# fnzhan/EMLight

Hardware: AMD Instinct MI355X
Metric: training images/sec (regression step: DenseNet-BC fwd + Sinkhorn loss + bwd + Adam) (higher is better)
Workload: dtype f32; 1 GPU; RegressionNetwork train step, BASELINE configs[1]; per_gpu_batch=64, global_batch=64, anchors=128, parallelism=single

## Files before the change

### emlight_amd/RegressionNetwork/dense_engine_bwd.py

```python
import ctypes
import os

import torch

from .. import _lib
from .._knobs import knob_choice, knob_flag


def _r16(v):
    return (v + 15) // 16 * 16


def _side_stream(dev, prio):
    if prio <= 0:
        return torch.cuda.Stream(device=dev, priority=prio)
    hip = ctypes.CDLL("libamdhip64.so")
    h = ctypes.c_void_p()
    with torch.cuda.device(dev):
        rc = hip.hipStreamCreateWithPriority(ctypes.byref(h), ctypes.c_uint(1), ctypes.c_int(prio))
    if rc != 0:
        raise RuntimeError("hipStreamCreateWithPriority failed (%d)" % rc)
    return torch.cuda.ExternalStream(h.value, device=dev)


def _masked_stream(dev, n_cu, keep):
    hip = ctypes.CDLL("libamdhip64.so")
    words = (n_cu + 31) // 32
    mask = (ctypes.c_uint32 * words)()
    for i in range(n_cu):
        if keep(i):
            mask[i // 32] |= 1 << (i % 32)
    h = ctypes.c_void_p()
    with torch.cuda.device(dev):
        rc = hip.hipExtStreamCreateWithCUMask(ctypes.byref(h), ctypes.c_uint32(words), mask)
    if rc != 0:
        raise RuntimeError("hipExtStreamCreateWithCUMask failed (%d)" % rc)
    return torch.cuda.ExternalStream(h.value, device=dev)


class _BwdBuffers:
    def __init__(self, enc, ws, dev):
        f32 = dict(dtype=torch.float32, device=dev)
        self.G = [torch.zeros(blk["P"], blk["ld"], **f32) for blk in ws.blocks]
        self.GF = torch.zeros(ws.F.shape[0], ws.F.shape[1], **f32)
        maxP = ws.blocks[0]["P"]
        self.DZ = torch.empty(2, maxP, 48, **f32)
        self.ring = max(1, int(os.environ.get("EML_WGRAD_RING", 4))) if enc.overlap_wgrad(dev) else 1
        self.GF12 = [torch.empty(maxP, 12, **f32) for _ in range(self.ring)]
        self.N12 = torch.empty(maxP, 12, **f32)
        self.TOP = torch.empty(2 * maxP * 12, **f32) if knob_flag("EML_DGRAD_TOP", True) else None
        kp, ko, g = enc.kp_max, max(enc.ko_max, 48), enc.grid_max
        self.Wd = [[torch.empty(lay["Kp"] * 48, **f32) for lay in blk["layers"]] for blk in ws.blocks]
        self.WdT = [torch.empty(blk["trans"]["Kp"] * blk["trans"]["Ko"], **f32) for blk in ws.blocks]
        self.permutes = None
        self.coef = torch.zeros(8, max(kp, ko), **f32)
        self.part2 = torch.zeros(2, g * kp * 2, dtype=torch.float64, device=dev)
        self.partW = torch.empty(g * max(kp * 48, 2 * 27 * 256, 4 * 1024), **f32)
        i32 = dict(dtype=torch.int32, device=dev)
        self.cond = [[torch.zeros(lay["Kp"], **i32) for lay in blk["layers"]] for blk in ws.blocks]
        self.condT = [torch.zeros(blk["trans"]["Kp"], **i32) for blk in ws.blocks]
        self.any_ill = torch.zeros(1, **i32)
        self.dg_grid = 128
        self.dg_scratch = torch.empty(self.dg_grid * kp, dtype=torch.float64, device=dev)
        self.side = None
        if enc.overlap_wgrad(dev):
            m = int(os.environ.get("EML_CU_SPLIT", 0))
            self.main_masked = None
            if m > 1:
                n_cu = torch.cuda.get_device_properties(dev).multi_processor_count
                self.side = _masked_stream(dev, n_cu, lambda i: i % m == m - 1)
                self.main_masked = _masked_stream(dev, n_cu, lambda i: i % m != m - 1)
            else:
                self.side = _side_stream(dev, int(os.environ.get("EML_SIDE_PRIO", 0)))
            self.partW3 = [torch.empty(g * 2 * 27 * 256, **f32) for _ in range(self.ring)]
            self.ev_ready = [torch.cuda.Event() for _ in range(self.ring)]
            self.ev_done = [None] * self.ring


def run_backward(enc, ws, x, gpooled, need_x=False, need_params=None):
    if getattr(ws, "bwd", None) is None:
        ws.bwd = _BwdBuffers(enc, ws, x.device)
    masked = getattr(ws.bwd, "main_masked", None)
    if masked is None:
        return _run_backward(enc, ws, x, gpooled, need_x, need_params)
    cur = torch.cuda.current_stream(x.device)
    masked.wait_stream(cur)
    with torch.cuda.stream(masked):
        out = _run_backward(enc, ws, x, gpooled, need_x, need_params)
    cur.wait_stream(masked)
    return out


def _run_backward(enc, ws, x, gpooled, need_x, need_params):
    L, p, st = _lib.lib(), _lib.ptr, _lib.current_stream()
    m = enc.model
    f = m.features
    if not m.training:
        raise NotImplementedError("HIP DenseNet backward is implemented for train-mode BatchNorm "
                                  "(EMLight trains and tests in train mode, train.py:42 / test.py:36-37)")
    dev = x.device
    B, _, H, W = x.shape
    G = enc._grid(dev)
    G3 = enc._grid3(dev)
    G3d = enc._tuned("EML_GRID3_DGRAD", 2 * G3 if knob_flag("EML_D3_SHORT", False) else G3)
    Gw = enc._tuned("EML_GRID_WGRAD1", G)
    Gd = enc._tuned("EML_GRID_DGRAD", G)
    Gb = min(enc.grid_max, 4 * enc._cu)
    bw = ws.bwd
    part = ws.partials
    ring = [0]
    if bw.side is not None:
        main = torch.cuda.current_stream(dev)
        st_side = ctypes.c_void_p(bw.side.cuda_stream)
        G3s = enc._tuned("EML_GRID3_SIDE", G3)
        bw.side.wait_stream(main)
    if bw.permutes is None:
        from .dense_engine import _PermuteTable
        bw.permutes = _PermuteTable()
    items = []
    for bi_, blk_ in enumerate(ws.blocks):
        mod_ = getattr(f, "denseblock%d" % (bi_ + 1))
        for l_, lay_ in enumerate(blk_["layers"]):
            items.append((getattr(mod_, "denselayer%d" % (l_ + 1)).conv1.weight, bw.Wd[bi_][l_], 2, 48, lay_["Cin"],
                          lay_["Kp"], 48))
        tr_ = blk_["trans"]
        items.append((getattr(f, "transition%d" % (bi_ + 1)).conv.weight, bw.WdT[bi_], 2, tr_["Cout"], blk_["Ctot"],
                      tr_["Kp"], tr_["Ko"]))
    bw.permutes.launch(L, st, items)
    params = enc.param_list()
    if need_params is None:
        need_params = [True] * len(params)
    from .._dist import grad_slot
    grads = {}
    for q, need in zip(params, need_params):
        slot = grad_slot(q) if need else None
        grads[id(q)] = slot if slot is not None else torch.empty_like(q)
    gr = lambda q: p(grads[id(q)])
    coefs = [tuple(bw.coef[3 * k + i] for i in range(3)) for k in range(2)]
    cA, cB, cC = coefs[0]
    sB, sC = bw.coef[6], bw.coef[7]

    direct = knob_choice("EML_DGAMMA_DIRECT", "always", ("always", "never")) != "never"
    c3_fold = knob_flag("EML_C3_FOLD", True)
    bw.any_ill.zero_()

    def dgamma_direct(blk, X_ld, Pin, Hin, Win, pool, DY, ld_dy, Zr, ld_z, co, Cout, conv, Cin, scale1, shift1, cond, bn):
        if not direct:
            return
        a, b, c = co if co is not None else (None, None, None)
        _lib.check(L.eml_dense_bn_dgamma_direct_f32(
            p(blk["X"]), X_ld, Pin, Hin, Win, pool, p(DY), ld_dy, p(Zr), ld_z, p(a), p(b), p(c), Cout, p(conv.weight), Cin,
            p(scale1), p(shift1), p(blk["mean"]), p(blk["istd"]), p(cond), p(bw.dg_scratch), gr(bn.weight), bw.dg_grid, st),
            "eml_dense_bn_dgamma_direct_f32")

    def finalize(R, pstride, count, bn, mean, istd, C, Cpad, coef=0, s_acc=None, src=None, c_lo=0, c_hi=None, conv=None,
                 cond=None):
        a, b, c = coefs[coef] if coef is not None else (None, None, None)
        wargs = (p(bn.bias), p(conv.weight), gr(conv.weight), conv.weight.shape[0]) if conv is not None else (None, None, None, 0)
        _lib.check(L.eml_dense_bn_bwd_finalize_f32(
            p(part if src is None else src), R, pstride, float(count), p(bn.weight), p(mean), p(istd), C, Cpad, 1,
            gr(bn.weight), gr(bn.bias), p(a), p(b), p(c),
            p(sB) if s_acc is not None else None, p(sC) if s_acc is not None else None, int(bool(s_acc)),
            c_lo, Cpad if c_hi is None else c_hi, *wargs, p(cond), p(bw.any_ill) if cond is not None else None, st),
            "eml_dense_bn_bwd_finalize_f32")

    def parr(tensors):
        return (ctypes.c_void_p * len(tensors))(*[t.data_ptr() for t in tensors])

    def materialize(Gbuf, blk, c0, n):
        _lib.check(L.eml_dense_grad_materialize_f32(p(Gbuf), blk["ld"], p(blk["X"]), blk["ld"], p(sB), p(sC), c0, n,
                                                    blk["P"], st), "eml_dense_grad_materialize_f32")

    cf, k = enc.trans_cout[-1], enc.avgpool
    ldF = ws.F.shape[1]
    _lib.check(L.eml_dense_head_pool_bwd_f32(p(gpooled), p(ws.F), ldF, cf, B, ws.hf, ws.wf, k, p(bw.GF), ldF, st),
               "eml_dense_head_pool_bwd_f32")
    dY, ld_dy = bw.GF, ldF
    nb = len(ws.blocks)
    for bi in reversed(range(nb)):
        blk, tr = ws.blocks[bi], ws.blocks[bi]["trans"]
        mod = getattr(f, "denseblock%d" % (bi + 1))
        T, LN = getattr(f, "transition%d" % (bi + 1)), getattr(f, "last_norm%d" % (bi + 1))
        P, Hb, Wb, ld, ctot = blk["P"], blk["H"], blk["W"], blk["ld"], blk["Ctot"]
        cout, Ko, kpt = tr["Cout"], tr["Ko"], tr["Kp"]
        Pn = B * (Hb // 2) * (Wb // 2)
        Gbuf = bw.G[bi]
        gl0 = sum(enc.block_layers[:bi])
        top2 = bw.TOP[:2 * P * 12].view(2, P, 12) if bw.TOP is not None else None
        _lib.check(L.eml_dense_bn_bwd_stats_f32(p(dY), ld_dy, p(tr["T"]), Ko, None, 0, 0, cout, Pn, p(tr["tmean"]),
                                                p(tr["tistd"]), p(part), Gb, st), "eml_dense_bn_bwd_stats_f32")
        finalize(Gb, 2 * cout, Pn, LN, tr["tmean"], tr["tistd"], cout, Ko, coef=0)
        _lib.check(L.eml_dense_conv1x1_bwd_weight_f32(
            p(tr["A"]), kpt, Pn, Hb // 2, Wb // 2, 0, kpt, ctot, p(tr["one"]), p(tr["zero"]), p(dY), ld_dy, p(tr["T"]),
            Ko, p(cA), p(cB), p(cC), cout, p(bw.partW), gr(T.conv.weight), G, None, None, 0, None, 0, None, None, st),
            "eml_dense_conv1x1_bwd_weight_f32")
        _lib.check(L.eml_dense_conv1x1_bwd_data_f32(
            p(dY), ld_dy, p(tr["T"]), Ko, p(cA), p(cB), p(cC), Ko, p(bw.WdT[bi]), None, ld, p(tr["scale"]),
            p(tr["shift"]), None, None, Pn, Hb, Wb, 1, kpt, p(Gbuf), ld, 0, p(part), G, p(tr["mask16"]), st),
            "eml_dense_conv1x1_bwd_data_f32")
        finalize(G, 2 * kpt, P, T.norm, blk["mean"], blk["istd"], ctot, kpt, coef=None, s_acc=False, conv=T.conv,
                 cond=bw.condT[bi])
        dgamma_direct(blk, ld, P, Hb, Wb, 1, dY, ld_dy, tr["T"], Ko, coefs[0], cout, T.conv, ctot, tr["scale"], tr["shift"],
                      bw.condT[bi], T.norm)
        def conv2_backward(l, slot, n12=False, narrow_lo=None, top=False):
            lay = blk["layers"][l]
            Lm = getattr(mod, "denselayer%d" % (l + 1))
            cin, kp, z, dz = lay["Cin"], lay["Kp"], blk["Z"][l], bw.DZ[slot]
            gsrc = (p(bw.N12), 12, 0) if n12 else (p(top2[1]), 12, 0) if top else (p(Gbuf), ld, cin)
            r = ring[0] = (ring[0] + 1) % bw.ring
            if bw.side is not None and bw.ev_done[r] is not None:
                main.wait_event(bw.ev_done[r])
            fold = (bw.side is None and c3_fold
                    and L.eml_dense_conv3x3_bwd_fused_supported(gsrc[1], gsrc[2], ld, cin) == 1)
            q = ws.drop_plan[bi][l] if ws.drop_plan is not None else 0.0
            drop = (ws.drop_key, gl0 + l, q) if q > 0 else ()
            if fold:
                fn = "eml_dense_conv3x3_bwd_fused_drop_f32" if drop else "eml_dense_conv3x3_bwd_fused_f32"
                _lib.check(getattr(L, fn)(*gsrc, p(Lm.conv2.weight), p(z), p(lay["zmean"]), p(lay["zistd"]), p(dz), B, Hb, Wb,
                                          p(part), G3d, p(blk["X"]), ld, cin, p(sB), p(sC), p(bw.GF12[r]), p(lay["scale2"]),
                                          p(lay["shift2"]), p(bw.partW), gr(Lm.conv2.weight), *drop, st), fn)
            else:
                fn = "eml_dense_conv3x3_bwd_data_drop_f32" if drop else "eml_dense_conv3x3_bwd_data_f32"
                _lib.check(getattr(L, fn)(*gsrc, p(Lm.conv2.weight), p(z), p(lay["zmean"]), p(lay["zistd"]), p(dz), B, Hb, Wb,
                                          p(part), G3d, p(blk["X"]), ld, cin, p(sB), p(sC), p(bw.GF12[r]), *drop, st), fn)
            if fold:
                pass
            elif bw.side is None:
                _lib.check(L.eml_dense_conv3x3_bwd_weight_f32(p(bw.GF12[r]), 12, 0, p(z), p(lay["scale2"]),
                                                              p(lay["shift2"]), B, Hb, Wb, p(bw.partW),
                                                              gr(Lm.conv2.weight), G3, st),
                           "eml_dense_conv3x3_bwd_weight_f32")
            else:
                bw.ev_ready[r].record(main)
                bw.side.wait_event(bw.ev_ready[r])
                _lib.check(L.eml_dense_conv3x3_bwd_weight_f32(p(bw.GF12[r]), 12, 0, p(z), p(lay["scale2"]),
                                                              p(lay["shift2"]), B, Hb, Wb, p(bw.partW3[r]),
                                                              gr(Lm.conv2.weight), G3s, st_side),
                           "eml_dense_conv3x3_bwd_weight_f32")
                if bw.ev_done[r] is None:
                    bw.ev_done[r] = torch.cuda.Event()
                bw.ev_done[r].record(bw.side)
            finalize(G3d, 96, P, Lm.norm2, lay["zmean"], lay["zistd"], 48, 48, coef=slot)
            a, b, c = coefs[slot]
            _lib.check(L.eml_dense_conv1x1_bwd_weight_f32(
                p(blk["X"]), ld, P, Hb, Wb, 0, kp, cin, p(lay["scale1"]), p(lay["shift1"]), p(dz), 48, p(z), 48,
                p(a), p(b), p(c), 48, p(bw.partW), gr(Lm.conv1.weight), Gw, p(dz),
                *((p(Lm.conv1.weight), narrow_lo, *((p(top2[0]), 12) if top else (p(Gbuf), ld)), p(bw.N12),
                   p(bw.part2[slot])) if narrow_lo is not None
                  else (None, 0, None, 0, None, None)), st), "eml_dense_conv1x1_bwd_weight_f32")
            return Lm

        def dgrad(layers, slots, k_lo, k_hi, top=False):
            lays = [blk["layers"][l] for l in layers]
            if top:
                _lib.check(L.eml_dense_conv1x1_bwd_data_multi_top_f32(
                    parr([bw.DZ[s_] for s_ in slots]), parr([bw.Wd[bi][l_] for l_ in layers]),
                    parr([y["scale1"] for y in lays]), parr([y["shift1"] for y in lays]),
                    parr([bw.part2[s_] for s_ in slots]), (ctypes.c_int * len(layers))(*[y["Kp"] for y in lays]),
                    P, k_hi, p(Gbuf), ld, Gd, parr([y["mask"] for y in lays]), p(top2), st),
                    "eml_dense_conv1x1_bwd_data_multi_top_f32")
                return
            _lib.check(L.eml_dense_conv1x1_bwd_data_multi_f32(
                len(layers), parr([bw.DZ[s_] for s_ in slots]), None, None, None, None,
                parr([bw.Wd[bi][l_] for l_ in layers]),
                parr([y["scale1"] for y in lays]), parr([y["shift1"] for y in lays]),
                parr([bw.part2[s_] for s_ in slots]), (ctypes.c_int * len(layers))(*[y["Kp"] for y in lays]),
                None, ld, None, None, P, k_lo, k_hi, p(Gbuf), ld, Gd,
                parr([y["mask"] for y in lays]), st),
                "eml_dense_conv1x1_bwd_data_multi_f32")

        def bn1_finalize(l, Lm, slot, c_lo, c_hi, rows=None):
            lay = blk["layers"][l]
            finalize(Gd if rows is None else rows, 2 * lay["Kp"], P, Lm.norm1, blk["mean"], blk["istd"], lay["Cin"], lay["Kp"], coef=None,
                     s_acc=True, src=bw.part2[slot], c_lo=c_lo, c_hi=c_hi, conv=Lm.conv1, cond=bw.cond[bi][l])

        def bn1_direct(l, Lm, slot):
            lay = blk["layers"][l]
            dgamma_direct(blk, ld, P, Hb, Wb, 0, bw.DZ[slot], 48, None, 0, None, 48, Lm.conv1, lay["Cin"], lay["scale1"],
                          lay["shift1"], bw.cond[bi][l], Lm.norm1)

        l = len(blk["layers"]) - 1
        have_top = False
        while l >= 0:
            if l >= 1:
                la, lb = l, l - 1
                cin_a, cin_b = blk["layers"][la]["Cin"], blk["layers"][lb]["Cin"]
                Lma = conv2_backward(la, 0, narrow_lo=cin_b, top=have_top)
                bn1_finalize(la, Lma, 0, cin_b, cin_a, rows=Gw)
                Lmb = conv2_backward(lb, 1, n12=True)
                to_top = (top2 is not None and lb >= 2 and blk["layers"][la]["mask"] is not None and bw.side is None
                          and cin_b >= 24 and cin_b % 4 == 0)
                dgrad([la, lb], [0, 1], 0, cin_b, top=to_top)
                have_top = to_top
                bn1_finalize(la, Lma, 0, 0, cin_b)
                bn1_finalize(lb, Lmb, 1, 0, blk["layers"][lb]["Kp"])
                bn1_direct(la, Lma, 0)
                bn1_direct(lb, Lmb, 1)
                l -= 2
            else:
                Lm0 = conv2_backward(l, 0)
                dgrad([l], [0], 0, blk["layers"][l]["Cin"])
                bn1_finalize(l, Lm0, 0, 0, blk["layers"][l]["Kp"])
                bn1_direct(l, Lm0, 0)
                l -= 1
        c0b = blk["C0"]
        norm0_fused = bi == 0 and knob_flag("EML_NORM0_FUSED", True) and c0b % 4 == 0 and c0b <= 32
        if not norm0_fused:
            materialize(Gbuf, blk, 0, c0b)
        dY, ld_dy = Gbuf, ld
    b0 = ws.blocks[0]
    c0 = enc.c_init
    if norm0_fused:
        _lib.check(L.eml_dense_norm0_bwd_stats_f32(p(dY), ld_dy, p(ws.Y0), c0, p(ws.scale0), p(ws.shift0), p(sB), p(sC), c0,
                                                   b0["P"], p(ws.mean0), p(ws.istd0), p(part), Gb, st),
                   "eml_dense_norm0_bwd_stats_f32")
    else:
        _lib.check(L.eml_dense_bn_bwd_stats_f32(p(dY), ld_dy, p(ws.Y0), c0, p(b0["X"]), b0["ld"], 1, c0, b0["P"],
                                                p(ws.mean0), p(ws.istd0), p(part), Gb, st), "eml_dense_bn_bwd_stats_f32")
    finalize(Gb, 2 * c0, b0["P"], f.norm0, ws.mean0, ws.istd0, c0, _r16(c0), coef=0)
    if norm0_fused:
        _lib.check(L.eml_dense_conv0_bwd_weight_fused_f32(p(x), p(dY), ld_dy, p(ws.Y0), c0, p(ws.scale0), p(ws.shift0), p(sB),
                                                          p(sC), p(cA), p(cB), p(cC), B, H, W, p(bw.partW),
                                                          gr(f.conv0.weight), G, st), "eml_dense_conv0_bwd_weight_fused_f32")
    else:
        _lib.check(L.eml_dense_conv0_bwd_weight_f32(p(x), p(dY), ld_dy, p(b0["X"]), b0["ld"], p(ws.Y0), c0, p(cA), p(cB),
                                                    p(cC), B, H, W, p(bw.partW), gr(f.conv0.weight), G, st),
                   "eml_dense_conv0_bwd_weight_f32")
    dx = None
    if need_x:
        dx = torch.empty(B, 3, H, W, dtype=torch.float32, device=dev)
        X1 = (None, 0) if norm0_fused else (p(b0["X"]), b0["ld"])
        _lib.check(L.eml_dense_conv0_bwd_data_f32(p(dY), ld_dy, *X1, p(ws.Y0), c0, p(ws.scale0), p(ws.shift0), p(sB), p(sC),
                                                  p(cA), p(cB), p(cC), p(f.conv0.weight), B, H, W, p(dx), st),
                   "eml_dense_conv0_bwd_data_f32")
    if bw.side is not None:
        main.wait_stream(bw.side)
    return dx, [grads[id(q)] for q in params]
```

### emlight_amd/_lib.py

```python
import ctypes
import os
import threading

_HERE = os.path.dirname(os.path.abspath(__file__))
LIB_PATH = os.environ.get("EML_LIB_PATH") or os.path.join(_HERE, "libemlight_hip.so")

_f32p = ctypes.c_void_p
_i32p = ctypes.c_void_p
_f64p = ctypes.c_void_p
_stream = ctypes.c_void_p
_int = ctypes.c_int
_u64 = ctypes.c_ulonglong

ABI_VERSION = 31

SIGNATURES = {
    "eml_abi_version": (_int, []),
    "eml_last_error": (ctypes.c_char_p, []),
    "eml_sg_rasterise_f32": (_int, [_f32p, _f32p, _f32p, _f32p, _int, _int, _int, _int, _stream]),
    "eml_sg_rasterise_ex_f32": (_int, [_f32p, _f32p, _f32p, _f32p, _int, _int, _int, _int, _int, ctypes.c_void_p, _stream]),
    "eml_sg_rasterise_bwd_colors_f32": (_int, [_f32p, _f32p, _f32p, _f32p, _int, _int, _int, _int, _stream]),
    "eml_emd_anchor_cost_f32": (_int, [_f32p, _f32p, _int, _stream]),
    "eml_sinkhorn_schedule_f32": (_int, [_f32p, _f32p, ctypes.c_long, ctypes.c_double, ctypes.c_double, _int,
                                         ctypes.c_double, _f32p, _f32p, _i32p, _f32p, _stream]),
    "eml_sinkhorn_work_floats": (ctypes.c_size_t, [_int, _int]),
    "eml_sinkhorn_fwd_f32": (_int, [_f32p, _f32p, _f32p, _f32p, _f32p, _f32p, ctypes.c_double, ctypes.c_double, _int,
                                    ctypes.c_double, _f32p, _f32p, _i32p, _f32p, _f32p, _f32p, _f32p, _f32p, _int, _int,
                                    _stream]),
    "eml_sinkhorn_fwd_ex_f32": (_int, [_f32p, _f32p, _f32p, _f32p, _f32p, _f32p, ctypes.c_double, ctypes.c_double, _int,
                                       ctypes.c_double, _f32p, _f32p, _i32p, _f32p, _f32p, _f32p, _f32p, _f32p, _int, _int,
                                       _int, _stream]),
    "eml_sinkhorn_fwd_rho_f32": (_int, [_f32p, _f32p, _f32p, _f32p, _f32p, _f32p, ctypes.c_double, ctypes.c_double, _int,
                                        ctypes.c_double, _f32p, _f32p, _i32p, _f32p, _f32p, _f32p, _f32p, _f32p, _int, _int,
                                        _int, ctypes.c_double, _f32p, _stream]),
    "eml_sinkhorn_bwd_f32": (_int, [_f32p, _f32p, _f32p, _int, _int, _stream]),
    "eml_l1_pairs_partial_doubles": (ctypes.c_size_t, [_int]),
    "eml_l1_pairs_fwd_f32": (_int, [_int, ctypes.c_void_p, ctypes.c_void_p, ctypes.c_void_p, ctypes.c_void_p, ctypes.c_void_p,
                                    ctypes.c_void_p, _f64p, _f32p, _stream]),
    "eml_l1_pairs_bwd_f32": (_int, [_int, ctypes.c_void_p, ctypes.c_void_p, ctypes.c_void_p, ctypes.c_void_p, ctypes.c_void_p,
                                    ctypes.c_void_p, _f32p, ctypes.c_void_p, ctypes.c_void_p, ctypes.c_void_p, _stream]),
    "eml_colsum_partial_doubles": (ctypes.c_size_t, [_int]),
    "eml_colsum_f32": (_int, [_f32p, ctypes.c_long, _int, _f64p, _f32p, _stream]),
    "eml_gt_anchor_index_i32": (_int, [_f32p, _int, _int, _int, _i32p, _stream]),
    "eml_gt_parametrise_f64": (_int, [_f32p, _i32p, _i32p, _int, _int, _int, _int, _f32p, _f32p, _f32p, _stream]),
    "eml_sphere_tap_table_f32": (_int, [_f32p, _int, _int, _int, _int, _i32p, _f32p, _stream]),
    "eml_sphere_im2col_f32": (_int, [_f32p, _i32p, _f32p, _f32p, _int, _int, _int, _int, _stream]),
    "eml_sphere_col2im_f32": (_int, [_f32p, _i32p, _i32p, _f32p, _f32p, _int, _int, _int, _int, _stream]),
    "eml_sphere_conv_fwd_fused_f32": (_int, [_f32p, _i32p, _f32p, _f32p, _f32p, _f32p, _int, _int, _int, _int, _int, _int,
                                             _stream]),
    "eml_sphere_conv_fwd_fused_ex_f32": (_int, [_f32p, _i32p, _f32p, _f32p, _f32p, _f32p, _int, _int, _int, _int, _int, _int,
                                                _f32p, ctypes.c_float, _int, _stream]),
    "eml_sphere_conv_small_supported": (_int, [_int, _int]),
    "eml_sphere_conv_small_fwd_f32": (_int, [_f32p, _i32p, _f32p, _f32p, _f32p, _f32p, _int, _int, _int, _int, _int,
                                             ctypes.c_float, _stream]),
    "eml_sphere_conv_small_wgrad_partial_floats": (ctypes.c_size_t, [_int, _int, _int, _int]),
    "eml_sphere_conv_small_wgrad_f32": (_int, [_f32p, _i32p, _f32p, _f32p, _f32p, ctypes.c_float, _f32p, _f32p, _f32p, _int,
                                               _int, _int, _int, _int, _stream]),
    "eml_sphere_conv_small_da9_f32": (_int, [_f32p, _f32p, ctypes.c_float, _f32p, _f32p, ctypes.c_long, _int, _int, _stream]),
    "eml_spade_norm_modulate_up2_fwd_f32": (_int, [_f32p, _f32p, _f32p, _int, _int, _int, _int, ctypes.c_float, _f32p, _f32p,
                                                   _stream]),
    "eml_spade_norm_modulate_bwd_cols_f32": (_int, [_f32p, _f32p, _f32p, _f32p, _f32p, _int, _int, _int, _int, _int,
                                                    ctypes.c_float, _f32p, _f32p, _f32p, _int, _stream]),
    "eml_sg_rasterise_bwd_work_floats": (ctypes.c_size_t, [_int, _int, _int, _int]),
    "eml_sg_rasterise_bwd_colors_ex_f32": (_int, [_f32p, _f32p, _f32p, _f32p, _f32p, _int, _int, _int, _int, _int, _stream]),
    "eml_sg_rasterise_bwd_full_work_floats": (ctypes.c_size_t, [_int, _int, _int, _int]),
    "eml_sg_rasterise_bwd_f32": (_int, [_f32p, _f32p, _f32p, _f32p, _f32p, _f32p, _f32p, _f32p, _int, _int, _int, _int, _int,
                                        _stream]),
    "eml_sphere_conv_narrow_supported": (_int, [_int, _int]),
    "eml_sphere_conv_narrow_fwd_f32": (_int, [_f32p, _i32p, _f32p, _f32p, _f32p, _f32p, _int, _int, _int, _int, _int, _stream]),
    "eml_sphere_conv_narrow_dgrad_f32": (_int, [_f32p, _i32p, _f32p, _int, _f32p, _f32p, _int, _int, _int, _int, _int, _stream]),
    "eml_sphere_conv_narrow_wgrad_partial_floats": (ctypes.c_size_t, [_int, _int, _int, _int]),
    "eml_sphere_conv_narrow_wgrad_f32": (_int, [_f32p, _i32p, _f32p, _f32p, _f32p, _f32p, _int, _int, _int, _int, _int, _stream]),
    "eml_sphere_conv_narrow_scratch_floats": (ctypes.c_size_t, [_int, _int]),
    "eml_sphere_conv_narrow_fwd2_f32": (_int, [_f32p, _i32p, _f32p, _f32p, _f32p, _f32p, _f32p, _int, _int, _int, _int, _int, _stream]),
    "eml_sphere_conv_narrow_wgrad2_partial_floats": (ctypes.c_size_t, [_int, _int, _int]),
    "eml_sphere_conv_narrow_dgrad2_f32": (_int, [_f32p, _i32p, _f32p, _int, ctypes.c_void_p, _f32p, _f32p, _f32p, _int, _int, _int,
                                                 _int, _int, _int, _stream]),
    "eml_sphere_conv_narrow_wgrad2_f32": (_int, [_f32p, _i32p, _f32p, _int, ctypes.c_void_p, _f32p, _f32p, _f32p, _f32p, _int, _int,
                                                 _int, _int, _int, _stream]),
    "eml_sphere_conv_spade_supported": (_int, [_int, _int, ctypes.c_long]),
    "eml_sphere_conv_spade_fwd_f32": (_int, [_f32p, _i32p, _f32p, _f32p, _f32p, _f32p, _f32p, _f32p, _f32p, _f32p, _int, _int,
                                             _int, _int, _int, _int, ctypes.c_float, _int, _stream]),
    "eml_spade_norm_modulate_bwd_y_f32": (_int, [_f32p, _f32p, _f32p, _f32p, _f32p, _f32p, _int, _int, _int, _int, _int,
                                                 ctypes.c_float, _f32p, _f32p, _f32p, _int, _stream]),
    "eml_bn_bwd_apply_up2_f32": (_int, [_f32p, _f32p, _int, _int, _int, _int, _f32p, _f32p, _f32p, _f32p, _stream]),
    "eml_spectral_norm_scratch_floats": (ctypes.c_size_t, [_int, _int]),
    "eml_spectral_norm_w2_f32": (_int, [_f32p, _f32p, _f32p, _int, ctypes.c_float, _f32p, _f32p, _f32p, _f32p, _int, _int,
                                        _stream]),
    "eml_spectral_norm_w2_bwd_f32": (_int, [_f32p, _f32p, _f32p, _f32p, _f32p, _f32p, _f32p, _int, _int, _stream]),
    "eml_spectral_norm_w2_batch_f32": (_int, [_int, ctypes.c_void_p, ctypes.c_void_p, ctypes.c_void_p, _int, ctypes.c_float,
                                              ctypes.c_void_p, ctypes.c_void_p, ctypes.c_void_p, ctypes.c_void_p, ctypes.c_void_p,
                                              ctypes.c_void_p, _stream]),
    "eml_spade_heads_w2_f32": (_int, [_f32p, _f32p, _f32p, _f32p, _f32p, _f32p, _int, _int, _int, _stream]),
    "eml_instance_norm_act_fwd_f32": (_int, [_f32p, _f32p, _f32p, _int, _int, _int, _int, ctypes.c_float, ctypes.c_float,
                                             _stream]),
    "eml_instance_norm_act_bwd_f32": (_int, [_f32p, _f32p, _f32p, _f32p, _int, _int, _int, _int, ctypes.c_float, _stream]),
    "eml_sphere_conv_dgrad_fused_f32": (_int, [_f32p, _i32p, _f32p, _i32p, _int, _f32p, _f32p, _int, _int, _int, _int, _int,
                                               _int, _stream]),
    "eml_sphere_conv_lowres_variant": (_int, [_int, _int, _int, _int]),
    "eml_sphere_conv_lowres_table_i32": (_int, [_i32p, _i32p, _i32p, _int, _int, _stream]),
    "eml_sphere_conv_lowres_partial_floats": (ctypes.c_size_t, [ctypes.c_long, _int, _int]),
    "eml_sphere_conv_lowres_f32": (_int, [_f32p, _i32p, _f32p, _i32p, _int, _i32p, _int, _f32p, _f32p, _f32p, _f32p, _int, _int,
                                          _int, _int, _int, _int, _f32p, ctypes.c_float, _stream]),
    "eml_sphere_conv_wgrad_partial_floats": (ctypes.c_size_t, [_int, _int, _int]),
    "eml_sphere_conv_wgrad_fused_f32": (_int, [_f32p, _i32p, _f32p, _f32p, _f32p, _f32p, _int, _int, _int, _int, _int, _int,
                                               _stream]),
    "eml_spade_modulate_fwd_f32": (_int, [_f32p, _int, _f32p, _int, _f32p, _int, ctypes.c_long, _int, ctypes.c_float,
                                          _stream]),
    "eml_spade_modulate_bwd_f32": (_int, [_f32p, _int, _f32p, _int, _f32p, _int, _f32p, _int, _f32p, _int, ctypes.c_long,
                                          _int, ctypes.c_float, _stream]),
    "eml_bn_stats_f32": (_int, [_f32p, _int, ctypes.c_long, _int, _f32p, _int, _stream]),
    "eml_bn_fold_f64": (_int, [_f32p, _int, _int, _f32p, _stream]),
    "eml_bn_finalize_f32": (_int, [_f32p, _int, ctypes.c_float, ctypes.c_float, _f32p, _f32p, _f32p, _f32p, _stream]),
    "eml_spade_norm_modulate_fwd_f32": (_int, [_f32p, _int, _f32p, _int, _f32p, _int, ctypes.c_long, _int, ctypes.c_float,
                                               _f32p, _f32p, _stream]),
    "eml_bn_bwd_apply_f32": (_int, [_f32p, _int, _f32p, _int, ctypes.c_long, _int, _f32p, _f32p, _f32p, _f32p, _int,
                                    _stream]),
    "eml_dense_conv0_fwd_f32": (_int, [_f32p, _f32p, _f32p, _int, _int, _int, _int, _int, _f32p, _int, _stream]),
    "eml_dense_conv0_fwd_mfma_f32": (_int, [_f32p, _f32p, _f32p, _int, _int, _int, _int, _int, _f32p, _int, _stream]),
    "eml_dense_bn_apply_f32": (_int, [_f32p, _int, _f32p, _int, _int, ctypes.c_long, _f32p, _f32p, _int, _f32p,
                                      _int, _stream]),
    "eml_dense_bn_prepare_f32": (_int, [_f32p, _int, _int, _int, _int, ctypes.c_double, _f32p, _f32p, _f32p, _f32p,
                                        _f32p, _f32p, _f32p, _int, _int, ctypes.c_float, ctypes.c_float, _int,
                                        _f32p, _f32p, _stream]),
    "eml_dense_permute_w1_f32": (_int, [_f32p, _int, _int, _int, _f32p, _stream]),
    "eml_dense_permute_w2_f32": (_int, [_f32p, _int, _f32p, _stream]),
    "eml_dense_permute_batch_f32": (_int, [ctypes.c_void_p, _int, _stream]),
    "eml_dense_conv1x1_fwd_f32": (_int, [_f32p, _int, ctypes.c_long, _int, _int, _int, _int, _f32p, _f32p, _f32p,
                                         _int, _f32p, _int, _f32p, _int, ctypes.c_void_p, _stream]),
    "eml_dense_conv3x3_fwd_f32": (_int, [_f32p, _f32p, _f32p, _f32p, _f32p, _int, _int, _int, _int, _int, _f32p,
                                         _int, _stream]),
    "eml_dense_permute_w2_tp_f32": (_int, [_f32p, _f32p, _stream]),
    "eml_dense_conv3x3_fwd_tp_supported": (_int, [_int, _int, _int]),
    "eml_dense_conv3x3_fwd_tp_f32": (_int, [_f32p, _f32p, _f32p, _f32p, _f32p, _int, _int, _int, _int, _int, _int, _f32p,
                                            _int, _stream]),
    "eml_dense_conv3x3_fwd_drop_f32": (_int, [_f32p, _f32p, _f32p, _f32p, _f32p, _int, _int, _int, _int, _int, _f32p,
                                              _int, _u64, _int, ctypes.c_double, _stream]),
    "eml_dense_conv3x3_fwd_tp_drop_f32": (_int, [_f32p, _f32p, _f32p, _f32p, _f32p, _int, _int, _int, _int, _int, _int, _f32p,
                                                 _int, _u64, _int, ctypes.c_double, _stream]),
    "eml_dense_dropout_mask_u16": (_int, [_u64, _int, ctypes.c_double, ctypes.c_long, ctypes.c_void_p, _stream]),
    "eml_dense_pool_act_f32": (_int, [_f32p, _int, _int, _int, _int, _int, _f32p, _f32p, _f32p, _int, ctypes.c_void_p,
                                      _stream]),
    "eml_dense_head_pool_fwd_f32": (_int, [_f32p, _int, _int, _int, _int, _int, _int, _f32p, _stream]),
    "eml_dense_conv3x3_bwd_data_f32": (_int, [_f32p, _int, _int, _f32p, _f32p, _f32p, _f32p, _f32p, _int, _int, _int,
                                              _f32p, _int, _f32p, _int, _int, _f32p, _f32p, _f32p, _stream]),
    "eml_dense_conv3x3_bwd_fused_supported": (_int, [_int, _int, _int, _int]),
    "eml_dense_conv3x3_bwd_fused_f32": (_int, [_f32p, _int, _int, _f32p, _f32p, _f32p, _f32p, _f32p, _int, _int, _int, _f64p, _int,
                                               _f32p, _int, _int, _f32p, _f32p, _f32p, _f32p, _f32p, _f32p, _f32p, _stream]),
    "eml_dense_conv3x3_bwd_data_drop_f32": (_int, [_f32p, _int, _int, _f32p, _f32p, _f32p, _f32p, _f32p, _int, _int, _int,
                                                   _f32p, _int, _f32p, _int, _int, _f32p, _f32p, _f32p, _u64, _int,
                                                   ctypes.c_double, _stream]),
    "eml_dense_conv3x3_bwd_fused_drop_f32": (_int, [_f32p, _int, _int, _f32p, _f32p, _f32p, _f32p, _f32p, _int, _int, _int,
                                                    _f64p, _int, _f32p, _int, _int, _f32p, _f32p, _f32p, _f32p, _f32p, _f32p,
                                                    _f32p, _u64, _int, ctypes.c_double, _stream]),
    "eml_dense_conv3x3_bwd_weight_f32": (_int, [_f32p, _int, _int, _f32p, _f32p, _f32p, _int, _int, _int, _f32p,
                                                _f32p, _int, _stream]),
    "eml_dense_bn_bwd_finalize_f32": (_int, [_f32p, _int, _int, ctypes.c_double, _f32p, _f32p, _f32p, _int, _int,
                                             _int, _f32p, _f32p, _f32p, _f32p, _f32p, _f32p, _f32p, _int, _int, _int,
                                             _f32p, _f32p, _f32p, _int, _i32p, _i32p, _stream]),
    "eml_dense_bn_dgamma_direct_f32": (_int, [_f32p, _int, ctypes.c_long, _int, _int, _int, _f32p, _int, _f32p, _int,
                                              _f32p, _f32p, _f32p, _int, _f32p, _int, _f32p, _f32p, _f32p, _f32p, _i32p,
                                              _f32p, _f32p, _int, _stream]),
    "eml_dense_conv1x1_bwd_weight_f32": (_int, [_f32p, _int, ctypes.c_long, _int, _int, _int, _int, _int, _f32p,
                                                _f32p, _f32p, _int, _f32p, _int, _f32p, _f32p, _f32p, _int, _f32p,
                                                _f32p, _int, _f32p, _f32p, _int, _f32p, _int, _f32p, _f32p, _stream]),
    "eml_dense_conv1x1_bwd_narrow_f32": (_int, [_f32p, _f32p, _int, _int, _f32p, _int, _f32p, _f32p, _f32p, _f32p,
                                                ctypes.c_long, _f32p, _int, _f32p, _f32p, _int, _int, _stream]),
    "eml_dense_permute_w1_bwd_f32": (_int, [_f32p, _int, _int, _int, _int, _f32p, _stream]),
    "eml_dense_conv1x1_bwd_data_f32": (_int, [_f32p, _int, _f32p, _int, _f32p, _f32p, _f32p, _int, _f32p, _f32p,
                                              _int, _f32p, _f32p, _f32p, _f32p, ctypes.c_long, _int, _int, _int,
                                              _int, _f32p, _int, _int, _f32p, _int, ctypes.c_void_p, _stream]),
    "eml_dense_conv1x1_bwd_data_multi_f32": (_int, [_int] + [ctypes.c_void_p] * 10 + [_f32p, _int, _f32p, _f32p,
                                                    ctypes.c_long, _int, _int, _f32p, _int, _int, ctypes.c_void_p,
                                                    _stream]),
    "eml_dense_conv1x1_bwd_data_multi_top_f32": (_int, [ctypes.c_void_p] * 6 + [ctypes.c_long, _int, _f32p, _int, _int,
                                                        ctypes.c_void_p, _f32p, _stream]),
    "eml_dense_grad_materialize_f32": (_int, [_f32p, _int, _f32p, _int, _f32p, _f32p, _int, _int, ctypes.c_long,
                                              _stream]),
    "eml_dense_bn_bwd_stats_f32": (_int, [_f32p, _int, _f32p, _int, _f32p, _int, _int, _int, ctypes.c_long, _f32p,
                                          _f32p, _f32p, _int, _stream]),
    "eml_dense_norm0_bwd_stats_f32": (_int, [_f32p, _int, _f32p, _int, _f32p, _f32p, _f32p, _f32p, _int, ctypes.c_long, _f32p, _f32p,
                                             ctypes.c_void_p, _int, _stream]),
    "eml_dense_conv0_bwd_weight_fused_f32": (_int, [_f32p, _f32p, _int, _f32p, _int, _f32p, _f32p, _f32p, _f32p, _f32p, _f32p, _f32p,
                                                    _int, _int, _int, _f32p, _f32p, _int, _stream]),
    "eml_dense_conv0_bwd_weight_f32": (_int, [_f32p, _f32p, _int, _f32p, _int, _f32p, _int, _f32p, _f32p, _f32p,
                                              _int, _int, _int, _f32p, _f32p, _int, _stream]),
    "eml_dense_conv0_bwd_data_f32": (_int, [_f32p, _int, _f32p, _int, _f32p, _int, _f32p, _f32p, _f32p, _f32p, _f32p, _f32p,
                                            _f32p, _f32p, _int, _int, _int, _f32p, _stream]),
    "eml_dense_head_pool_bwd_f32": (_int, [_f32p, _f32p, _int, _int, _int, _int, _int, _int, _f32p, _int, _stream]),
}

_lock = threading.Lock()
_lib = None


class EmlightHipError(RuntimeError):
    pass


def lib():
    global _lib
    if _lib is not None:
        return _lib
    with _lock:
        if _lib is not None:
            return _lib
        if not os.path.exists(LIB_PATH):
            raise EmlightHipError(
                "libemlight_hip.so not found at %s -- build it with "
                "`python -c 'import __graft_entry__ as g; g.build()'` or `make -C emlight_amd/csrc`. "
                "There is no CPU fallback." % LIB_PATH)
        handle = ctypes.CDLL(LIB_PATH)
        for name, (res, args) in SIGNATURES.items():
            try:
                fn = getattr(handle, name)
            except AttributeError as e:
                raise EmlightHipError("libemlight_hip.so lacks symbol %s" % name) from e
            fn.restype, fn.argtypes = res, args
        got = handle.eml_abi_version()
        if got != ABI_VERSION:
            raise EmlightHipError("libemlight_hip.so has ABI version %d, this binding expects %d -- rebuild it "
                                  "(make -C emlight_amd/csrc)" % (got, ABI_VERSION))
        _lib = handle
    from . import _gemm_selection
    _gemm_selection.ensure_if_requested()
    return _lib


_DEBUG_SYNC = bool(os.environ.get("EML_DEBUG_SYNC"))


def check(rc, what):
    if rc != 0:
        msg = lib().eml_last_error()
        raise EmlightHipError("%s failed (rc=%d): %s" % (what, rc, msg.decode() if msg else "?"))
    if _DEBUG_SYNC:
        import sys
        import torch
        sys.stderr.write("[eml] %s ... " % what)
        sys.stderr.flush()
        torch.cuda.synchronize()
        sys.stderr.write("ok\n")


def ptr(t):
    if t is None:
        return None
    return ctypes.c_void_p(t.data_ptr())


def current_stream():
    import torch
    return ctypes.c_void_p(torch.cuda.current_stream().cuda_stream)


def require_gpu_tensor(t, name, dtype=None):
    import torch
    if not isinstance(t, torch.Tensor) or not t.is_cuda:
        raise EmlightHipError("%s must be a tensor on the MI355X (got %s); there is no CPU path"
                              % (name, getattr(t, "device", type(t))))
    if t.dtype != (dtype or torch.float32):
        raise EmlightHipError("%s must be %s (got %s)" % (name, dtype or torch.float32, t.dtype))
    return t.contiguous()
```

### emlight_amd/csrc/dense_bwd.hip

```cpp
#include "eml_common.h"
#include "eml_dropout.h"

#include <cstdint>
#include <cstdlib>
#include <type_traits>

namespace {

using f32x4 = __attribute__((ext_vector_type(4))) float;

__device__ __forceinline__ f32x4 mfma16(float a, float b, f32x4 c) {
  return __builtin_amdgcn_mfma_f32_16x16x4f32(a, b, c, 0, 0, 0);
}
__device__ __forceinline__ float f4c(const float4& v, int t) { return t == 0 ? v.x : t == 1 ? v.y : t == 2 ? v.z : v.w; }
__device__ __forceinline__ double shfl_xor_d(double v, int m) { return __shfl_xor(v, m, 64); }

constexpr int kTH = 8, kTW = 32, kHH = kTH + 2, kHW = kTW + 2;

constexpr int kPSG = 14;
constexpr int kBD = 512;
constexpr int kGRows = 2;
constexpr int kGPass = kHH / kGRows;

template <bool FUSE, bool WIDE, int TH, bool DROP = false>
// ... 991 lines not shown
        }
        __builtin_amdgcn_sched_barrier(0);
      }
    };
    if (role == 0) phase_b(std::integral_constant<int, 3>{});
    else phase_b(std::integral_constant<int, 4>{});
    EML_C3_STAMP(2);
    eml::lds_barrier();
    EML_C3_STAMP(3);
#ifdef EML_STAMPS
    st_acc[4] += 1;
#endif
    cur ^= 1;
  }
#ifdef EML_STAMPS
  if (tid == 0)
    for (int i = 0; i < 5; ++i) atomicAdd(&eml_c3_stamps[i], st_acc[i]);
#endif
  asm volatile("s_waitcnt vmcnt(0)" ::: "memory");
  __syncthreads();
  float* wsum = smem;
  for (int w8 = 0; w8 < 8; ++w8) {
    if (wave == w8) {
#pragma unroll
      for (int i = 0; i < 4; ++i)
        if (i < 3 + role) {
#pragma unroll
          for (int n = 0; n < 3; ++n)
#pragma unroll
            for (int g = 0; g < 4; ++g) {
              float* q = wsum + ((((3 * role + i) * 3 + n) * 16 + 4 * kk + g) * 16 + r);
              *q = ((w8 & 3) == 0 ? 0.f : *q) + accw[i][n][g];
            }
        }
    }
    __syncthreads();
  }
  for (int e = tid; e < 21 * 256; e += 512) partialW[(size_t)blockIdx.x * (21 * 256) + e] = wsum[e];
  if (tid < 48) {
    double t1 = 0.0, t2 = 0.0;
#pragma unroll
    for (int w8 = 0; w8 < 8; ++w8) {
      t1 += red[(w8 * 48 + tid) * 2 + 0];
      t2 += red[(w8 * 48 + tid) * 2 + 1];
    }
    partials[(size_t)blockIdx.x * 96 + 2 * tid + 0] = t1;
    partials[(size_t)blockIdx.x * 96 + 2 * tid + 1] = (double)zistd[tid] * (t2 - (double)zmean[tid] * t1);
  }
}


__global__ __launch_bounds__(256) void bn_bwd_finalize_kernel(
    const double* __restrict__ partials, int R, int pstride, double count, const float* __restrict__ gamma,
    const float* __restrict__ mean, const float* __restrict__ istd, int C, int Cpad, int training,
    float* __restrict__ dgamma, float* __restrict__ dbeta, float* __restrict__ cA, float* __restrict__ cB,
    float* __restrict__ cC, float* __restrict__ sB, float* __restrict__ sC, int s_accumulate, int c_lo, int c_hi,
    const float* __restrict__ beta, const float* __restrict__ Wc, const float* __restrict__ dWc, int w_rows,
    int* __restrict__ cond , int* __restrict__ any_cond ) {
  const int lane = threadIdx.x & 63, wave = threadIdx.x >> 6;
  const int c = c_lo + blockIdx.x * 4 + wave;
  if (c >= Cpad || c >= c_hi) return;
  float a = 0.f, b = 0.f, d = 0.f;
  if (c < C) {
    double S1 = 0.0, S2 = 0.0;
    for (int g = lane; g < R; g += 64) {
      S1 += partials[(size_t)g * pstride + 2 * c];
      S2 += partials[(size_t)g * pstride + 2 * c + 1];
    }
    double Q = 0.0;
    if (Wc)
      for (int o = lane; o < w_rows; o += 64) Q += (double)Wc[(size_t)o * C + c] * (double)dWc[(size_t)o * C + c];
#pragma unroll
    for (int o = 32; o > 0; o >>= 1) {
      S1 += __shfl_xor(S1, o, 64);
      S2 += __shfl_xor(S2, o, 64);
      Q += __shfl_xor(Q, o, 64);
    }
    if (Wc) {
      const double ga0 = gamma[c], bs = (double)beta[c] * S1, num = Q - bs;
      S2 = fabs(ga0) >= 1e-12 ? num / ga0 : 0.0;
      if (cond && lane == 0) {
        const int ill = fabs(ga0) < 1e-3 * fabs((double)beta[c]) || ga0 == 0.0;
        cond[c] = ill;
        if (ill && any_cond) *any_cond = 1;
      }
    }
    if (lane == 0) {
      dgamma[c] = (float)S2;
      dbeta[c] = (float)S1;
    }
    const double ga = gamma[c], is = istd[c], mu = mean[c];
    a = (float)(ga * is);
    if (training) {
      b = (float)(-ga * is * is * S2 / count);
      d = (float)(-ga * is * S1 / count + ga * is * is * S2 / count * mu);
    }
  }
  if (lane != 0) return;
  if (cA) {
    cA[c] = a;
    cB[c] = b;
    cC[c] = d;
  }
  if (sB) {
    sB[c] = (s_accumulate ? sB[c] : 0.f) + b;
    sC[c] = (s_accumulate ? sC[c] : 0.f) + d;
  }
}

__global__ __launch_bounds__(256) void reduce_rows_kernel(const float* __restrict__ partial, int R, size_t row_stride,
                                                          int mode, int dim0, int dim1, int n0,
                                                          float* __restrict__ out) {
  __shared__ double red[4][64];
  const int tid = threadIdx.x, e = blockIdx.x * 64 + (tid & 63), slice = tid >> 6;
  size_t src = 0, dst = 0;
  bool valid = false;
  if (mode == 0) {
    const int k = e / 48, o = e - 48 * k;
    valid = k < dim0 && o < dim1;
    src = (size_t)e;
    dst = (size_t)(n0 + o) * dim0 + k;
  } else if (mode == 1) {
    const int o = e & 15, ci = (e >> 4) & 15, pair = e >> 8, tap = pair / 3, mc = pair - 3 * tap;
    valid = pair < 27 && o < 12;
    src = (size_t)e;
    dst = (size_t)(o * 48 + 16 * mc + ci) * 9 + tap;
  } else if (mode == 3) {
    const int j = e & 15, i = (e >> 4) & 15, tn = e >> 8, t = tn / 3, n = tn - 3 * t, row = 16 * t + i;
    valid = tn < 21 && row < 108;
    src = (size_t)e;
    dst = (size_t)((row % 12) * 48 + 16 * n + j) * 9 + row / 12;
  } else {
    const int t = e >> 5, o = e & 31;
    valid = t < 27 && o < dim1;
    src = (size_t)e;
    dst = (size_t)o * 27 + t;
  }
  double s = 0.0;
  if (valid) {
#pragma unroll 8
    for (int r = slice; r < R; r += 4) s += (double)partial[(size_t)r * row_stride + src];
  }
  red[slice][tid & 63] = s;
  __syncthreads();
  if (slice == 0 && valid) out[dst] = (float)((red[0][tid] + red[1][tid]) + (red[2][tid] + red[3][tid]));
}

struct NarrowArgs {
  const float* W1;
  const float* G;
  float* N12;
  double* partials;
  int Cin, k_lo, ldg;
};
template <bool POOL, bool NARROW = false, int VEC = 2>
__global__ __launch_bounds__(256, (NARROW || VEC == 4) ? 2 : 1) void conv1x1_bwd_weight_kernel(
    const float* __restrict__ X, int ldx, int P, int Hin, int Win, int Kp, const float* __restrict__ scale1,
    const float* __restrict__ shift1, const float* __restrict__ DY, int ld_dy, const float* __restrict__ Zr,
    int ld_z, const float* __restrict__ cA, const float* __restrict__ cB, const float* __restrict__ cC, int n_valid,
    int n_load ,
    float* __restrict__ partial ,
    float* __restrict__ dz_out ,
    NarrowArgs na) {
  __shared__ __attribute__((aligned(16))) float dz_l[2][64 * 48];
  const int tid = threadIdx.x, lane = tid & 63, wave = tid >> 6;
  const int r = lane & 15, kk = lane >> 4;
  static_assert(VEC == 2 || (VEC == 4 && !POOL), "float4 operand: dense layers only");
  constexpr int GW = 16 * VEC;
  constexpr int MAXG = VEC == 2 ? 3 : 2;
  const int ngroups = (Kp + GW - 1) / GW;
  float nsk[4] = {0.f, 0.f, 0.f, 0.f}, ntk[4] = {0.f, 0.f, 0.f, 0.f};
  double ns1[4] = {0.0, 0.0, 0.0, 0.0};
  const int kq = min(kk, 2);
  if constexpr (NARROW) {
#pragma unroll
    for (int g = 0; g < 4; ++g) {
      nsk[g] = kk < 3 ? scale1[na.k_lo + 4 * kq + g] : 0.f;
      ntk[g] = kk < 3 ? shift1[na.k_lo + 4 * kq + g] : 0.f;
    }
  }

  float sv[MAXG][VEC], tv[MAXG][VEC];
  int coff[MAXG];
  bool gv[MAXG];
#pragma unroll
  for (int i = 0; i < MAXG; ++i) {
    const int cg = wave + 4 * i;
    const int ch = GW * cg + VEC * r;
    gv[i] = cg < ngroups && ch < Kp;
    coff[i] = gv[i] ? ch : 0;
#pragma unroll
    for (int t = 0; t < VEC; ++t) {
      sv[i][t] = gv[i] ? scale1[ch + t] : 0.f;
      tv[i][t] = gv[i] ? shift1[ch + t] : 0.f;
    }
  }
  const int spix = tid >> 2, sq = tid & 3;
  __shared__ __attribute__((aligned(16))) float co_l[3 * 48];
  __shared__ float wn_l[NARROW ? 12 * 64 : 1];
  constexpr bool CO_LDS = NARROW || VEC == 4;
  float4 sa_r[CO_LDS ? 1 : 3], sb_r[CO_LDS ? 1 : 3], sc_r[CO_LDS ? 1 : 3];
  if constexpr (CO_LDS) {
    if (tid < 48) {
      const bool v = tid < n_valid;
      co_l[tid] = v ? cA[tid] : 0.f;
      co_l[48 + tid] = v ? cB[tid] : 0.f;
      co_l[96 + tid] = v ? cC[tid] : 0.f;
    }
  } else {
#pragma unroll
    for (int j = 0; j < 3; ++j) {
      const int col = 4 * (sq + 4 * j);
      float a[4], b[4], c[4];
#pragma unroll
      for (int e = 0; e < 4; ++e) {
        const bool v = col + e < n_valid;
        a[e] = v ? cA[col + e] : 0.f;
        b[e] = v ? cB[col + e] : 0.f;
        c[e] = v ? cC[col + e] : 0.f;
      }
      sa_r[j] = make_float4(a[0], a[1], a[2], a[3]);
      sb_r[j] = make_float4(b[0], b[1], b[2], b[3]);
      sc_r[j] = make_float4(c[0], c[1], c[2], c[3]);
    }
  }
  if constexpr (NARROW) {
    for (int e = tid; e < 12 * 64; e += 256) {
      const int st = e >> 6, l = e & 63, rr = l & 15, k4 = l >> 4;
      wn_l[e] = rr < 12 ? na.W1[(size_t)(4 * st + k4) * na.Cin + na.k_lo + rr] : 0.f;
    }
  }
  __syncthreads();
  f32x4 acc[MAXG][VEC][3];
#pragma unroll
  for (int i = 0; i < MAXG; ++i)
#pragma unroll
    for (int t = 0; t < VEC; ++t)
#pragma unroll
      for (int n = 0; n < 3; ++n) acc[i][t][n] = f32x4{0.f, 0.f, 0.f, 0.f};

  const int Wo = Win >> 1, Ho = Hin >> 1;
  const int nchunks = (P + 63) >> 6;
  const int ngw = (ngroups > wave) ? (ngroups - wave + 3) >> 2 : 0;

  float4 rdy[3], rzr[3];
  bool rpv = false;
  int rp = 0;
  auto stage_load = [&](int chunk) {
    const int p = chunk * 64 + spix;
    rpv = chunk < nchunks && p < P;
    const size_t pc = rpv ? p : 0;
    rp = (int)pc;
#pragma unroll
    for (int j = 0; j < 3; ++j) {
      const int col = 4 * (sq + 4 * j);
      const bool cv = col < n_load;
      rdy[j] = cv ? *reinterpret_cast<const float4*>(DY + pc * ld_dy + col) : make_float4(0.f, 0.f, 0.f, 0.f);
      rzr[j] = cv ? *reinterpret_cast<const float4*>(Zr + pc * ld_z + col) : make_float4(0.f, 0.f, 0.f, 0.f);
    }
  };
  auto stage_write = [&](float* dzb) {
#pragma unroll
    for (int j = 0; j < 3; ++j) {
      const int col = 4 * (sq + 4 * j);
      float4 sa, sb, sc;
      if constexpr (CO_LDS) {
        sa = *reinterpret_cast<const float4*>(co_l + col);
        sb = *reinterpret_cast<const float4*>(co_l + 48 + col);
        sc = *reinterpret_cast<const float4*>(co_l + 96 + col);
      } else {
        sa = sa_r[j];
        sb = sb_r[j];
        sc = sc_r[j];
      }
      float4 v;
      v.x = rpv ? fmaf(sa.x, rdy[j].x, fmaf(sb.x, rzr[j].x, sc.x)) : 0.f;
      v.y = rpv ? fmaf(sa.y, rdy[j].y, fmaf(sb.y, rzr[j].y, sc.y)) : 0.f;
      v.z = rpv ? fmaf(sa.z, rdy[j].z, fmaf(sb.z, rzr[j].z, sc.z)) : 0.f;
      v.w = rpv ? fmaf(sa.w, rdy[j].w, fmaf(sb.w, rzr[j].w, sc.w)) : 0.f;
      *reinterpret_cast<float4*>(dzb + spix * 48 + col) = v;
      if (dz_out && rpv) *reinterpret_cast<float4*>(dz_out + (size_t)rp * 48 + col) = v;
    }
  };
  auto chunk_loop = [&](auto ngw_c) {
    constexpr int NGW = decltype(ngw_c)::value;
#ifdef EML_WGRAD_DEEP
    constexpr int UQ = POOL ? 1 : 2;
    constexpr int NBUF = POOL ? 2 : 4;
#else
    constexpr int UQ = POOL ? 1 : (VEC == 4 ? 2 : 4);
    constexpr int NBUF = 2;
#endif
    constexpr int NS = POOL ? 4 : 1;
    constexpr int NB = 16 / UQ;
    constexpr int AHEAD = NBUF - 1;
    using xv_t = std::conditional_t<VEC == 2, float2, float4>;
    xv_t xr[NBUF][UQ][NGW > 0 ? NGW : 1][NS];
    auto load_batch = [&](int chunk, int q0, xv_t (&dst)[UQ][NGW > 0 ? NGW : 1][NS]) {
#pragma unroll
      for (int u = 0; u < UQ; ++u) {
        const int pc = min(chunk * 64 + 4 * (q0 + u) + kk, P - 1);
        const float* xp;
        if constexpr (POOL) {
          const int b = pc / (Ho * Wo), rem = pc - b * (Ho * Wo);
          const int oy = rem / Wo, ox = rem - oy * Wo;
          xp = X + ((size_t)(b * Hin + 2 * oy) * Win + 2 * ox) * ldx;
        } else {
          xp = X + (size_t)pc * ldx;
        }
#pragma unroll
        for (int i = 0; i < NGW; ++i)
#pragma unroll
          for (int sub = 0; sub < NS; ++sub)
            dst[u][i][sub] = *reinterpret_cast<const xv_t*>(xp + ((sub >> 1) * (size_t)Win + (sub & 1)) * ldx + coff[i]);
      }
    };
    stage_load(blockIdx.x);
    stage_write(dz_l[0]);
    if constexpr (NGW > 0) {
#pragma unroll
      for (int a = 0; a < AHEAD; ++a) load_batch(min((int)blockIdx.x, nchunks - 1), a * UQ, xr[a]);
    }
    __syncthreads();
    int it = 0;
    for (int chunk = blockIdx.x; chunk < nchunks; chunk += gridDim.x, ++it) {
      const float* dzb = dz_l[it & 1];
      stage_load(chunk + gridDim.x);
      float2 nx[2], ng[2];
      const int pn = chunk * 64 + 16 * wave + r;
      if constexpr (NARROW) {
        const size_t pc = (size_t)min(pn, P - 1);
        const float* xs = X + pc * ldx + na.k_lo + 4 * kq;
        const float* gs = na.G + pc * na.ldg + (na.ldg == 12 ? 0 : na.k_lo) + 4 * kq;
        nx[0] = *reinterpret_cast<const float2*>(xs);
        nx[1] = *reinterpret_cast<const float2*>(xs + 2);
        ng[0] = *reinterpret_cast<const float2*>(gs);
        ng[1] = *reinterpret_cast<const float2*>(gs + 2);
      }
      if constexpr (NGW > 0) {
        float bzq[2][3];
#pragma unroll
        for (int n = 0; n < 3; ++n) bzq[0][n] = dzb[kk * 48 + 16 * n + r];
#pragma unroll
        for (int bi = 0; bi < NB; ++bi) {
          const int q0 = bi * UQ;
          if (bi + AHEAD < NB)
            load_batch(chunk, q0 + AHEAD * UQ, xr[(bi + AHEAD) % NBUF]);
          else
            load_batch(min(chunk + (int)gridDim.x, nchunks - 1), (bi + AHEAD - NB) * UQ, xr[(bi + AHEAD) % NBUF]);
          __builtin_amdgcn_sched_barrier(0);
#pragma unroll
          for (int u = 0; u < UQ; ++u) {
            const int pl = 4 * (q0 + u) + kk;
            const bool pvu = chunk * 64 + pl < P;
            float bz[3];
#pragma unroll
            for (int n = 0; n < 3; ++n) bz[n] = bzq[(q0 + u) & 1][n];
            if (q0 + u + 1 < 16) {
#pragma unroll
              for (int n = 0; n < 3; ++n) bzq[(q0 + u + 1) & 1][n] = dzb[(pl + 4) * 48 + 16 * n + r];
            }
#pragma unroll
            for (int i = 0; i < NGW; ++i) {
              float av[VEC];
#pragma unroll
              for (int t = 0; t < VEC; ++t) av[t] = 0.f;
#pragma unroll
              for (int sub = 0; sub < NS; ++sub) {
                const xv_t xv = xr[bi % NBUF][u][i][sub];
                av[0] += fmaxf(fmaf(xv.x, sv[i][0], tv[i][0]), 0.f);
                av[1] += fmaxf(fmaf(xv.y, sv[i][1], tv[i][1]), 0.f);
                if constexpr (VEC == 4) {
                  av[2] += fmaxf(fmaf(xv.z, sv[i][2], tv[i][2]), 0.f);
                  av[3] += fmaxf(fmaf(xv.w, sv[i][3], tv[i][3]), 0.f);
                }
              }
#pragma unroll
              for (int t = 0; t < VEC; ++t) {
                if constexpr (POOL) av[t] *= 0.25f;
                if (!pvu) av[t] = 0.f;
              }
#pragma unroll
              for (int n = 0; n < 3; ++n)
#pragma unroll
                for (int t = 0; t < VEC; ++t) acc[i][t][n] = mfma16(av[t], bz[n], acc[i][t][n]);
            }
          }
          __builtin_amdgcn_sched_barrier(0);
        }
      }
      if constexpr (NARROW) {
        asm volatile("" ::"v"(ng[0].x), "v"(ng[0].y), "v"(ng[1].x), "v"(ng[1].y), "v"(nx[0].x), "v"(nx[0].y), "v"(nx[1].x), "v"(nx[1].y));
        f32x4 an = f32x4{0.f, 0.f, 0.f, 0.f};
#pragma unroll
        for (int st = 0; st < 12; ++st) an = mfma16(wn_l[st * 64 + lane], dzb[(16 * wave + r) * 48 + 4 * st + kk], an);
        const bool nv = pn < P && kk < 3;
        const float xg[4] = {nx[0].x, nx[0].y, nx[1].x, nx[1].y}, gg[4] = {ng[0].x, ng[0].y, ng[1].x, ng[1].y};
        float o4[4];
#pragma unroll
        for (int g = 0; g < 4; ++g) {
          const float dam = (nv && fmaf(xg[g], nsk[g], ntk[g]) > 0.f) ? an[g] : 0.f;
          o4[g] = fmaf(nsk[g], dam, gg[g]);
          ns1[g] += (double)dam;
        }
        if (nv) *reinterpret_cast<float4*>(na.N12 + ((unsigned)pn * 12u + 4u * (unsigned)kk)) = make_float4(o4[0], o4[1], o4[2], o4[3]);
      }
      stage_write(dz_l[(it + 1) & 1]);
      eml::lds_barrier();
    }
  };
  switch (ngw) {
    case 0: chunk_loop(std::integral_constant<int, 0>{}); break;
    case 1: chunk_loop(std::integral_constant<int, 1>{}); break;
    case 2: chunk_loop(std::integral_constant<int, 2>{}); break;
    default: chunk_loop(std::integral_constant<int, MAXG>{}); break;
  }
  float* out = partial + (size_t)blockIdx.x * Kp * 48;
#pragma unroll
  for (int i = 0; i < MAXG; ++i) {
    const int cg = wave + 4 * i;
#pragma unroll
    for (int t = 0; t < VEC; ++t)
#pragma unroll
      for (int g = 0; g < 4; ++g) {
        const int ch = GW * cg + VEC * (4 * kk + g) + t;
        if (cg < ngroups && ch < Kp) {
#pragma unroll
          for (int n = 0; n < 3; ++n) out[(size_t)ch * 48 + 16 * n + r] = acc[i][t][n][g];
        }
      }
  }
  if constexpr (NARROW) {
    __syncthreads();
    double* red = reinterpret_cast<double*>(&dz_l[0][0]);
#pragma unroll
    for (int g = 0; g < 4; ++g) {
#pragma unroll
      for (int o = 1; o < 16; o <<= 1) ns1[g] += shfl_xor_d(ns1[g], o);
      if (r == 0 && kk < 3) red[wave * 12 + 4 * kk + g] = ns1[g];
    }
    __syncthreads();
    if (tid < 12) {
      double* dst = na.partials + ((size_t)blockIdx.x * Kp + na.k_lo + tid) * 2;
      dst[0] = (red[tid] + red[12 + tid]) + (red[24 + tid] + red[36 + tid]);
      dst[1] = 0.0;
    }
  }
}

template <bool POOL, bool RES , int NCH = 4>
__global__ __launch_bounds__(256) void conv1x1_bwd_data_kernel(
    const float* __restrict__ DY, int ld_dy, const float* __restrict__ Zr, int ld_z, const float* __restrict__ cA,
    const float* __restrict__ cB, const float* __restrict__ cC, int Ko, const float* __restrict__ Wd,
    const float* __restrict__ X, int ldx, const float* __restrict__ scale1, const float* __restrict__ shift1,
    const float* __restrict__ mean, const float* __restrict__ istd, int P, int Hin, int Win, int Kp,
    float* __restrict__ Gd, int ldg, int accumulate, double* __restrict__ partials ) {
  extern __shared__ __attribute__((aligned(16))) float smem[];
  double* sacc = reinterpret_cast<double*>(smem);
  const int tid = threadIdx.x, lane = tid & 63, wave = tid >> 6;
  const int r = lane & 15, kk = lane >> 4;
  for (int e = tid; e < 4 * Kp * 2; e += 256) sacc[e] = 0.0;
  __syncthreads();
  double* my = sacc + (size_t)wave * Kp * 2;
  const int nnt = Kp >> 4, njo = Ko >> 4;
  const int ntiles = (P + 255) >> 8;
  const int Wo = Win >> 1, Ho = Hin >> 1;

  for (int tile = blockIdx.x; tile < ntiles; tile += gridDim.x) {
    const int p0 = tile * 256 + wave * 64;
    long prow[4];
    size_t pin[4];
#pragma unroll
    for (int m = 0; m < 4; ++m) {
      prow[m] = min(p0 + 16 * m + r, P - 1);
      if constexpr (POOL) {
        const int b = (int)(prow[m] / (Ho * Wo)), rem = (int)(prow[m] - (long)b * (Ho * Wo));
        const int oy = rem / Wo, ox = rem - oy * Wo;
        pin[m] = (size_t)(b * Hin + 2 * oy) * Win + 2 * ox;
      } else {
        pin[m] = (size_t)prow[m];
      }
    }
    auto load_dz = [&](int jo, float4 (&dz)[4]) {
      const int ch = 16 * jo + 4 * kk;
      const float4 a4 = *reinterpret_cast<const float4*>(cA + ch);
      const float4 b4 = *reinterpret_cast<const float4*>(cB + ch);
      const float4 c4 = *reinterpret_cast<const float4*>(cC + ch);
#pragma unroll
      for (int m = 0; m < 4; ++m) {
        const float4 dy = *reinterpret_cast<const float4*>(DY + prow[m] * ld_dy + ch);
        const float4 zr = *reinterpret_cast<const float4*>(Zr + prow[m] * ld_z + ch);
        dz[m].x = fmaf(a4.x, dy.x, fmaf(b4.x, zr.x, c4.x));
        dz[m].y = fmaf(a4.y, dy.y, fmaf(b4.y, zr.y, c4.y));
        dz[m].z = fmaf(a4.z, dy.z, fmaf(b4.z, zr.z, c4.z));
        dz[m].w = fmaf(a4.w, dy.w, fmaf(b4.w, zr.w, c4.w));
      }
    };
    float4 dzr[3][4];
    if constexpr (RES) {
#pragma unroll
      for (int jo = 0; jo < 3; ++jo) load_dz(jo, dzr[jo]);
    }
    for (int nt0 = 0; nt0 < nnt; nt0 += NCH) {
      f32x4 acc[4][NCH];
#pragma unroll
      for (int m = 0; m < 4; ++m)
#pragma unroll
        for (int n = 0; n < NCH; ++n) acc[m][n] = f32x4{0.f, 0.f, 0.f, 0.f};
      auto mma = [&](int jo, const float4 (&dz)[4]) {
#pragma unroll
        for (int n = 0; n < NCH; ++n) {
          const int nt = min(nt0 + n, nnt - 1);
          const float4 w = *reinterpret_cast<const float4*>(Wd + ((((size_t)nt * njo + jo) * 4 + kk) * 16 + r) * 4);
#pragma unroll
          for (int t = 0; t < 4; ++t)
#pragma unroll
            for (int m = 0; m < 4; ++m) acc[m][n] = mfma16(f4c(w, t), f4c(dz[m], t), acc[m][n]);
        }
      };
      if constexpr (RES) {
#pragma unroll
        for (int jo = 0; jo < 3; ++jo) mma(jo, dzr[jo]);
      } else {
        for (int jo = 0; jo < njo; ++jo) {
          float4 dz[4];
          load_dz(jo, dz);
          mma(jo, dz);
        }
      }
#pragma unroll
      for (int n = 0; n < NCH; ++n) {
        const int nt = nt0 + n;
        if (nt < nnt) {
          const int k4 = 16 * nt + 4 * kk;
          const float4 sk = *reinterpret_cast<const float4*>(scale1 + k4);
          const float4 tk = *reinterpret_cast<const float4*>(shift1 + k4);
          const float4 mu = *reinterpret_cast<const float4*>(mean + k4);
          const float4 is = *reinterpret_cast<const float4*>(istd + k4);
          float l1[4] = {0.f, 0.f, 0.f, 0.f}, l2[4] = {0.f, 0.f, 0.f, 0.f};
#pragma unroll
          for (int m = 0; m < 4; ++m) {
            if (p0 + 16 * m + r < P) {
              const float da[4] = {acc[m][n][0], acc[m][n][1], acc[m][n][2], acc[m][n][3]};
              constexpr int NSUB = POOL ? 4 : 1;
#pragma unroll
              for (int sub = 0; sub < NSUB; ++sub) {
                const size_t pi = pin[m] + (sub >> 1) * (size_t)Win + (sub & 1);
                const float4 xv = *reinterpret_cast<const float4*>(X + pi * ldx + k4);
                float4* gp = reinterpret_cast<float4*>(Gd + pi * ldg + k4);
                float4 g = accumulate ? *gp : make_float4(0.f, 0.f, 0.f, 0.f);
                const float f = POOL ? 0.25f : 1.0f;
                const float d0 = (fmaf(xv.x, sk.x, tk.x) > 0.f) ? f * da[0] : 0.f;
                const float d1 = (fmaf(xv.y, sk.y, tk.y) > 0.f) ? f * da[1] : 0.f;
                const float d2 = (fmaf(xv.z, sk.z, tk.z) > 0.f) ? f * da[2] : 0.f;
                const float d3 = (fmaf(xv.w, sk.w, tk.w) > 0.f) ? f * da[3] : 0.f;
                g.x = fmaf(sk.x, d0, g.x);
                g.y = fmaf(sk.y, d1, g.y);
                g.z = fmaf(sk.z, d2, g.z);
                g.w = fmaf(sk.w, d3, g.w);
                *gp = g;
                l1[0] += d0;
                l1[1] += d1;
                l1[2] += d2;
                l1[3] += d3;
                l2[0] = fmaf(d0, (xv.x - mu.x) * is.x, l2[0]);
                l2[1] = fmaf(d1, (xv.y - mu.y) * is.y, l2[1]);
                l2[2] = fmaf(d2, (xv.z - mu.z) * is.z, l2[2]);
                l2[3] = fmaf(d3, (xv.w - mu.w) * is.w, l2[3]);
              }
            }
          }
#pragma unroll
          for (int g = 0; g < 4; ++g) {
            l1[g] = eml::row16_sum(l1[g]);
            l2[g] = eml::row16_sum(l2[g]);
            if (r == 0) {
              my[2 * (k4 + g)] += (double)l1[g];
              my[2 * (k4 + g) + 1] += (double)l2[g];
            }
          }
        }
      }
    }
  }
  __syncthreads();
  for (int e = tid; e < Kp * 2; e += 256)
    partials[(size_t)blockIdx.x * Kp * 2 + e] =
        (sacc[e] + sacc[(size_t)Kp * 2 + e]) + (sacc[(size_t)2 * Kp * 2 + e] + sacc[(size_t)3 * Kp * 2 + e]);
}

template <int MT, int NCH, bool ACC , bool MASKED = false, int NJO = 0>
__global__ __launch_bounds__(256, 2) void transition_bwd_data_kernel(
    const float* __restrict__ DY, int ld_dy, const float* __restrict__ Zr, int ld_z, const float* __restrict__ cA,
    const float* __restrict__ cB, const float* __restrict__ cC, int Ko, const float* __restrict__ Wd,
    const float* __restrict__ X, int ldx, const float* __restrict__ scale1, const float* __restrict__ shift1,
    const float* __restrict__ mean, const float* __restrict__ istd, int P, int Hin, int Win, int Kp,
    float* __restrict__ Gd, int ldg, double* __restrict__ partials ,
// ... 132 lines not shown
          float4 dz[MT];
#pragma unroll
          for (int m = 0; m < MT; ++m) {
            dz[m].x = fmaf(a4.x, ry[m].x, fmaf(b4.x, rz[m].x, c4.x));
            dz[m].y = fmaf(a4.y, ry[m].y, fmaf(b4.y, rz[m].y, c4.y));
            dz[m].z = fmaf(a4.z, ry[m].z, fmaf(b4.z, rz[m].z, c4.z));
            dz[m].w = fmaf(a4.w, ry[m].w, fmaf(b4.w, rz[m].w, c4.w));
          }
          group_step(jo, dz);
        }
      }
      if constexpr (MASKED && !ACC) {
        float l1n[NCH][4];
        float4 skn[NCH];
#pragma unroll
        for (int n = 0; n < NCH; ++n) {
          skn[n] = *reinterpret_cast<const float4*>(vec_l + 16 * min(nt0 + n, nnt - 1) + 4 * kk);
#pragma unroll
          for (int g = 0; g < 4; ++g) l1n[n][g] = 0.f;
        }
        const int piece = lane & 7;
        const bool col_ok = nt0 + (piece >> 2) < nnt;
#pragma unroll
        for (int m = 0; m < MT; ++m) {
#pragma unroll
          for (int sub = 0; sub < 4; ++sub) {
#pragma unroll
            for (int n = 0; n < NCH; ++n) {
              const unsigned b = pv[m] ? mk[m][n] >> (4 * sub) : 0u;
              const float d0 = (b & 1u) ? 0.25f * acc[m][n][0] : 0.f, d1 = (b & 2u) ? 0.25f * acc[m][n][1] : 0.f;
              const float d2 = (b & 4u) ? 0.25f * acc[m][n][2] : 0.f, d3 = (b & 8u) ? 0.25f * acc[m][n][3] : 0.f;
              *reinterpret_cast<f32x4*>(stg + r * 36 + 16 * n + 4 * kk) = f32x4{skn[n].x * d0, skn[n].y * d1, skn[n].z * d2, skn[n].w * d3};
              if (nt0 + n < nnt) {
                l1n[n][0] += d0;
                l1n[n][1] += d1;
                l1n[n][2] += d2;
                l1n[n][3] += d3;
              }
            }
            __builtin_amdgcn_fence(__ATOMIC_RELEASE, "wavefront");
            __builtin_amdgcn_wave_barrier();
            __builtin_amdgcn_fence(__ATOMIC_ACQUIRE, "wavefront");
            const size_t suboff = ((size_t)(sub >> 1) * Win + (sub & 1)) * (size_t)ldg + 16 * nt0 + 4 * piece;
#pragma unroll
            for (int h = 0; h < 2; ++h) {
              const f32x4 v = *reinterpret_cast<const f32x4*>(stg + ((lane >> 3) + 8 * h) * 36 + 4 * piece);
              if (pvx[m][h] && col_ok) *reinterpret_cast<f32x4*>(Gd + pinx[m][h] * ldg + suboff) = v;
            }
            __builtin_amdgcn_fence(__ATOMIC_RELEASE, "wavefront");
            __builtin_amdgcn_wave_barrier();
            __builtin_amdgcn_fence(__ATOMIC_ACQUIRE, "wavefront");
          }
        }
#pragma unroll
        for (int n = 0; n < NCH; ++n) {
          if (nt0 + n < nnt) {
            const int k4 = 16 * (nt0 + n) + 4 * kk;
#pragma unroll
            for (int g = 0; g < 4; ++g) {
              const float t1 = eml::row16_sum(l1n[n][g]);
              if (r == 0) my[2 * (k4 + g)] += (double)t1;
            }
          }
        }
      } else {
#pragma unroll
      for (int n = 0; n < NCH; ++n) {
        const int nt = nt0 + n;
        if (nt < nnt) {
          const int k4 = 16 * nt + 4 * kk;
          const float4 sk = *reinterpret_cast<const float4*>(vec_l + k4);
          const float4 tk = *reinterpret_cast<const float4*>(vec_l + Kp + k4);
          const float4 mu = *reinterpret_cast<const float4*>(vec_l + 2 * Kp + k4);
          const float4 is = *reinterpret_cast<const float4*>(vec_l + 3 * Kp + k4);
          float l1[4] = {0.f, 0.f, 0.f, 0.f}, l2[4] = {0.f, 0.f, 0.f, 0.f};
#pragma unroll
          for (int m = 0; m < MT; ++m) {
            const float da0 = 0.25f * acc[m][n][0], da1 = 0.25f * acc[m][n][1];
            const float da2 = 0.25f * acc[m][n][2], da3 = 0.25f * acc[m][n][3];
#pragma unroll
            for (int sub = 0; sub < 4; ++sub) {
              float4 g = make_float4(0.f, 0.f, 0.f, 0.f);
              if constexpr (ACC) g = gs[m][n][sub];
              float d0, d1, d2, d3;
              float4 x = make_float4(0.f, 0.f, 0.f, 0.f);
              if constexpr (MASKED) {
                const unsigned b = pv[m] ? mk[m][n] >> (4 * sub) : 0u;
                d0 = (b & 1u) ? da0 : 0.f;
                d1 = (b & 2u) ? da1 : 0.f;
                d2 = (b & 4u) ? da2 : 0.f;
                d3 = (b & 8u) ? da3 : 0.f;
              } else {
                x = xv[m][n][sub];
                d0 = (pv[m] && fmaf(x.x, sk.x, tk.x) > 0.f) ? da0 : 0.f;
                d1 = (pv[m] && fmaf(x.y, sk.y, tk.y) > 0.f) ? da1 : 0.f;
                d2 = (pv[m] && fmaf(x.z, sk.z, tk.z) > 0.f) ? da2 : 0.f;
                d3 = (pv[m] && fmaf(x.w, sk.w, tk.w) > 0.f) ? da3 : 0.f;
              }
              g.x = fmaf(sk.x, d0, g.x);
              g.y = fmaf(sk.y, d1, g.y);
              g.z = fmaf(sk.z, d2, g.z);
              g.w = fmaf(sk.w, d3, g.w);
              if (pv[m]) {
                const size_t pi = pin[m] + (sub >> 1) * (size_t)Win + (sub & 1);
                *reinterpret_cast<float4*>(Gd + pi * ldg + k4) = g;
              }
              l1[0] += d0;
              l1[1] += d1;
              l1[2] += d2;
              l1[3] += d3;
              if constexpr (!MASKED) {
                l2[0] = fmaf(d0, (x.x - mu.x) * is.x, l2[0]);
                l2[1] = fmaf(d1, (x.y - mu.y) * is.y, l2[1]);
                l2[2] = fmaf(d2, (x.z - mu.z) * is.z, l2[2]);
                l2[3] = fmaf(d3, (x.w - mu.w) * is.w, l2[3]);
              }
            }
          }
#pragma unroll
          for (int g = 0; g < 4; ++g) {
            l1[g] = eml::row16_sum(l1[g]);
            if constexpr (!MASKED) l2[g] = eml::row16_sum(l2[g]);
            if (r == 0) {
              my[2 * (k4 + g)] += (double)l1[g];
              if constexpr (!MASKED) my[2 * (k4 + g) + 1] += (double)l2[g];
            }
          }
        }
      }
      }
    }
  }
  __syncthreads();
  for (int e = tid; e < Kp * 2; e += 256)
    partials[(size_t)blockIdx.x * Kp * 2 + e] =
        (sacc[e] + sacc[(size_t)Kp * 2 + e]) + (sacc[(size_t)2 * Kp * 2 + e] + sacc[(size_t)3 * Kp * 2 + e]);
}

struct BwdLayer {
  const float* DZ;
  const float* Zr;
  const float* cA;
  const float* cB;
  const float* cC;
  const float* Wd;
  const float* scale1;
  const float* shift1;
  double* partials;
  int Kp;
};

template <int NL, int MT , bool RAW = false ,
          bool MASKED = false, bool TOP = false>
__global__ __launch_bounds__(256, 2) void conv1x1_bwd_data_multi_kernel(BwdLayer L0, BwdLayer L1,
                                                                        const float* __restrict__ X, int ldx,
                                                                        const float* __restrict__ mean,
                                                                        const float* __restrict__ istd, int P,
                                                                        int k_lo, int k_hi, float* __restrict__ Gd,
                                                                        int ldg, int KpMax,
                                                                        const unsigned long long* __restrict__ M0,
                                                                        const unsigned long long* __restrict__ M1,
                                                                        float* __restrict__ Top) {
  extern __shared__ __attribute__((aligned(16))) float smem[];
  double* sacc = reinterpret_cast<double*>(smem);
  float* vec_l = reinterpret_cast<float*>(sacc + (size_t)NL * 4 * KpMax * 2);
  const int tid = threadIdx.x, lane = tid & 63, wave = tid >> 6;
  const int r = lane & 15, kk = lane >> 4;
  const BwdLayer Ls[2] = {L0, L1};
  for (int e = tid; e < NL * 4 * KpMax * 2; e += 256) sacc[e] = 0.0;
  for (int e = tid; e < KpMax; e += 256) {
    vec_l[e] = MASKED ? 0.f : mean[e];
    vec_l[KpMax + e] = MASKED ? 0.f : istd[e];
#pragma unroll
    for (int j = 0; j < NL; ++j) {
      vec_l[(2 + 2 * j) * KpMax + e] = e < Ls[j].Kp ? Ls[j].scale1[e] : 0.f;
      vec_l[(3 + 2 * j) * KpMax + e] = e < Ls[j].Kp ? Ls[j].shift1[e] : 0.f;
    }
  }
  __syncthreads();
  constexpr int TP = 64 * MT;
  const int ntiles = (P + TP - 1) / TP;
  const int nt_lo = k_lo >> 4, nt_hi = (k_hi + 15) >> 4;
  constexpr int NCH = 2;

  float4 wq[2][3][NCH];
  auto load_w = [&](int j, int nt0, float4 (&dst)[3][NCH]) {
    const int nnt = Ls[j].Kp >> 4;
#pragma unroll
    for (int jo = 0; jo < 3; ++jo)
#pragma unroll
      for (int n = 0; n < NCH; ++n) {
        const int nt = min(nt0 + n, nnt - 1);
        dst[jo][n] = *reinterpret_cast<const float4*>(Ls[j].Wd + ((((size_t)nt * 3 + jo) * 4 + kk) * 16 + r) * 4);
      }
  };
  load_w(0, nt_lo, wq[0]);
  int wsel = 0;

  for (int tile = blockIdx.x; tile < ntiles; tile += gridDim.x) {
    const int p0 = tile * TP + wave * 16 * MT;
    long prow[MT];
    bool pv[MT];
#pragma unroll
    for (int m = 0; m < MT; ++m) {
      pv[m] = p0 + 16 * m + r < P;
      prow[m] = min(p0 + 16 * m + r, P - 1);
    }
    unsigned long long pvb[MT];
#pragma unroll
    for (int m = 0; m < MT; ++m) pvb[m] = MASKED ? __ballot(pv[m]) : 0ull;
    float4 dz[NL][3][MT];
#pragma unroll
    for (int j = 0; j < NL; ++j)
#pragma unroll
      for (int jo = 0; jo < 3; ++jo) {
        const int ch = 16 * jo + 4 * kk;
        if constexpr (RAW) {
#pragma unroll
          for (int m = 0; m < MT; ++m) dz[j][jo][m] = *reinterpret_cast<const float4*>(Ls[j].DZ + prow[m] * 48 + ch);
        } else {
          const float4 a4 = *reinterpret_cast<const float4*>(Ls[j].cA + ch);
          const float4 b4 = *reinterpret_cast<const float4*>(Ls[j].cB + ch);
          const float4 c4 = *reinterpret_cast<const float4*>(Ls[j].cC + ch);
#pragma unroll
          for (int m = 0; m < MT; ++m) {
            const float4 dy = *reinterpret_cast<const float4*>(Ls[j].DZ + prow[m] * 48 + ch);
            const float4 zr = *reinterpret_cast<const float4*>(Ls[j].Zr + prow[m] * 48 + ch);
            dz[j][jo][m].x = fmaf(a4.x, dy.x, fmaf(b4.x, zr.x, c4.x));
            dz[j][jo][m].y = fmaf(a4.y, dy.y, fmaf(b4.y, zr.y, c4.y));
            dz[j][jo][m].z = fmaf(a4.z, dy.z, fmaf(b4.z, zr.z, c4.z));
            dz[j][jo][m].w = fmaf(a4.w, dy.w, fmaf(b4.w, zr.w, c4.w));
          }
        }
      }
    for (int nt0 = nt_lo; nt0 < nt_hi; nt0 += NCH) {
      float4 gs[MT][NCH], xv[MT][NCH];
#pragma unroll
      for (int n = 0; n < NCH; ++n) {
        const int k4 = 16 * min(nt0 + n, nt_hi - 1) + 4 * kk;
        const int k4l = (k4 + 3 >= k_lo && k4 < k_hi) ? k4 : (k_lo & ~3);
#pragma unroll
        for (int m = 0; m < MT; ++m) {
          gs[m][n] = *reinterpret_cast<const float4*>(Gd + prow[m] * ldg + k4l);
          if constexpr (!MASKED) xv[m][n] = *reinterpret_cast<const float4*>(X + prow[m] * ldx + k4l);
        }
      }
      const int nt_next = nt0 + NCH < nt_hi ? nt0 + NCH : nt_lo;
#pragma unroll
      for (int j = 0; j < NL; ++j) {
        const int nnt = Ls[j].Kp >> 4;
        unsigned long long mk[MT][NCH][4];
        if constexpr (MASKED) {
          const unsigned long long* __restrict__ Mj = j == 0 ? M0 : M1;
#pragma unroll
          for (int m = 0; m < MT; ++m)
#pragma unroll
            for (int n = 0; n < NCH; ++n) {
              const size_t wi =
                  ((size_t)__builtin_amdgcn_readfirstlane((p0 >> 4) + m) * nnt + min(nt0 + n, nnt - 1)) * 4;
#pragma unroll
              for (int g = 0; g < 4; ++g) mk[m][n][g] = Mj[wi + g];
            }
        }
        const int cur = NL == 2 ? j : wsel;
        if (j + 1 < NL)
          load_w(j + 1, nt0, wq[cur ^ 1]);
        else
          load_w(0, nt_next, wq[cur ^ 1]);
        __builtin_amdgcn_sched_barrier(0);
        f32x4 acc[MT][NCH];
#pragma unroll
        for (int m = 0; m < MT; ++m)
#pragma unroll
          for (int n = 0; n < NCH; ++n) acc[m][n] = f32x4{0.f, 0.f, 0.f, 0.f};
#pragma unroll
        for (int jo = 0; jo < 3; ++jo)
#pragma unroll
          for (int t = 0; t < 4; ++t)
#pragma unroll
            for (int n = 0; n < NCH; ++n)
#pragma unroll
              for (int m = 0; m < MT; ++m) acc[m][n] = mfma16(f4c(wq[cur][jo][n], t), f4c(dz[j][jo][m], t), acc[m][n]);
        if (NL == 1) wsel ^= 1;
        double* my = sacc + ((size_t)(j * 4 + wave) * KpMax) * 2;
#pragma unroll
        for (int n = 0; n < NCH; ++n) {
          const int nt = nt0 + n;
          if (nt < nnt && nt < nt_hi) {
            const int k4 = 16 * nt + 4 * kk;
            const float4 mu = *reinterpret_cast<const float4*>(vec_l + k4);
            const float4 is = *reinterpret_cast<const float4*>(vec_l + KpMax + k4);
            const float4 sk = *reinterpret_cast<const float4*>(vec_l + (2 + 2 * j) * KpMax + k4);
            const float4 tk = *reinterpret_cast<const float4*>(vec_l + (3 + 2 * j) * KpMax + k4);
            const bool in0 = k4 + 0 >= k_lo && k4 + 0 < k_hi, in1 = k4 + 1 >= k_lo && k4 + 1 < k_hi;
            const bool in2 = k4 + 2 >= k_lo && k4 + 2 < k_hi, in3 = k4 + 3 >= k_lo && k4 + 3 < k_hi;
            unsigned long long inb[4] = {0ull, 0ull, 0ull, 0ull};
            if constexpr (MASKED) {
              inb[0] = __ballot(in0);
              inb[1] = __ballot(in1);
              inb[2] = __ballot(in2);
              inb[3] = __ballot(in3);
            }
            float l1[4] = {0.f, 0.f, 0.f, 0.f}, l2[4] = {0.f, 0.f, 0.f, 0.f};
#pragma unroll
            for (int m = 0; m < MT; ++m) {
              float d0, d1, d2, d3;
              if constexpr (MASKED) {
                d0 = __builtin_amdgcn_inverse_ballot_w64(mk[m][n][0] & pvb[m] & inb[0]) ? acc[m][n][0] : 0.f;
                d1 = __builtin_amdgcn_inverse_ballot_w64(mk[m][n][1] & pvb[m] & inb[1]) ? acc[m][n][1] : 0.f;
                d2 = __builtin_amdgcn_inverse_ballot_w64(mk[m][n][2] & pvb[m] & inb[2]) ? acc[m][n][2] : 0.f;
                d3 = __builtin_amdgcn_inverse_ballot_w64(mk[m][n][3] & pvb[m] & inb[3]) ? acc[m][n][3] : 0.f;
              } else {
                const float4 x = xv[m][n];
                d0 = (pv[m] && in0 && fmaf(x.x, sk.x, tk.x) > 0.f) ? acc[m][n][0] : 0.f;
                d1 = (pv[m] && in1 && fmaf(x.y, sk.y, tk.y) > 0.f) ? acc[m][n][1] : 0.f;
                d2 = (pv[m] && in2 && fmaf(x.z, sk.z, tk.z) > 0.f) ? acc[m][n][2] : 0.f;
                d3 = (pv[m] && in3 && fmaf(x.w, sk.w, tk.w) > 0.f) ? acc[m][n][3] : 0.f;
                l2[0] = fmaf(d0, (x.x - mu.x) * is.x, l2[0]);
                l2[1] = fmaf(d1, (x.y - mu.y) * is.y, l2[1]);
                l2[2] = fmaf(d2, (x.z - mu.z) * is.z, l2[2]);
                l2[3] = fmaf(d3, (x.w - mu.w) * is.w, l2[3]);
              }
              gs[m][n].x = fmaf(sk.x, d0, gs[m][n].x);
              gs[m][n].y = fmaf(sk.y, d1, gs[m][n].y);
              gs[m][n].z = fmaf(sk.z, d2, gs[m][n].z);
              gs[m][n].w = fmaf(sk.w, d3, gs[m][n].w);
              l1[0] += d0;
              l1[1] += d1;
              l1[2] += d2;
              l1[3] += d3;
            }
#pragma unroll
            for (int g = 0; g < 4; ++g) {
              l1[g] = eml::row16_sum(l1[g]);
              if constexpr (!MASKED) l2[g] = eml::row16_sum(l2[g]);
              if (r == 0) {
                my[2 * (k4 + g)] += (double)l1[g];
                if constexpr (!MASKED) my[2 * (k4 + g) + 1] += (double)l2[g];
              }
            }
          }
        }
      }
#pragma unroll
      for (int n = 0; n < NCH; ++n) {
        const int nt = nt0 + n;
        if (nt < nt_hi) {
          const int k4 = 16 * nt + 4 * kk;
          const bool act = k4 + 3 >= k_lo && k4 < k_hi;
          if constexpr (TOP) {
            const int t = k4 - (k_hi - 24);
            float* cdst = Top + (t >= 12 ? (size_t)P * 12 + (t - 12) : (size_t)max(t, 0));
#pragma unroll
            for (int m = 0; m < MT; ++m) {
              float* dst = t >= 0 ? cdst + prow[m] * 12 : Gd + prow[m] * ldg + k4;
              if (pv[m] && act) *reinterpret_cast<float4*>(dst) = gs[m][n];
            }
          } else {
#pragma unroll
            for (int m = 0; m < MT; ++m) {
              if (pv[m] && act) *reinterpret_cast<float4*>(Gd + prow[m] * ldg + k4) = gs[m][n];
            }
          }
        }
      }
    }
  }
  __syncthreads();
#pragma unroll
  for (int j = 0; j < NL; ++j) {
    const int Kp = Ls[j].Kp;
    const double* base = sacc + (size_t)j * 4 * KpMax * 2;
    for (int e = tid; e < Kp * 2; e += 256)
      Ls[j].partials[(size_t)blockIdx.x * Kp * 2 + e] = (base[e] + base[(size_t)KpMax * 2 + e]) +
                                                        (base[(size_t)2 * KpMax * 2 + e] + base[(size_t)3 * KpMax * 2 + e]);
  }
}

template <int MT>
__global__ __launch_bounds__(256, 2) void conv1x1_bwd_narrow_kernel(
    const float* __restrict__ DZ, const float* __restrict__ W1 , int Cin, int k_lo,
    const float* __restrict__ X, int ldx, const float* __restrict__ scale1, const float* __restrict__ shift1,
    const float* __restrict__ mean, const float* __restrict__ istd, int P, const float* __restrict__ Gd, int ldg,
    float* __restrict__ N12, double* __restrict__ partials , int Kp) {
  __shared__ double red[4][12][2];
  const int tid = threadIdx.x, lane = tid & 63, wave = tid >> 6;
  const int r = lane & 15, kk = lane >> 4;
  float aw[3][4];
#pragma unroll
  for (int jo = 0; jo < 3; ++jo)
#pragma unroll
    for (int t = 0; t < 4; ++t) aw[jo][t] = r < 12 ? W1[(size_t)(16 * jo + 4 * kk + t) * Cin + k_lo + r] : 0.f;
  const bool cv = kk < 3;
  const int cq = k_lo + 4 * (cv ? kk : 2);
  float sk[4], tk[4], mu[4], is[4];
#pragma unroll
  for (int g = 0; g < 4; ++g) {
    sk[g] = scale1[cq + g];
    tk[g] = shift1[cq + g];
    mu[g] = mean[cq + g];
    is[g] = istd[cq + g];
  }
  double s1[4] = {0.0, 0.0, 0.0, 0.0}, s2[4] = {0.0, 0.0, 0.0, 0.0};
  constexpr int TP = 64 * MT;
  const int ntiles = (P + TP - 1) / TP;
  for (int tile = blockIdx.x; tile < ntiles; tile += gridDim.x) {
    const int p0 = tile * TP + wave * 16 * MT;
    size_t prow[MT];
    bool pv[MT];
    float4 dz[MT][3];
    float2 xa[MT], xb[MT], ga[MT], gb[MT];
#pragma unroll
    for (int m = 0; m < MT; ++m) {
      pv[m] = p0 + 16 * m + r < P;
      prow[m] = (size_t)min(p0 + 16 * m + r, P - 1);
#pragma unroll
      for (int jo = 0; jo < 3; ++jo) dz[m][jo] = *reinterpret_cast<const float4*>(DZ + prow[m] * 48 + 16 * jo + 4 * kk);
      xa[m] = *reinterpret_cast<const float2*>(X + prow[m] * ldx + cq);
      xb[m] = *reinterpret_cast<const float2*>(X + prow[m] * ldx + cq + 2);
      ga[m] = *reinterpret_cast<const float2*>(Gd + prow[m] * ldg + cq);
      gb[m] = *reinterpret_cast<const float2*>(Gd + prow[m] * ldg + cq + 2);
    }
    f32x4 acc[MT];
#pragma unroll
    for (int m = 0; m < MT; ++m) acc[m] = f32x4{0.f, 0.f, 0.f, 0.f};
#pragma unroll
    for (int jo = 0; jo < 3; ++jo)
#pragma unroll
      for (int t = 0; t < 4; ++t)
#pragma unroll
        for (int m = 0; m < MT; ++m) acc[m] = mfma16(aw[jo][t], f4c(dz[m][jo], t), acc[m]);
#pragma unroll
    for (int m = 0; m < MT; ++m) {
      const float x[4] = {xa[m].x, xa[m].y, xb[m].x, xb[m].y};
      const float gold[4] = {ga[m].x, ga[m].y, gb[m].x, gb[m].y};
      float o[4];
#pragma unroll
      for (int g = 0; g < 4; ++g) {
        const float d = (pv[m] && cv && fmaf(x[g], sk[g], tk[g]) > 0.f) ? acc[m][g] : 0.f;
        o[g] = fmaf(sk[g], d, gold[g]);
        s1[g] += (double)d;
        s2[g] += (double)(d * ((x[g] - mu[g]) * is[g]));
      }
      if (pv[m] && cv) *reinterpret_cast<float4*>(N12 + prow[m] * 12 + 4 * kk) = make_float4(o[0], o[1], o[2], o[3]);
    }
  }
#pragma unroll
  for (int g = 0; g < 4; ++g) {
#pragma unroll
    for (int o = 1; o < 16; o <<= 1) {
      s1[g] += shfl_xor_d(s1[g], o);
      s2[g] += shfl_xor_d(s2[g], o);
    }
    if (r == 0 && cv) {
      red[wave][4 * kk + g][0] = s1[g];
      red[wave][4 * kk + g][1] = s2[g];
    }
  }
  __syncthreads();
  if (tid < 24) {
    const int c = tid >> 1, e = tid & 1;
    partials[((size_t)blockIdx.x * Kp + k_lo + c) * 2 + e] = (red[0][c][e] + red[1][c][e]) + (red[2][c][e] + red[3][c][e]);
  }
}

__global__ void permute_w1_bwd_kernel(const float* __restrict__ W, int Cout, int Cin, int Kp, int Ko,
                                      float* __restrict__ Wd) {
  const size_t total = (size_t)Kp * Ko;
  for (size_t e = (size_t)blockIdx.x * blockDim.x + threadIdx.x; e < total; e += (size_t)gridDim.x * blockDim.x) {
    const int t = (int)(e & 3), col = (int)((e >> 2) & 15), kk = (int)((e >> 6) & 3);
    const size_t rest = e >> 8;
    const int jo = (int)(rest % (Ko >> 4)), nt = (int)(rest / (Ko >> 4));
    const int o = 16 * jo + 4 * kk + t, k = 16 * nt + col;
    Wd[e] = (o < Cout && k < Cin) ? W[(size_t)o * Cin + k] : 0.f;
  }
}

__global__ __launch_bounds__(256) void grad_materialize_kernel(float* __restrict__ Gd, int ldg,
                                                               const float* __restrict__ X, int ldx,
                                                               const float* __restrict__ sB,
                                                               const float* __restrict__ sC, int c0, int n, size_t P) {
  const int nh = n >> 1;
  const size_t total = P * nh;
  for (size_t e = (size_t)blockIdx.x * 256 + threadIdx.x; e < total; e += (size_t)gridDim.x * 256) {
    const size_t p = e / nh;
    const int c = c0 + 2 * (int)(e - p * nh);
    const float2 x = *reinterpret_cast<const float2*>(X + p * ldx + c);
    float2* gp = reinterpret_cast<float2*>(Gd + p * ldg + c);
    float2 g = *gp;
    g.x += fmaf(sB[c], x.x, sC[c]);
    g.y += fmaf(sB[c + 1], x.y, sC[c + 1]);
    *gp = g;
  }
}

__global__ __launch_bounds__(256) void bn_bwd_stats_kernel(const float* __restrict__ DY, int ld_dy,
                                                           const float* __restrict__ raw, int ld_raw,
                                                           const float* __restrict__ out, int ld_out, int relu, int C,
                                                           size_t P, const float* __restrict__ mean,
                                                           const float* __restrict__ istd,
                                                           double* __restrict__ partials ) {
  extern __shared__ __attribute__((aligned(16))) float smem[];
  double* red = reinterpret_cast<double*>(smem);
  const int tid = threadIdx.x, lane = tid & 63, wave = tid >> 6;
  const int nk = (C + 63) >> 6;
// ... 529 lines not shown
#ifdef EML_STAMPS
extern "C" int eml_c3_read_stamps(unsigned long long* out, int reset) {
  if (hipMemcpyFromSymbol(out, HIP_SYMBOL(eml_c3_stamps), 8 * sizeof(unsigned long long)) != hipSuccess) return -1;
  if (reset) {
    const unsigned long long z[8] = {0};
    if (hipMemcpyToSymbol(HIP_SYMBOL(eml_c3_stamps), z, sizeof(z)) != hipSuccess) return -1;
  }
  return 0;
}
#endif
extern "C" int eml_dense_conv3x3_bwd_fused_supported(int ldg, int c0, int ldx, int cx) {
  return ((ldg & 1) == 0 && (c0 & 1) == 0 && (ldx & 1) == 0 && (cx & 1) == 0) ? 1 : 0;
}
template <bool DROP>
static int conv3x3_bwd_fused_launch(const char* name, const float* G, int ldg, int c0, const float* W2, const float* Z,
                                    const float* zmean, const float* zistd, float* DZ, int B, int H, int W, double* partials,
                                    int grid, const float* X, int ldx, int cx, const float* sB, const float* sC, float* GF,
                                    const float* scale2, const float* shift2, float* partialW, float* dW2, eml::DropKey dk,
                                    eml_stream_t stream) {
  if (!G || !W2 || !Z || !zmean || !zistd || !DZ || !partials || !X || !sB || !sC || !GF || !scale2 || !shift2 || !partialW ||
      !dW2 || B < 1 || H < 1 || W < 1 || grid < 1 || cx < 0)
    return eml::fail(EML_EINVAL, "%s: bad arguments", name);
  const auto al16 = [](const void* q) { return (reinterpret_cast<uintptr_t>(q) & 15) == 0; };
  if (!eml_dense_conv3x3_bwd_fused_supported(ldg, c0, ldx, cx) || !al16(G) || !al16(X) || !al16(GF) || !al16(Z) || !al16(scale2) ||
      !al16(shift2))
    return eml::fail(EML_EINVAL, "%s: needs even ldg, c0, ldx, cx and 16-byte aligned buffers", name);
  const bool a16 = (ldg & 3) == 0 && (c0 & 3) == 0 && (ldx & 3) == 0 && (cx & 3) == 0;
#ifndef EML_C3_WTP
#define EML_C3_WTP 1
#endif
#if EML_C3_WTP
  const size_t lds = (size_t)(2 * kHH * kHW * kPSG + 2 * kTH * kTW * 48 + 27 * 3 * 64 + 32) * sizeof(float) + 8 * 48 * 2 * sizeof(double);
  if (a16) {
    EML_ENSURE_LDS((&conv3x3_bwd_fused_tp_kernel<true, DROP>), lds);
    hipLaunchKernelGGL((conv3x3_bwd_fused_tp_kernel<true, DROP>), dim3(grid), dim3(512), lds, (hipStream_t)stream, G, ldg, c0, W2, Z,
                       zmean, zistd, DZ, B, H, W, partials, X, ldx, cx, sB, sC, GF, scale2, shift2, partialW, dk);
  } else {
    EML_ENSURE_LDS((&conv3x3_bwd_fused_tp_kernel<false, DROP>), lds);
    hipLaunchKernelGGL((conv3x3_bwd_fused_tp_kernel<false, DROP>), dim3(grid), dim3(512), lds, (hipStream_t)stream, G, ldg, c0, W2, Z,
                       zmean, zistd, DZ, B, H, W, partials, X, ldx, cx, sB, sC, GF, scale2, shift2, partialW, dk);
  }
  int rc = eml::check_launch(name);
  if (rc) return rc;
  hipLaunchKernelGGL(reduce_rows_kernel, dim3(21 * 256 / 64), dim3(256), 0, (hipStream_t)stream, partialW, grid,
                     (size_t)21 * 256, 3, 0, 0, 0, dW2);
  return eml::check_launch(DROP ? "eml_dense_conv3x3_bwd_fused_drop_f32(reduce)" : "eml_dense_conv3x3_bwd_fused_f32(reduce)");
#else
  const size_t lds = (size_t)(2 * kHH * kHW * kPSG + kHH * kHW * kPSW + 27 * 3 * 64 + 32) * sizeof(float) + 8 * 48 * 2 * sizeof(double);
  if (a16) {
    EML_ENSURE_LDS((&conv3x3_bwd_fused_kernel<true, DROP>), lds);
    hipLaunchKernelGGL((conv3x3_bwd_fused_kernel<true, DROP>), dim3(grid), dim3(512), lds, (hipStream_t)stream, G, ldg, c0, W2, Z, zmean,
                       zistd, DZ, B, H, W, partials, X, ldx, cx, sB, sC, GF, scale2, shift2, partialW, dk);
  } else {
    EML_ENSURE_LDS((&conv3x3_bwd_fused_kernel<false, DROP>), lds);
    hipLaunchKernelGGL((conv3x3_bwd_fused_kernel<false, DROP>), dim3(grid), dim3(512), lds, (hipStream_t)stream, G, ldg, c0, W2, Z, zmean,
                       zistd, DZ, B, H, W, partials, X, ldx, cx, sB, sC, GF, scale2, shift2, partialW, dk);
  }
  int rc = eml::check_launch(name);
  if (rc) return rc;
  hipLaunchKernelGGL(reduce_rows_kernel, dim3(27 * 256 / 64), dim3(256), 0, (hipStream_t)stream, partialW, 2 * grid,
                     (size_t)27 * 256, 1, 0, 0, 0, dW2);
  return eml::check_launch(DROP ? "eml_dense_conv3x3_bwd_fused_drop_f32(reduce)" : "eml_dense_conv3x3_bwd_fused_f32(reduce)");
#endif
}

extern "C" int eml_dense_conv3x3_bwd_fused_f32(const float* G, int ldg, int c0, const float* W2, const float* Z,
                                               const float* zmean, const float* zistd, float* DZ, int B, int H, int W,
                                               double* partials, int grid, const float* X, int ldx, int cx,
                                               const float* sB, const float* sC, float* GF, const float* scale2,
                                               const float* shift2, float* partialW, float* dW2, eml_stream_t stream) {
  return conv3x3_bwd_fused_launch<false>("eml_dense_conv3x3_bwd_fused_f32", G, ldg, c0, W2, Z, zmean, zistd, DZ, B, H, W, partials,
                                         grid, X, ldx, cx, sB, sC, GF, scale2, shift2, partialW, dW2, eml::DropKey{}, stream);
}

extern "C" int eml_dense_conv3x3_bwd_fused_drop_f32(const float* G, int ldg, int c0, const float* W2, const float* Z,
                                                    const float* zmean, const float* zistd, float* DZ, int B, int H, int W,
                                                    double* partials, int grid, const float* X, int ldx, int cx,
                                                    const float* sB, const float* sC, float* GF, const float* scale2,
                                                    const float* shift2, float* partialW, float* dW2, unsigned long long seed,
                                                    int layer, double p, eml_stream_t stream) {
  if (!(p >= 0.0 && p <= 1.0) || layer < 0)
    return eml::fail(EML_EINVAL, "eml_dense_conv3x3_bwd_fused_drop_f32: p must be in [0, 1] and layer >= 0 (p = %g, layer = %d)", p,
                     layer);
  if ((long long)B * H * W > 0x7FFFFFFFll)
    return eml::fail(EML_EINVAL, "eml_dense_conv3x3_bwd_fused_drop_f32: B*H*W must fit the 32-bit pixel counter");
  return conv3x3_bwd_fused_launch<true>("eml_dense_conv3x3_bwd_fused_drop_f32", G, ldg, c0, W2, Z, zmean, zistd, DZ, B, H, W,
                                        partials, grid, X, ldx, cx, sB, sC, GF, scale2, shift2, partialW, dW2,
                                        eml_drop_key(seed, layer, p), stream);
}

namespace {
__global__ __launch_bounds__(256) void dropout_mask_kernel(eml::DropKey dk, unsigned P, unsigned short* __restrict__ out) {
  for (unsigned q = blockIdx.x * 256u + threadIdx.x; q < P; q += gridDim.x * 256u) {
    unsigned m = 0;
#pragma unroll
    for (unsigned grp = 0; grp < 3; ++grp) {
      const uint4 d = eml::drop_draws(dk, q, grp);
#pragma unroll
      for (int w = 0; w < 4; ++w)
        if ((unsigned long long)eml::draw_word(d, w) >= dk.thr) m |= 1u << (4 * grp + w);
    }
    out[q] = (unsigned short)m;
  }
}
}

extern "C" int eml_dense_dropout_mask_u16(unsigned long long seed, int layer, double p, long P, unsigned short* mask,
                                          eml_stream_t stream) {
  if (!mask || P < 1 || P > 0x7FFFFFFFl || layer < 0 || !(p >= 0.0 && p <= 1.0))
    return eml::fail(EML_EINVAL, "eml_dense_dropout_mask_u16: bad arguments (mask null, P outside [1, 2^31), layer < 0 or p "
                                 "outside [0, 1])");
  const unsigned grid = (unsigned)std::min<long>((P + 255) / 256, 4096);
  hipLaunchKernelGGL(dropout_mask_kernel, dim3(grid), dim3(256), 0, (hipStream_t)stream, eml_drop_key(seed, layer, p), (unsigned)P,
                     mask);
  return eml::check_launch("eml_dense_dropout_mask_u16");
}

extern "C" int eml_dense_bn_bwd_finalize_f32(const double* partials, int R, int pstride, double count,
                                             const float* gamma, const float* mean, const float* istd, int C, int Cpad,
                                             int training, float* dgamma, float* dbeta, float* cA, float* cB,
                                             float* cC, float* sB, float* sC, int s_accumulate, int c_lo,
                                             int c_hi, const float* beta, const float* W, const float* dW, int w_rows,
                                             int* cond, int* any_cond, eml_stream_t stream) {
  if (!partials || !gamma || !mean || !istd || !dgamma || !dbeta || C < 1 || Cpad < C || R < 1 ||
      (cA && (!cB || !cC)) || (sB && !sC) || c_lo < 0 || c_hi <= c_lo)
    return eml::fail(EML_EINVAL, "eml_dense_bn_bwd_finalize_f32: bad arguments");
  if (W && (!dW || !beta || w_rows < 1))
    return eml::fail(EML_EINVAL, "eml_dense_bn_bwd_finalize_f32: W given without dW / beta / w_rows");
  if (c_hi > Cpad) c_hi = Cpad;
  hipLaunchKernelGGL(bn_bwd_finalize_kernel, dim3((c_hi - c_lo + 3) / 4), dim3(256), 0, (hipStream_t)stream, partials,
                     R, pstride, count, gamma, mean, istd, C, Cpad, training, dgamma, dbeta, cA, cB, cC, sB, sC,
                     s_accumulate, c_lo, c_hi, beta, W, dW, w_rows, W ? cond : nullptr, W ? any_cond : nullptr);
  return eml::check_launch("eml_dense_bn_bwd_finalize_f32");
}

extern "C" int eml_dense_bn_dgamma_direct_f32(const float* X, int ldx, long P, int Hin, int Win, int pool, const float* DY,
                                              int ld_dy, const float* Zr, int ld_z, const float* cA, const float* cB,
                                              const float* cC, int Cout, const float* W, int Cin, const float* scale1,
                                              const float* shift1, const float* mean, const float* istd, const int* cond,
                                              double* scratch, float* dgamma, int grid, eml_stream_t stream) {
  if (!X || !DY || !W || !scale1 || !shift1 || !mean || !istd || !cond || !scratch || !dgamma || P < 1 || grid < 1 ||
      Cin < 1 || Cin > 384 || Cout < 1 || Cout > 192 || Cin > ldx || Cout > ld_dy || (Zr && (!cA || !cB || !cC || Cout > ld_z)) ||
      (pool && ((Hin | Win) & 1)))
    return eml::fail(EML_EINVAL, "eml_dense_bn_dgamma_direct_f32: bad arguments (Cin <= 384, Cout <= 192, even maps when pooled)");
  hipLaunchKernelGGL(bn_dgamma_direct_partial_kernel, dim3(grid), dim3(256), 0, (hipStream_t)stream, X, ldx, P, Hin, Win,
                     pool, DY, ld_dy, Zr, ld_z, cA, cB, cC, Cout, W, Cin, scale1, shift1, mean, istd, cond, scratch);
  int rc = eml::check_launch("eml_dense_bn_dgamma_direct_f32(partial)");
  if (rc) return rc;
  hipLaunchKernelGGL(bn_dgamma_direct_reduce_kernel, dim3((Cin + 255) / 256), dim3(256), 0, (hipStream_t)stream, scratch,
                     grid, Cin, cond, dgamma);
  return eml::check_launch("eml_dense_bn_dgamma_direct_f32(reduce)");
}

extern "C" int eml_dense_conv1x1_bwd_weight_f32(const float* X, int ldx, long P, int Hin, int Win, int pool, int Kp,
                                                int Cin, const float* scale1, const float* shift1, const float* DY,
                                                int ld_dy, const float* Zr, int ld_z, const float* cA, const float* cB,
                                                const float* cC, int Cout, float* partial, float* dW, int grid,
                                                float* dz_out, const float* W1, int k_lo, const float* G, int ldg,
                                                float* N12, double* partials_n, eml_stream_t stream) {
  if (dz_out && (Cout != 48 || pool))
    return eml::fail(EML_EINVAL, "eml_dense_conv1x1_bwd_weight_f32: dz_out is for dense layers (Cout == 48, no pool)");
  if (N12 && (Cout != 48 || pool || !W1 || !G || !partials_n || k_lo < 0 || (k_lo & 1) || k_lo + 12 > Cin || (ldg & 1) ||
              (ldg != 12 && k_lo + 12 > ldg)))
    return eml::fail(EML_EINVAL, "eml_dense_conv1x1_bwd_weight_f32: fused narrow pass needs a dense layer, W1, G, partials_n "
                                 "and an even k_lo with k_lo + 12 <= Cin (k_lo=%d, Cin=%d)", k_lo, Cin);
  if (!X || !scale1 || !shift1 || !DY || !Zr || !cA || !cB || !cC || !partial || !dW || P < 1 || grid < 1 || Kp < 32 ||
      (Kp & 15) || Cin > Kp || Cout < 1)
    return eml::fail(EML_EINVAL, "eml_dense_conv1x1_bwd_weight_f32: bad arguments");
  const int nchunks = (Cout + 47) / 48;
  for (int ch = 0; ch < nchunks; ++ch) {
    const int n0 = ch * 48, nv = (Cout - n0 < 48) ? Cout - n0 : 48;
    int n_load = ((ld_dy < ld_z ? ld_dy : ld_z) - n0) & ~3;
    if (n_load > 48) n_load = 48;
    if (n_load < nv) return eml::fail(EML_EINVAL, "eml_dense_conv1x1_bwd_weight_f32: DY/Zr rows narrower than Cout");
    const NarrowArgs na{W1, G, N12, partials_n, Cin, k_lo, ldg};
    static const int vec_env = [] { const char* v = getenv("EML_W1_VEC"); return v ? atoi(v) : 0; }();
    const bool vec4 = !pool && (ldx & 3) == 0 && (reinterpret_cast<uintptr_t>(X) & 15) == 0 &&
                      vec_env == 4;
    if (vec4 && N12 && vec_env == 4)
      hipLaunchKernelGGL((conv1x1_bwd_weight_kernel<false, true, 4>), dim3(grid), dim3(256), 0, (hipStream_t)stream, X, ldx,
                         (int)P, Hin, Win, Kp, scale1, shift1, DY + n0, ld_dy, Zr + n0, ld_z, cA + n0, cB + n0, cC + n0,
                         nv, n_load, partial, dz_out, na);
    else if (vec4 && !N12)
      hipLaunchKernelGGL((conv1x1_bwd_weight_kernel<false, false, 4>), dim3(grid), dim3(256), 0, (hipStream_t)stream, X, ldx,
                         (int)P, Hin, Win, Kp, scale1, shift1, DY + n0, ld_dy, Zr + n0, ld_z, cA + n0, cB + n0, cC + n0,
                         nv, n_load, partial, dz_out, na);
    else if (pool)
      hipLaunchKernelGGL((conv1x1_bwd_weight_kernel<true, false>), dim3(grid), dim3(256), 0, (hipStream_t)stream, X, ldx,
                         (int)P, Hin, Win, Kp, scale1, shift1, DY + n0, ld_dy, Zr + n0, ld_z, cA + n0, cB + n0, cC + n0,
                         nv, n_load, partial, nullptr, na);
    else if (N12)
      hipLaunchKernelGGL((conv1x1_bwd_weight_kernel<false, true>), dim3(grid), dim3(256), 0, (hipStream_t)stream, X, ldx,
                         (int)P, Hin, Win, Kp, scale1, shift1, DY + n0, ld_dy, Zr + n0, ld_z, cA + n0, cB + n0, cC + n0,
                         nv, n_load, partial, dz_out, na);
    else
      hipLaunchKernelGGL((conv1x1_bwd_weight_kernel<false, false>), dim3(grid), dim3(256), 0, (hipStream_t)stream, X, ldx,
                         (int)P, Hin, Win, Kp, scale1, shift1, DY + n0, ld_dy, Zr + n0, ld_z, cA + n0, cB + n0, cC + n0,
                         nv, n_load, partial, dz_out, na);
    int rc = eml::check_launch("eml_dense_conv1x1_bwd_weight_f32");
    if (rc) return rc;
    hipLaunchKernelGGL(reduce_rows_kernel, dim3((Cin * 48 + 63) / 64), dim3(256), 0, (hipStream_t)stream, partial,
                       grid, (size_t)Kp * 48, 0, Cin, nv, n0, dW);
    rc = eml::check_launch("eml_dense_conv1x1_bwd_weight_f32(reduce)");
    if (rc) return rc;
  }
  return EML_OK;
}

extern "C" int eml_dense_permute_w1_bwd_f32(const float* W, int Cout, int Cin, int Kp, int Ko, float* Wd,
                                            eml_stream_t stream) {
  if (!W || !Wd || Cout < 1 || Cin < 1 || Kp < Cin || (Kp & 15) || Ko < Cout || (Ko & 15))
    return eml::fail(EML_EINVAL, "eml_dense_permute_w1_bwd_f32: bad arguments");
  hipLaunchKernelGGL(permute_w1_bwd_kernel, dim3(64), dim3(256), 0, (hipStream_t)stream, W, Cout, Cin, Kp, Ko, Wd);
  return eml::check_launch("eml_dense_permute_w1_bwd_f32");
}

extern "C" int eml_dense_conv1x1_bwd_data_f32(const float* DY, int ld_dy, const float* Zr, int ld_z, const float* cA,
                                              const float* cB, const float* cC, int Ko, const float* Wd,
                                              const float* X, int ldx, const float* scale1, const float* shift1,
                                              const float* mean, const float* istd, long P, int Hin, int Win, int pool,
                                              int Kp, float* G, int ldg, int accumulate, double* partials, int grid,
                                              const unsigned short* relu_mask16, eml_stream_t stream) {
  if (!DY || !Zr || !cA || !cB || !cC || !Wd || (!relu_mask16 && (!X || !mean || !istd)) || !scale1 || !shift1 || !G ||
      !partials || P < 1 || grid < 1 || (Kp & 15) || (Ko & 15) || Ko > ld_dy || Ko > ld_z || (ld_dy & 3) || (ld_z & 3) ||
      (ldx & 3) || (ldg & 3) || (!relu_mask16 && Kp > ldx) || Kp > ldg)
    return eml::fail(EML_EINVAL, "eml_dense_conv1x1_bwd_data_f32: bad arguments");
  if (relu_mask16 && !(pool && Ko != 48))
    return eml::fail(EML_EINVAL, "eml_dense_conv1x1_bwd_data_f32: relu_mask16 is for the transition form (pool, Ko != 48)");
  const size_t lds = (size_t)4 * Kp * 2 * sizeof(double);
#define EML_LAUNCH_BWD_DATA(POOLV, RESV, NCHV)                                                                        \
  hipLaunchKernelGGL((conv1x1_bwd_data_kernel<POOLV, RESV, NCHV>), dim3(grid), dim3(256), lds, (hipStream_t)stream, DY, \
                     ld_dy, Zr, ld_z, cA, cB, cC, Ko, Wd, X, ldx, scale1, shift1, mean, istd, (int)P, Hin, Win, Kp, G, \
                     ldg, accumulate, partials)
  if (pool) {
    if (Ko == 48) {
      EML_LAUNCH_BWD_DATA(true, true, 4);
    } else {
      const size_t lds_t = lds + (size_t)(4 * Kp + 3 * Ko + 4 * 16 * 36) * sizeof(float);
#define EML_LAUNCH_TRANSITION(ACCV, MSKV)                                                                              \
  do {                                                                                                                \
    EML_ENSURE_LDS((&transition_bwd_data_kernel<2, 2, ACCV, MSKV>), lds_t);                                 \
    hipLaunchKernelGGL((transition_bwd_data_kernel<2, 2, ACCV, MSKV>), dim3(grid), dim3(256), lds_t,                   \
                       (hipStream_t)stream, DY, ld_dy, Zr, ld_z, cA, cB, cC, Ko, Wd, X, ldx, scale1, shift1, mean, istd, \
                       (int)P, Hin, Win, Kp, G, ldg, partials, relu_mask16);                                           \
  } while (0)
#define EML_LAUNCH_TRANSITION_RES(NJOV)                                                                                \
  do {                                                                                                                \
    EML_ENSURE_LDS((&transition_bwd_data_kernel<2, 2, false, true, NJOV>), lds_t);                                     \
    hipLaunchKernelGGL((transition_bwd_data_kernel<2, 2, false, true, NJOV>), dim3(grid), dim3(256), lds_t,            \
                       (hipStream_t)stream, DY, ld_dy, Zr, ld_z, cA, cB, cC, Ko, Wd, X, ldx, scale1, shift1, mean, istd, \
                       (int)P, Hin, Win, Kp, G, ldg, partials, relu_mask16);                                           \
  } while (0)
      if (relu_mask16 && !accumulate && Ko == 112) EML_LAUNCH_TRANSITION_RES(7);
      else if (relu_mask16 && !accumulate && Ko == 160) EML_LAUNCH_TRANSITION_RES(10);
      else if (relu_mask16 && !accumulate && Ko == 176) EML_LAUNCH_TRANSITION_RES(11);
      else if (relu_mask16) {
        if (accumulate) EML_LAUNCH_TRANSITION(true, true); else EML_LAUNCH_TRANSITION(false, true);
      } else {
        if (accumulate) EML_LAUNCH_TRANSITION(true, false); else EML_LAUNCH_TRANSITION(false, false);
      }
#undef EML_LAUNCH_TRANSITION
#undef EML_LAUNCH_TRANSITION_RES
    }
  } else {
    if (Ko == 48) EML_LAUNCH_BWD_DATA(false, true, 2); else EML_LAUNCH_BWD_DATA(false, false, 4);
  }
#undef EML_LAUNCH_BWD_DATA
  return eml::check_launch("eml_dense_conv1x1_bwd_data_f32");
}

namespace {
int launch_bwd_data_multi(int n_layers, const float* const* DZ, const float* const* Zr, const float* const* cA,
                          const float* const* cB, const float* const* cC, const float* const* Wd,
                          const float* const* scale1, const float* const* shift1, double* const* partials, const int* Kp,
                          const float* X, int ldx, const float* mean, const float* istd, long P, int k_lo, int k_hi,
                          float* G, int ldg, int grid, const unsigned long long* const* relu_masks, float* top,
                          eml_stream_t stream) {
  if (top && (n_layers != 2 || !relu_masks || Zr || k_lo != 0 || k_hi < 24 || (k_hi & 3) || P * 12 > 2147483647L))
    return eml::fail(EML_EINVAL, "eml_dense_conv1x1_bwd_data_multi_top_f32: the compact top-24 output needs two layers, "
                                 "relu_masks, materialised dz, k_lo == 0 and k_hi >= 24, a multiple of 4 (k_hi=%d)", k_hi);
  if (n_layers < 1 || n_layers > 2 || !DZ || !Wd || !scale1 || !shift1 || !partials ||
      !Kp || (!relu_masks && (!X || !mean || !istd)) || !G || P < 1 || grid < 1 || k_lo < 0 || k_hi <= k_lo ||
      (ldx & 3) || (ldg & 3))
    return eml::fail(EML_EINVAL, "eml_dense_conv1x1_bwd_data_multi_f32: bad arguments");
  const bool raw = Zr == nullptr;
  if (!raw && (!cA || !cB || !cC))
    return eml::fail(EML_EINVAL, "eml_dense_conv1x1_bwd_data_multi_f32: Zr given without cA/cB/cC");
  if (relu_masks && !raw)
    return eml::fail(EML_EINVAL, "eml_dense_conv1x1_bwd_data_multi_f32: relu_masks needs the materialised dz (Zr == NULL)");
  BwdLayer L[2];
  const unsigned long long* Mk[2] = {nullptr, nullptr};
  int kmax = 0;
  for (int j = 0; j < 2; ++j) {
    const int s = j < n_layers ? j : 0;
    const unsigned long long* mk = relu_masks ? relu_masks[s] : nullptr;
    Mk[j] = mk;
    L[j] = raw ? BwdLayer{DZ[s], nullptr, nullptr, nullptr, nullptr, Wd[s], scale1[s], shift1[s], partials[s], Kp[s]}
               : BwdLayer{DZ[s], Zr[s], cA[s], cB[s], cC[s], Wd[s], scale1[s], shift1[s], partials[s], Kp[s]};
    if (!DZ[s] || (!raw && !Zr[s]) || !Wd[s] || !partials[s] || (relu_masks && !mk) || (Kp[s] & 15) ||
        (!relu_masks && Kp[s] > ldx) || Kp[s] > ldg)
      return eml::fail(EML_EINVAL, "eml_dense_conv1x1_bwd_data_multi_f32: bad layer %d", s);
    if (Kp[s] > kmax) kmax = Kp[s];
  }
  if (((k_hi + 15) & ~15) > kmax) return eml::fail(EML_EINVAL, "eml_dense_conv1x1_bwd_data_multi_f32: range beyond Kp");
  const size_t lds = (size_t)n_layers * 4 * kmax * 2 * sizeof(double) + (size_t)(2 + 2 * n_layers) * kmax * sizeof(float);
  if (lds > 80 * 1024) return eml::fail(EML_EINVAL, "eml_dense_conv1x1_bwd_data_multi_f32: Kp=%d does not fit LDS", kmax);
#define EML_LAUNCH_MULTI(NLV, MTV, RAWV, MSKV)                                                                       \
  do {                                                                                                              \
    EML_ENSURE_LDS((&conv1x1_bwd_data_multi_kernel<NLV, MTV, RAWV, MSKV>), lds);                                 \
    hipLaunchKernelGGL((conv1x1_bwd_data_multi_kernel<NLV, MTV, RAWV, MSKV>), dim3(grid), dim3(256), lds,            \
                       (hipStream_t)stream, L[0], L[1], X, ldx, mean, istd, (int)P, k_lo, k_hi, G, ldg, kmax,        \
                       Mk[0], Mk[1], (float*)nullptr);                                                              \
  } while (0)
  if (n_layers == 1) {
    if (relu_masks) EML_LAUNCH_MULTI(1, 4, true, true);
    else if (raw) EML_LAUNCH_MULTI(1, 4, true, false);
    else EML_LAUNCH_MULTI(1, 4, false, false);
  } else if (top) {
    EML_ENSURE_LDS((&conv1x1_bwd_data_multi_kernel<2, 2, true, true, true>), lds);
    hipLaunchKernelGGL((conv1x1_bwd_data_multi_kernel<2, 2, true, true, true>), dim3(grid), dim3(256), lds,
                       (hipStream_t)stream, L[0], L[1], X, ldx, mean, istd, (int)P, k_lo, k_hi, G, ldg, kmax, Mk[0], Mk[1],
                       top);
  } else {
    if (relu_masks) EML_LAUNCH_MULTI(2, 2, true, true);
    else if (raw) EML_LAUNCH_MULTI(2, 2, true, false);
    else EML_LAUNCH_MULTI(2, 2, false, false);
  }
#undef EML_LAUNCH_MULTI
  return eml::check_launch("eml_dense_conv1x1_bwd_data_multi_f32");
}
}

extern "C" int eml_dense_conv1x1_bwd_data_multi_f32(int n_layers, const float* const* DZ, const float* const* Zr,
                                                    const float* const* cA, const float* const* cB,
                                                    const float* const* cC, const float* const* Wd,
                                                    const float* const* scale1, const float* const* shift1,
                                                    double* const* partials, const int* Kp, const float* X, int ldx,
                                                    const float* mean, const float* istd, long P, int k_lo, int k_hi,
                                                    float* G, int ldg, int grid,
                                                    const unsigned long long* const* relu_masks, eml_stream_t stream) {
  return launch_bwd_data_multi(n_layers, DZ, Zr, cA, cB, cC, Wd, scale1, shift1, partials, Kp, X, ldx, mean, istd, P, k_lo,
                               k_hi, G, ldg, grid, relu_masks, nullptr, stream);
}

extern "C" int eml_dense_conv1x1_bwd_data_multi_top_f32(const float* const* DZ, const float* const* Wd,
                                                        const float* const* scale1, const float* const* shift1,
                                                        double* const* partials, const int* Kp, long P, int k_hi,
                                                        float* G, int ldg, int grid,
                                                        const unsigned long long* const* relu_masks, float* top,
                                                        eml_stream_t stream) {
  if (!top) return eml::fail(EML_EINVAL, "eml_dense_conv1x1_bwd_data_multi_top_f32: top is NULL");
  return launch_bwd_data_multi(2, DZ, nullptr, nullptr, nullptr, nullptr, Wd, scale1, shift1, partials, Kp, nullptr, 0,
                               nullptr, nullptr, P, 0, k_hi, G, ldg, grid, relu_masks, top, stream);
}

extern "C" int eml_dense_conv1x1_bwd_narrow_f32(const float* DZ, const float* W1, int Cin, int k_lo, const float* X,
                                                int ldx, const float* scale1, const float* shift1, const float* mean,
                                                const float* istd, long P, const float* G, int ldg, float* N12,
                                                double* partials, int Kp, int grid, eml_stream_t stream) {
  if (!DZ || !W1 || !X || !scale1 || !shift1 || !mean || !istd || !G || !N12 || !partials || P < 1 || grid < 1 ||
      k_lo < 0 || (k_lo & 1) || k_lo + 12 > Cin || Cin > Kp || (ldx & 1) || (ldg & 1) || Kp > ldx || Kp > ldg)
    return eml::fail(EML_EINVAL, "eml_dense_conv1x1_bwd_narrow_f32: bad arguments");
  hipLaunchKernelGGL((conv1x1_bwd_narrow_kernel<4>), dim3(grid), dim3(256), 0, (hipStream_t)stream, DZ, W1, Cin, k_lo, X,
                     ldx, scale1, shift1, mean, istd, (int)P, G, ldg, N12, partials, Kp);
  return eml::check_launch("eml_dense_conv1x1_bwd_narrow_f32");
}

extern "C" int eml_dense_grad_materialize_f32(float* G, int ldg, const float* X, int ldx, const float* sB,
                                              const float* sC, int c0, int n, long P, eml_stream_t stream) {
  if (!G || !X || !sB || !sC || P < 1 || n < 2 || (n & 1) || (c0 & 1) || (ldg & 1) || (ldx & 1))
    return eml::fail(EML_EINVAL, "eml_dense_grad_materialize_f32: bad arguments");
  const size_t total = (size_t)P * (n >> 1);
  const int grid = (int)((total + 255) / 256 < 8192 ? (total + 255) / 256 : 8192);
  hipLaunchKernelGGL(grad_materialize_kernel, dim3(grid), dim3(256), 0, (hipStream_t)stream, G, ldg, X, ldx, sB, sC, c0,
                     n, (size_t)P);
  return eml::check_launch("eml_dense_grad_materialize_f32");
}

extern "C" int eml_dense_bn_bwd_stats_f32(const float* DY, int ld_dy, const float* raw, int ld_raw, const float* out,
                                          int ld_out, int relu, int C, long P, const float* mean, const float* istd,
                                          double* partials, int grid, eml_stream_t stream) {
  if (!DY || !raw || !mean || !istd || !partials || (relu && !out) || C < 1 || C > 384 || P < 1 || grid < 1)
    return eml::fail(EML_EINVAL, "eml_dense_bn_bwd_stats_f32: bad arguments");
  auto a16 = [](const void* q) { return (reinterpret_cast<size_t>(q) & 15) == 0; };
  if (C <= 32 && (C & 3) == 0 && ((ld_dy | ld_raw | (relu ? ld_out : 0)) & 3) == 0 && a16(DY) && a16(raw) && (!relu || a16(out)) &&
      a16(mean) && a16(istd)) {
    hipLaunchKernelGGL(bn_bwd_stats_small_kernel, dim3(grid), dim3(256), 0, (hipStream_t)stream, DY, ld_dy, raw, ld_raw, out, ld_out,
                       relu, C, (size_t)P, mean, istd, partials);
    return eml::check_launch("eml_dense_bn_bwd_stats_f32");
  }
  const size_t lds = (size_t)4 * ((C + 63) / 64) * 64 * 2 * sizeof(double);
  hipLaunchKernelGGL(bn_bwd_stats_kernel, dim3(grid), dim3(256), lds, (hipStream_t)stream, DY, ld_dy, raw, ld_raw, out,
                     ld_out, relu, C, (size_t)P, mean, istd, partials);
  return eml::check_launch("eml_dense_bn_bwd_stats_f32");
}

extern "C" int eml_dense_conv0_bwd_weight_f32(const float* x, const float* G, int ldg, const float* X1, int ldx,
                                              const float* Y0, int C0, const float* cA, const float* cB,
                                              const float* cC, int B, int H, int W, float* partial, float* dW0,
                                              int grid, eml_stream_t stream) {
  if (!x || !G || !X1 || !Y0 || !cA || !cB || !cC || !partial || !dW0 || C0 < 1 || C0 > 32 || B < 1 || grid < 1)
    return eml::fail(EML_EINVAL, "eml_dense_conv0_bwd_weight_f32: bad arguments");
  hipLaunchKernelGGL(conv0_bwd_weight_kernel<false>, dim3(grid), dim3(256), 0, (hipStream_t)stream, x, G, ldg, X1, ldx, Y0, C0,
                     cA, cB, cC, B, H, W, partial, nullptr, nullptr, nullptr, nullptr);
  int rc = eml::check_launch("eml_dense_conv0_bwd_weight_f32");
  if (rc) return rc;
  hipLaunchKernelGGL(reduce_rows_kernel, dim3(27 * 32 / 64 + 1), dim3(256), 0, (hipStream_t)stream, partial, grid * 4,
                     (size_t)1024, 2, 0, C0, 0, dW0);
  return eml::check_launch("eml_dense_conv0_bwd_weight_f32(reduce)");
}

extern "C" int eml_dense_head_pool_bwd_f32(const float* gpooled, const float* F, int ldf, int C, int B, int H, int W,
                                           int k, float* dF, int ldd, eml_stream_t stream) {
  if (!gpooled || !F || !dF || C < 1 || B < 1 || k < 1) return eml::fail(EML_EINVAL, "eml_dense_head_pool_bwd_f32: bad arguments");
  const size_t total = (size_t)B * H * W * C;
  const int grid = (int)((total + 255) / 256 < 4096 ? (total + 255) / 256 : 4096);
  hipLaunchKernelGGL(head_pool_bwd_kernel, dim3(grid), dim3(256), 0, (hipStream_t)stream, gpooled, F, ldf, C, B, H, W, k,
                     dF, ldd);
  return eml::check_launch("eml_dense_head_pool_bwd_f32");
}

extern "C" int eml_dense_norm0_bwd_stats_f32(const float* G, int ldg, const float* Y0, int ld_y0, const float* scale0,
                                             const float* shift0, const float* sB, const float* sC, int C, long P,
                                             const float* mean, const float* istd, double* partials, int grid,
                                             eml_stream_t stream) {
  auto a16 = [](const void* q) { return (reinterpret_cast<size_t>(q) & 15) == 0; };
  if (!G || !Y0 || !scale0 || !shift0 || !sB || !sC || !mean || !istd || !partials || C < 4 || C > 32 || (C & 3) || P < 1 ||
      grid < 1 || ((ldg | ld_y0) & 3) || !a16(G) || !a16(Y0) || !a16(scale0) || !a16(shift0) || !a16(sB) || !a16(sC) || !a16(mean) ||
      !a16(istd))
    return eml::fail(EML_EINVAL, "eml_dense_norm0_bwd_stats_f32: bad arguments (C a multiple of 4 <= 32, 16-byte aligned operands)");
  hipLaunchKernelGGL(norm0_bwd_stats_kernel, dim3(grid), dim3(256), 0, (hipStream_t)stream, G, ldg, Y0, ld_y0, scale0, shift0, sB,
                     sC, C, (size_t)P, mean, istd, partials);
  return eml::check_launch("eml_dense_norm0_bwd_stats_f32");
}

extern "C" int eml_dense_conv0_bwd_weight_fused_f32(const float* x, const float* G, int ldg, const float* Y0, int C0,
                                                    const float* scale0, const float* shift0, const float* sB, const float* sC,
                                                    const float* cA, const float* cB, const float* cC, int B, int H, int W,
                                                    float* partial, float* dW0, int grid, eml_stream_t stream) {
  if (!x || !G || !Y0 || !scale0 || !shift0 || !sB || !sC || !cA || !cB || !cC || !partial || !dW0 || C0 < 1 || C0 > 32 || B < 1 ||
      grid < 1)
    return eml::fail(EML_EINVAL, "eml_dense_conv0_bwd_weight_fused_f32: bad arguments");
  hipLaunchKernelGGL(conv0_bwd_weight_kernel<true>, dim3(grid), dim3(256), 0, (hipStream_t)stream, x, G, ldg, nullptr, 0, Y0, C0, cA,
                     cB, cC, B, H, W, partial, scale0, shift0, sB, sC);
  int rc = eml::check_launch("eml_dense_conv0_bwd_weight_fused_f32");
  if (rc) return rc;
  hipLaunchKernelGGL(reduce_rows_kernel, dim3(27 * 32 / 64 + 1), dim3(256), 0, (hipStream_t)stream, partial, grid * 4,
                     (size_t)1024, 2, 0, C0, 0, dW0);
  return eml::check_launch("eml_dense_conv0_bwd_weight_fused_f32(reduce)");
}

extern "C" int eml_dense_conv0_bwd_data_f32(const float* G, int ldg, const float* X1, int ldx, const float* Y0, int C0,
                                            const float* scale0, const float* shift0, const float* sB, const float* sC,
                                            const float* cA, const float* cB, const float* cC, const float* W0, int B, int H,
                                            int W, float* dX, eml_stream_t stream) {
  auto a16 = [](const void* q) { return (reinterpret_cast<size_t>(q) & 15) == 0; };
  const bool fused = X1 == nullptr;
  if (!G || !Y0 || !cA || !cB || !cC || !W0 || !dX || (fused && (!scale0 || !shift0 || !sB || !sC)))
    return eml::fail(EML_EINVAL, "eml_dense_conv0_bwd_data_f32: null pointer");
  if (C0 != kC0dC || B < 1 || H < 1 || W < 1 || ldg < C0 || (ldg & 3) || (!fused && (ldx < C0 || (ldx & 3))))
    return eml::fail(EML_EINVAL, "eml_dense_conv0_bwd_data_f32: bad shape (C0 == 24, B, H, W >= 1, ldg / ldx >= 24 and multiples of 4)");
  if (!a16(G) || !a16(Y0) || (!fused && !a16(X1)) || !a16(cA) || !a16(cB) || !a16(cC) ||
      (fused && (!a16(scale0) || !a16(shift0) || !a16(sB) || !a16(sC))))
    return eml::fail(EML_EINVAL, "eml_dense_conv0_bwd_data_f32: G, X1, Y0 and the coefficient vectors must be 16-byte aligned");
  const size_t tiles = (size_t)B * ((H + kC0dTH - 1) / kC0dTH) * ((W + kC0dTW - 1) / kC0dTW);
  if (tiles > 0x7fffffff) return eml::fail(EML_EINVAL, "eml_dense_conv0_bwd_data_f32: more than 2^31 - 1 tiles of 8 x 32 pixels");
  const int grid = (int)tiles;
  if (fused)
    hipLaunchKernelGGL(conv0_bwd_data_kernel<true>, dim3(grid), dim3(256), 0, (hipStream_t)stream, G, ldg, nullptr, 0, Y0,
                       scale0, shift0, sB, sC, cA, cB, cC, W0, B, H, W, dX);
  else
    hipLaunchKernelGGL(conv0_bwd_data_kernel<false>, dim3(grid), dim3(256), 0, (hipStream_t)stream, G, ldg, X1, ldx, Y0,
                       nullptr, nullptr, nullptr, nullptr, cA, cB, cC, W0, B, H, W, dX);
  return eml::check_launch("eml_dense_conv0_bwd_data_f32");
}
```

### include/emlight_hip.h

```cpp
#ifndef EMLIGHT_HIP_H
#define EMLIGHT_HIP_H

#include <stddef.h>
#include <stdint.h>

#ifdef __cplusplus
extern "C" {
#endif

typedef void* eml_stream_t;

#define EML_OK 0
#define EML_EINVAL (-1)
#define EML_ELAUNCH (-2)

#define EML_MAX_EPS 64

#define EML_ABI_VERSION 31
int eml_abi_version(void);
const char* eml_last_error(void);

int eml_sg_rasterise_f32(const float* dirs, const float* sizes, const float* colors,
                         float* out, int B, int N, int H, int W, eml_stream_t stream);

// ... 5 lines not shown
int eml_sg_rasterise_bwd_colors_f32(const float* dirs, const float* sizes, const float* gout,
                                    float* gcolors, int B, int N, int H, int W,
                                    eml_stream_t stream);
size_t eml_sg_rasterise_bwd_work_floats(int B, int N, int H, int W);
int eml_sg_rasterise_bwd_colors_ex_f32(const float* dirs, const float* sizes, const float* gout, float* gcolors, float* work,
                                       int B, int N, int H, int W, int flags, eml_stream_t stream);
size_t eml_sg_rasterise_bwd_full_work_floats(int B, int N, int H, int W);
int eml_sg_rasterise_bwd_f32(const float* dirs, const float* sizes, const float* colors, const float* gout, float* gdirs,
                             float* gsizes, float* gcolors, float* work, int B, int N, int H, int W, int flags,
                             eml_stream_t stream);

int eml_emd_anchor_cost_f32(const float* anchors, float* M, int N, eml_stream_t stream);

int eml_sinkhorn_schedule_f32(const float* x, const float* y, long n, double blur,
                              double scaling, int p, double diameter, const float* range_lo_hi,
                              float* eps_out, int* n_eps_out, float* diameter_out, eml_stream_t stream);

size_t eml_sinkhorn_work_floats(int B, int N);
int eml_sinkhorn_fwd_f32(const float* x, const float* y, const float* M, const float* Mt,
                         const float* alpha, const float* beta, double blur, double scaling, int p,
                         double diameter, const float* range_lo_hi, float* eps_out, int* n_eps_out,
                         float* diameter_out, float* loss, float* gx, float* gy, float* work, int B, int N,
                         eml_stream_t stream);

#define EML_SINKHORN_NO_SPLIT 1
#define EML_SINKHORN_FORCE_SPLIT 2
#define EML_SINKHORN_TEST_STALL 4
int eml_sinkhorn_fwd_ex_f32(const float* x, const float* y, const float* M, const float* Mt,
                            const float* alpha, const float* beta, double blur, double scaling, int p,
                            double diameter, const float* range_lo_hi, float* eps_out, int* n_eps_out,
                            float* diameter_out, float* loss, float* gx, float* gy, float* work, int B, int N,
                            int flags, eml_stream_t stream);

int eml_sinkhorn_fwd_rho_f32(const float* x, const float* y, const float* M, const float* Mt,
                             const float* alpha, const float* beta, double blur, double scaling, int p,
                             double diameter, const float* range_lo_hi, float* eps_out, int* n_eps_out,
                             float* diameter_out, float* loss, float* gx, float* gy, float* work, int B, int N,
                             int flags, double rho, float* lam_out, eml_stream_t stream);

int eml_sinkhorn_bwd_f32(const float* gloss, const float* gunit, float* gout, int B, int N,
                         eml_stream_t stream);



int eml_dense_conv0_fwd_f32(const float* x, const float* w0, float* X, int ldx, int B, int H, int W,
                            int C0, double* partials, int grid, eml_stream_t stream);
int eml_dense_conv0_fwd_mfma_f32(const float* x, const float* w0, float* X, int ldx, int B, int H, int W,
                                 int C0, double* partials, int grid, eml_stream_t stream);

int eml_dense_bn_apply_f32(const float* src, int ld_src, float* dst, int ld_dst, int C, long P,
                           const float* scale, const float* shift, int relu, double* partials,
                           int grid, eml_stream_t stream);

int eml_dense_bn_prepare_f32(const double* partials, int G, int pstride, int n_new, int c_new0,
                             double count, float* mean, float* var, float* istd, const float* gamma,
                             const float* beta, float* rmean, float* rvar, int C, int Cpad, float eps,
                             float momentum, int training, float* scale, float* shift,
                             eml_stream_t stream);

int eml_dense_permute_w1_f32(const float* W, int Cout, int Cin, int Kp, float* Wp, eml_stream_t stream);
int eml_dense_permute_w2_f32(const float* W2, int Cout, float* W2p, eml_stream_t stream);

typedef struct eml_permute_desc {
  const float* src;
  float* dst;
  int kind, Cout, Cin, Kp, Ko, reserved;
} eml_permute_desc;
int eml_dense_permute_batch_f32(const eml_permute_desc* descs, int n, eml_stream_t stream);

int eml_dense_conv1x1_fwd_f32(const float* X, int ldx, long P, int Hin, int Win, int pool, int Kp,
                              const float* scale, const float* shift, const float* Wp, int Cout,
                              float* out, int ldo, double* partials, int grid,
                              unsigned long long* relu_mask, eml_stream_t stream);

int eml_dense_conv3x3_fwd_f32(const float* Z, const float* scale2, const float* shift2,
                              const float* W2p, float* X, int ldx, int c_out0, int B, int H, int W,
                              double* partials, int grid, eml_stream_t stream);

int eml_dense_permute_w2_tp_f32(const float* W2, float* W2t, eml_stream_t stream);
int eml_dense_conv3x3_fwd_tp_supported(int B, int H, int W);
int eml_dense_conv3x3_fwd_tp_f32(const float* Z, const float* scale2, const float* shift2,
                                 const float* W2t, float* X, int ldx, int c_out0, int B, int H, int W,
                                 int band_rows, double* partials, int grid, eml_stream_t stream);

int eml_dense_conv3x3_fwd_drop_f32(const float* Z, const float* scale2, const float* shift2,
                                   const float* W2p, float* X, int ldx, int c_out0, int B, int H, int W,
                                   double* partials, int grid, unsigned long long seed, int layer, double p,
                                   eml_stream_t stream);
int eml_dense_conv3x3_fwd_tp_drop_f32(const float* Z, const float* scale2, const float* shift2,
                                      const float* W2t, float* X, int ldx, int c_out0, int B, int H, int W,
                                      int band_rows, double* partials, int grid, unsigned long long seed, int layer,
                                      double p, eml_stream_t stream);
int eml_dense_dropout_mask_u16(unsigned long long seed, int layer, double p, long P, unsigned short* mask,
                               eml_stream_t stream);

int eml_dense_pool_act_f32(const float* X, int ldx, int B, int Hin, int Win, int Kp, const float* scale,
                           const float* shift, float* A, int lda, unsigned short* relu_mask16,
                           eml_stream_t stream);

int eml_dense_head_pool_fwd_f32(const float* F, int ldf, int C, int B, int H, int W, int k,
                                float* out, eml_stream_t stream);


int eml_dense_conv3x3_bwd_data_f32(const float* G, int ldg, int c0, const float* W2, const float* Z,
                                   const float* zmean, const float* zistd, float* DZ, int B, int H,
                                   int W, double* partials, int grid, const float* X, int ldx, int cx,
                                   const float* sB, const float* sC, float* GF, eml_stream_t stream);

int eml_dense_conv3x3_bwd_fused_supported(int ldg, int c0, int ldx, int cx);
int eml_dense_conv3x3_bwd_fused_f32(const float* G, int ldg, int c0, const float* W2, const float* Z,
                                    const float* zmean, const float* zistd, float* DZ, int B, int H, int W,
                                    double* partials, int grid, const float* X, int ldx, int cx,
                                    const float* sB, const float* sC, float* GF, const float* scale2,
                                    const float* shift2, float* partialW, float* dW2, eml_stream_t stream);

int eml_dense_conv3x3_bwd_data_drop_f32(const float* G, int ldg, int c0, const float* W2, const float* Z,
                                        const float* zmean, const float* zistd, float* DZ, int B, int H,
                                        int W, double* partials, int grid, const float* X, int ldx, int cx,
                                        const float* sB, const float* sC, float* GF, unsigned long long seed,
                                        int layer, double p, eml_stream_t stream);
int eml_dense_conv3x3_bwd_fused_drop_f32(const float* G, int ldg, int c0, const float* W2, const float* Z,
                                         const float* zmean, const float* zistd, float* DZ, int B, int H, int W,
                                         double* partials, int grid, const float* X, int ldx, int cx,
                                         const float* sB, const float* sC, float* GF, const float* scale2,
                                         const float* shift2, float* partialW, float* dW2, unsigned long long seed,
                                         int layer, double p, eml_stream_t stream);

int eml_dense_conv3x3_bwd_weight_f32(const float* G, int ldg, int c0, const float* Z,
                                     const float* scale2, const float* shift2, int B, int H, int W,
                                     float* partial, float* dW2, int grid, eml_stream_t stream);

int eml_dense_bn_bwd_finalize_f32(const double* partials, int R, int pstride, double count,
                                  const float* gamma, const float* mean, const float* istd, int C,
                                  int Cpad, int training, float* dgamma, float* dbeta, float* cA,
                                  float* cB, float* cC, float* sB, float* sC, int s_accumulate,
                                  int c_lo, int c_hi, const float* beta, const float* W, const float* dW,
                                  int w_rows, int* cond, int* any_cond, eml_stream_t stream);

int eml_dense_bn_dgamma_direct_f32(const float* X, int ldx, long P, int Hin, int Win, int pool,
                                   const float* DY, int ld_dy, const float* Zr, int ld_z, const float* cA,
                                   const float* cB, const float* cC, int Cout, const float* W, int Cin,
                                   const float* scale1, const float* shift1, const float* mean,
                                   const float* istd, const int* cond, double* scratch, float* dgamma,
                                   int grid, eml_stream_t stream);

int eml_dense_conv1x1_bwd_weight_f32(const float* X, int ldx, long P, int Hin, int Win, int pool,
                                     int Kp, int Cin, const float* scale1, const float* shift1,
                                     const float* DY, int ld_dy, const float* Zr, int ld_z,
                                     const float* cA, const float* cB, const float* cC, int Cout,
                                     float* partial, float* dW, int grid, float* dz_out,
                                     const float* W1, int k_lo, const float* G, int ldg, float* N12,
                                     double* partials_n, eml_stream_t stream);

int eml_dense_permute_w1_bwd_f32(const float* W, int Cout, int Cin, int Kp, int Ko, float* Wd,
                                 eml_stream_t stream);

int eml_dense_conv1x1_bwd_data_f32(const float* DY, int ld_dy, const float* Zr, int ld_z,
                                   const float* cA, const float* cB, const float* cC, int Ko,
                                   const float* Wd, const float* X, int ldx, const float* scale1,
                                   const float* shift1, const float* mean, const float* istd, long P,
                                   int Hin, int Win, int pool, int Kp, float* G, int ldg,
                                   int accumulate, double* partials, int grid,
                                   const unsigned short* relu_mask16, eml_stream_t stream);

int eml_dense_conv1x1_bwd_data_multi_f32(int n_layers, const float* const* DZ, const float* const* Zr,
                                         const float* const* cA, const float* const* cB,
                                         const float* const* cC, const float* const* Wd,
                                         const float* const* scale1, const float* const* shift1,
                                         double* const* partials, const int* Kp, const float* X, int ldx,
                                         const float* mean, const float* istd, long P, int k_lo,
                                         int k_hi, float* G, int ldg, int grid,
                                         const unsigned long long* const* relu_masks, eml_stream_t stream);

int eml_dense_conv1x1_bwd_data_multi_top_f32(const float* const* DZ, const float* const* Wd,
                                             const float* const* scale1, const float* const* shift1,
                                             double* const* partials, const int* Kp, long P, int k_hi, float* G,
                                             int ldg, int grid, const unsigned long long* const* relu_masks,
                                             float* top, eml_stream_t stream);

int eml_dense_conv1x1_bwd_narrow_f32(const float* DZ, const float* W1, int Cin, int k_lo, const float* X,
                                     int ldx, const float* scale1, const float* shift1,
                                     const float* mean, const float* istd, long P, const float* G, int ldg,
                                     float* N12, double* partials, int Kp, int grid, eml_stream_t stream);

int eml_dense_grad_materialize_f32(float* G, int ldg, const float* X, int ldx, const float* sB,
                                   const float* sC, int c0, int n, long P, eml_stream_t stream);

int eml_dense_bn_bwd_stats_f32(const float* DY, int ld_dy, const float* raw, int ld_raw,
                               const float* out, int ld_out, int relu, int C, long P,
                               const float* mean, const float* istd, double* partials, int grid,
                               eml_stream_t stream);

int eml_dense_conv0_bwd_weight_f32(const float* x, const float* G, int ldg, const float* X1, int ldx,
                                   const float* Y0, int C0, const float* cA, const float* cB,
                                   const float* cC, int B, int H, int W, float* partial, float* dW0,
                                   int grid, eml_stream_t stream);

int eml_dense_norm0_bwd_stats_f32(const float* G, int ldg, const float* Y0, int ld_y0, const float* scale0,
                                  const float* shift0, const float* sB, const float* sC, int C, long P,
                                  const float* mean, const float* istd, double* partials, int grid, eml_stream_t stream);
int eml_dense_conv0_bwd_weight_fused_f32(const float* x, const float* G, int ldg, const float* Y0, int C0,
                                         const float* scale0, const float* shift0, const float* sB, const float* sC,
                                         const float* cA, const float* cB, const float* cC, int B, int H, int W,
                                         float* partial, float* dW0, int grid, eml_stream_t stream);

int eml_dense_conv0_bwd_data_f32(const float* G, int ldg, const float* X1, int ldx, const float* Y0, int C0,
                                 const float* scale0, const float* shift0, const float* sB, const float* sC,
                                 const float* cA, const float* cB, const float* cC, const float* W0, int B, int H, int W,
                                 float* dX, eml_stream_t stream);

int eml_dense_head_pool_bwd_f32(const float* gpooled, const float* F, int ldf, int C, int B, int H,
                                int W, int k, float* dF, int ldd, eml_stream_t stream);


int eml_sphere_tap_table_f32(const float* grid, int H, int W, int Ho, int Wo, int* idx, float* wgt,
                             eml_stream_t stream);

int eml_sphere_im2col_f32(const float* X, const int* idx, const float* wgt, float* A9, int B, int HW,
                          int Po, int C, eml_stream_t stream);

int eml_sphere_col2im_f32(const float* dA9, const int* ptr, const int* src, const float* w, float* dX,
                          int B, int HW, int Po, int C, eml_stream_t stream);

int eml_sphere_conv_fwd_fused_f32(const float* X, const int* idx, const float* wgt, const float* W2,
                                  const float* bias, float* Y, int B, int HW, int Po, int C, int O, int ke,
                                  eml_stream_t stream);
#define EML_TAP_ROWSHARE 1
int eml_sphere_conv_fwd_fused_ex_f32(const float* X, const int* idx, const float* wgt, const float* W2,
                                     const float* bias, float* Y, int B, int HW, int Po, int C, int O, int ke,
                                     const float* residual, float act_slope, int table_flags, eml_stream_t stream);
int eml_sphere_conv_small_supported(int C, int O);
int eml_sphere_conv_small_fwd_f32(const float* X, const int* idx, const float* wgt, const float* W2, const float* bias,
                                  float* Y, int B, int HW, int Po, int C, int O, float act_slope, eml_stream_t stream);
size_t eml_sphere_conv_small_wgrad_partial_floats(int B, int Po, int C, int O);
int eml_sphere_conv_small_wgrad_f32(const float* X, const int* idx, const float* wgt, const float* dY, const float* Yact,
                                    float act_slope, float* partial, float* dW2, float* db, int B, int HW, int Po, int C,
                                    int O, eml_stream_t stream);
int eml_sphere_conv_small_da9_f32(const float* dY, const float* Yact, float act_slope, const float* W2, float* dA9, long M,
                                  int C, int O, eml_stream_t stream);
int eml_sphere_conv_narrow_supported(int C, int O);
int eml_sphere_conv_narrow_fwd_f32(const float* X, const int* idx, const float* wgt, const float* W2, const float* bias, float* Y,
                                   int B, int HW, int Po, int C, int O, eml_stream_t stream);
int eml_sphere_conv_narrow_dgrad_f32(const float* dY, const int* tidx, const float* twgt, int ke, const float* W2, float* dX, int B,
                                     int HW, int Po, int C, int O, eml_stream_t stream);
size_t eml_sphere_conv_narrow_wgrad_partial_floats(int B, int Po, int C, int O);
int eml_sphere_conv_narrow_wgrad_f32(const float* X, const int* idx, const float* wgt, const float* dY, float* partial, float* dW2,
                                     int B, int HW, int Po, int C, int O, eml_stream_t stream);

size_t eml_sphere_conv_narrow_scratch_floats(int B, int HW);
int eml_sphere_conv_narrow_fwd2_f32(const float* X, const int* idx, const float* wgt, const float* W2, const float* bias,
                                    float* Y, float* scratch, int B, int HW, int Po, int C, int O, eml_stream_t stream);
size_t eml_sphere_conv_narrow_wgrad2_partial_floats(int B, int HW, int C);
int eml_sphere_conv_narrow_wgrad2_f32(const float* X, const int* tidx, const float* twgt, int ke,
                                      const unsigned char* rowmax, const float* dY, float* scratch, float* partial, float* dW2, int B, int HW, int Po, int C, int O,
                                      eml_stream_t stream);
int eml_sphere_conv_narrow_dgrad2_f32(const float* dY, const int* tidx, const float* twgt, int ke,
                                      const unsigned char* rowmax, const float* W2, float* dX, float* scratch,
                                      int scratch_has_v, int B, int HW, int Po, int C, int O, eml_stream_t stream);
int eml_sphere_conv_dgrad_fused_f32(const float* dY, const int* tidx, const float* twgt, const unsigned char* rowmax,
                                    int ke, const float* W2t, float* dX, int B, int HW, int Po, int C, int O,
                                    int table_flags, eml_stream_t stream);
int eml_sphere_conv_lowres_variant(int C, int O, int Po, int fp_max);
int eml_sphere_conv_lowres_table_i32(const int* idx, const int* fp, int* lidx, int Po, int ke, eml_stream_t stream);
size_t eml_sphere_conv_lowres_partial_floats(long M, int O, int split);
int eml_sphere_conv_lowres_f32(const float* X, const int* lidx, const float* wgt, const unsigned char* rowmax, int ke,
                               const int* fp, int fp_max, const float* W2, const float* bias, float* Y, float* partial,
                               int split, int B, int HW, int Po, int C, int O, const float* residual, float act_slope,
                               eml_stream_t stream);
size_t eml_sphere_conv_wgrad_partial_floats(int C, int O, int split_k);
int eml_sphere_conv_wgrad_fused_f32(const float* X, const int* idx, const float* wgt, const float* dY,
                                    float* partial, float* dW2, int B, int HW, int Po, int C, int O,
                                    int split_k, eml_stream_t stream);

int eml_spade_modulate_fwd_f32(const float* xn, int ld_x, const float* gb, int ld_gb, float* y, int ld_y,
                               long rows, int C, float slope, eml_stream_t stream);
int eml_spade_modulate_bwd_f32(const float* gy, int ld_gy, const float* xn, int ld_x, const float* gb,
                               int ld_gb, float* dxn, int ld_dx, float* dgb, int ld_dgb, long rows, int C,
                               float slope, eml_stream_t stream);

int eml_bn_stats_f32(const float* x, int ld, long rows, int C, double* partials, int grid, eml_stream_t stream);
int eml_bn_fold_f64(const double* partials, int R, int n, double* sums, eml_stream_t stream);
int eml_bn_finalize_f32(const double* sums, int C, float eps, float momentum, float* mean, float* istd,
                        float* running_mean, float* running_var, eml_stream_t stream);
int eml_spade_norm_modulate_fwd_f32(const float* x, int ld_x, const float* gb, int ld_gb, float* y, int ld_y,
                                    long rows, int C, float slope, const float* mean, const float* istd,
                                    eml_stream_t stream);
int eml_bn_bwd_apply_f32(const float* dxn, int ld_d, const float* x, int ld_x, long rows, int C,
                         const float* mean, const float* istd, const double* sums, float* dx, int ld_o,
                         eml_stream_t stream);

int eml_spade_norm_modulate_up2_fwd_f32(const float* x_lo, const float* gb, float* y, int B, int H, int W, int C, float slope,
                                        const float* mean, const float* istd, eml_stream_t stream);
int eml_bn_bwd_apply_up2_f32(const float* dxn, const float* x_lo, int B, int H, int W, int C, const float* mean,
                             const float* istd, const double* sums, float* dx_lo, eml_stream_t stream);

int eml_spade_norm_modulate_bwd_cols_f32(const float* gy, const float* x, const float* gb, float* dxn, float* dgb, int B, int H,
                                         int W, int C, int up2, float slope, const float* mean, const float* istd,
                                         double* partials, int grid, eml_stream_t stream);

int eml_sphere_conv_spade_supported(int Cin, int Cn, long HW);
int eml_sphere_conv_spade_fwd_f32(const float* actv, const int* idx, const float* wgt, const float* W2r, const float* bias_r,
                                  const float* x, const float* mean, const float* istd, float* Y, float* gamma_out, int B, int H,
                                  int W, int Cin, int Cn, int up2, float act_slope, int table_flags, eml_stream_t stream);
int eml_spade_norm_modulate_bwd_y_f32(const float* gy, const float* x, const float* gamma, const float* y, float* dxn, float* dgb,
                                      int B, int H, int W, int C, int up2, float slope, const float* mean, const float* istd,
                                      double* partials, int grid, eml_stream_t stream);

size_t eml_spectral_norm_scratch_floats(int O, int C);
int eml_spectral_norm_w2_f32(const float* W, float* u, float* v, int iterate, float eps, float* W2, float* sigma,
                             float* uv_used, float* scratch, int O, int C, eml_stream_t stream);
int eml_spectral_norm_w2_bwd_f32(const float* dW2, const float* W2, const float* u_used, const float* v_used,
                                 const float* sigma, double* partial, float* dW, int O, int C, eml_stream_t stream);
int eml_spectral_norm_w2_batch_f32(int n, const float* const* W, float* const* u, float* const* v, int iterate, float eps,
                                   float* const* W2, float* const* sigma, float* const* uv_used, float* const* scratch,
                                   const int* O, const int* C, eml_stream_t stream);

int eml_spade_heads_w2_f32(const float* Wg, const float* Wb, const float* bg, const float* bb, float* W2, float* b2, int Cn,
                           int C, int reorder, eml_stream_t stream);

int eml_instance_norm_act_fwd_f32(const float* x, float* y, float* stats, int B, int HW, int C, int channels_last,
                                  float eps, float slope, eml_stream_t stream);
int eml_instance_norm_act_bwd_f32(const float* gy, const float* x, const float* stats, float* dx, int B, int HW, int C,
                                  int channels_last, float slope, eml_stream_t stream);

size_t eml_l1_pairs_partial_doubles(int npairs);
int eml_l1_pairs_fwd_f32(int npairs, const float* const* f, const float* const* r, const float* const* w, const long* rows,
                         const int* C, const float* scale, double* partial, float* out, eml_stream_t stream);
int eml_l1_pairs_bwd_f32(int npairs, const float* const* f, const float* const* r, const float* const* w, const long* rows,
                         const int* C, const float* scale, const float* gout, float* const* g, float* const* gzero,
                         const long* nzero, eml_stream_t stream);

// ... 13 lines not shown
```

Baseline: 567.1 images/s.

## Group dense-layer backward into triples with shared data-gradient pass and 24-channel narrow epilogue

```diff
diff --git a/emlight_amd/RegressionNetwork/dense_engine_bwd.py b/emlight_amd/RegressionNetwork/dense_engine_bwd.py
--- a/emlight_amd/RegressionNetwork/dense_engine_bwd.py
+++ b/emlight_amd/RegressionNetwork/dense_engine_bwd.py
@@ -44,17 +44,20 @@
         self.G = [torch.zeros(blk["P"], blk["ld"], **f32) for blk in ws.blocks]
         self.GF = torch.zeros(ws.F.shape[0], ws.F.shape[1], **f32)
         maxP = ws.blocks[0]["P"]
-        self.DZ = torch.empty(2, maxP, 48, **f32)
+        self.triple = knob_flag("EML_DGRAD_TRIPLE", True)
+        ng = 3 if self.triple else 2
+        self.DZ = torch.empty(ng, maxP, 48, **f32)
         self.ring = max(1, int(os.environ.get("EML_WGRAD_RING", 4))) if enc.overlap_wgrad(dev) else 1
         self.GF12 = [torch.empty(maxP, 12, **f32) for _ in range(self.ring)]
         self.N12 = torch.empty(maxP, 12, **f32)
-        self.TOP = torch.empty(2 * maxP * 12, **f32) if knob_flag("EML_DGRAD_TOP", True) else None
+        self.N12lo = torch.empty(maxP, 12, **f32) if self.triple else None
+        self.TOP = torch.empty(ng * maxP * 12, **f32) if knob_flag("EML_DGRAD_TOP", True) else None
         kp, ko, g = enc.kp_max, max(enc.ko_max, 48), enc.grid_max
         self.Wd = [[torch.empty(lay["Kp"] * 48, **f32) for lay in blk["layers"]] for blk in ws.blocks]
         self.WdT = [torch.empty(blk["trans"]["Kp"] * blk["trans"]["Ko"], **f32) for blk in ws.blocks]
         self.permutes = None
-        self.coef = torch.zeros(8, max(kp, ko), **f32)
-        self.part2 = torch.zeros(2, g * kp * 2, dtype=torch.float64, device=dev)
+        self.coef = torch.zeros(3 * ng + 2, max(kp, ko), **f32)
+        self.part2 = torch.zeros(ng, g * kp * 2, dtype=torch.float64, device=dev)
         self.partW = torch.empty(g * max(kp * 48, 2 * 27 * 256, 4 * 1024), **f32)
         i32 = dict(dtype=torch.int32, device=dev)
         self.cond = [[torch.zeros(lay["Kp"], **i32) for lay in blk["layers"]] for blk in ws.blocks]
@@ -136,9 +139,10 @@
         slot = grad_slot(q) if need else None
         grads[id(q)] = slot if slot is not None else torch.empty_like(q)
     gr = lambda q: p(grads[id(q)])
-    coefs = [tuple(bw.coef[3 * k + i] for i in range(3)) for k in range(2)]
+    ng = bw.part2.shape[0]
+    coefs = [tuple(bw.coef[3 * k + i] for i in range(3)) for k in range(ng)]
     cA, cB, cC = coefs[0]
-    sB, sC = bw.coef[6], bw.coef[7]
+    sB, sC = bw.coef[3 * ng], bw.coef[3 * ng + 1]
 
     direct = knob_choice("EML_DGAMMA_DIRECT", "always", ("always", "never")) != "never"
     c3_fold = knob_flag("EML_C3_FOLD", True)
@@ -186,7 +190,10 @@
         Pn = B * (Hb // 2) * (Wb // 2)
         Gbuf = bw.G[bi]
         gl0 = sum(enc.block_layers[:bi])
-        top2 = bw.TOP[:2 * P * 12].view(2, P, 12) if bw.TOP is not None else None
+        use3 = (bw.triple and P >= Gd * 128 and len(blk["layers"]) >= 3
+                and all(y["mask"] is not None for y in blk["layers"]))
+        ntop = 3 if use3 else 2
+        top2 = bw.TOP[:ntop * P * 12].view(ntop, P, 12) if bw.TOP is not None else None
         _lib.check(L.eml_dense_bn_bwd_stats_f32(p(dY), ld_dy, p(tr["T"]), Ko, None, 0, 0, cout, Pn, p(tr["tmean"]),
                                                 p(tr["tistd"]), p(part), Gb, st), "eml_dense_bn_bwd_stats_f32")
         finalize(Gb, 2 * cout, Pn, LN, tr["tmean"], tr["tistd"], cout, Ko, coef=0)
@@ -202,11 +209,11 @@
                  cond=bw.condT[bi])
         dgamma_direct(blk, ld, P, Hb, Wb, 1, dY, ld_dy, tr["T"], Ko, coefs[0], cout, T.conv, ctot, tr["scale"], tr["shift"],
                       bw.condT[bi], T.norm)
-        def conv2_backward(l, slot, n12=False, narrow_lo=None, top=False):
+        def conv2_backward(l, slot, n12=False, narrow_lo=None, top=False, n24=False, nsrc=None):
             lay = blk["layers"][l]
             Lm = getattr(mod, "denselayer%d" % (l + 1))
             cin, kp, z, dz = lay["Cin"], lay["Kp"], blk["Z"][l], bw.DZ[slot]
-            gsrc = (p(bw.N12), 12, 0) if n12 else (p(top2[1]), 12, 0) if top else (p(Gbuf), ld, cin)
+            gsrc = (p(bw.N12), 12, 0) if n12 else (p(top2[-1]), 12, 0) if top else (p(Gbuf), ld, cin)
             r = ring[0] = (ring[0] + 1) % bw.ring
             if bw.side is not None and bw.ev_done[r] is not None:
                 main.wait_event(bw.ev_done[r])
@@ -242,16 +249,32 @@
                 bw.ev_done[r].record(bw.side)
             finalize(G3d, 96, P, Lm.norm2, lay["zmean"], lay["zistd"], 48, 48, coef=slot)
             a, b, c = coefs[slot]
+            if n24:
+                gn = (p(top2[0]), p(top2[1]), 12) if top else (p(Gbuf), p(Gbuf), ld)
+                _lib.check(L.eml_dense_conv1x1_bwd_weight_n24_f32(
+                    p(blk["X"]), ld, P, Hb, Wb, kp, cin, p(lay["scale1"]), p(lay["shift1"]), p(dz), 48, p(z), 48,
+                    p(a), p(b), p(c), p(bw.partW), gr(Lm.conv1.weight), Gw, p(dz), p(Lm.conv1.weight), narrow_lo, *gn,
+                    p(bw.N12lo), p(bw.N12), p(bw.part2[slot]), st), "eml_dense_conv1x1_bwd_weight_n24_f32")
+                return Lm
+            if nsrc is None:
+                nsrc = (p(top2[0]), 12) if top else (p(Gbuf), ld)
             _lib.check(L.eml_dense_conv1x1_bwd_weight_f32(
                 p(blk["X"]), ld, P, Hb, Wb, 0, kp, cin, p(lay["scale1"]), p(lay["shift1"]), p(dz), 48, p(z), 48,
                 p(a), p(b), p(c), 48, p(bw.partW), gr(Lm.conv1.weight), Gw, p(dz),
-                *((p(Lm.conv1.weight), narrow_lo, *((p(top2[0]), 12) if top else (p(Gbuf), ld)), p(bw.N12),
-                   p(bw.part2[slot])) if narrow_lo is not None
+                *((p(Lm.conv1.weight), narrow_lo, *nsrc, p(bw.N12), p(bw.part2[slot])) if narrow_lo is not None
                   else (None, 0, None, 0, None, None)), st), "eml_dense_conv1x1_bwd_weight_f32")
             return Lm
 
         def dgrad(layers, slots, k_lo, k_hi, top=False):
             lays = [blk["layers"][l] for l in layers]
+            if len(layers) == 3:
+                _lib.check(L.eml_dense_conv1x1_bwd_data_masked_f32(
+                    3, parr([bw.DZ[s_] for s_ in slots]), parr([bw.Wd[bi][l_] for l_ in layers]),
+                    parr([y["scale1"] for y in lays]), parr([y["shift1"] for y in lays]),
+                    parr([bw.part2[s_] for s_ in slots]), (ctypes.c_int * 3)(*[y["Kp"] for y in lays]),
+                    P, k_lo, k_hi, p(Gbuf), ld, Gd, parr([y["mask"] for y in lays]), p(top2) if top else None, st),
+                    "eml_dense_conv1x1_bwd_data_masked_f32")
+                return
             if top:
                 _lib.check(L.eml_dense_conv1x1_bwd_data_multi_top_f32(
                     parr([bw.DZ[s_] for s_ in slots]), parr([bw.Wd[bi][l_] for l_ in layers]),
@@ -282,7 +305,25 @@
         l = len(blk["layers"]) - 1
         have_top = False
         while l >= 0:
-            if l >= 1:
+            if use3 and l >= 2:
+                lt, lm, lb = l, l - 1, l - 2
+                cin_t, cin_m, cin_b = (blk["layers"][j]["Cin"] for j in (lt, lm, lb))
+                Lmt = conv2_backward(lt, 0, narrow_lo=cin_b, top=have_top, n24=True)
+                bn1_finalize(lt, Lmt, 0, cin_b, cin_t, rows=Gw)
+                Lmm = conv2_backward(lm, 1, n12=True, narrow_lo=cin_b, nsrc=(p(bw.N12lo), 12))
+                bn1_finalize(lm, Lmm, 1, cin_b, cin_m, rows=Gw)
+                Lmb = conv2_backward(lb, 2, n12=True)
+                to_top = top2 is not None and lb >= 3 and bw.side is None and cin_b >= 36 and cin_b % 4 == 0
+                dgrad([lt, lm, lb], [0, 1, 2], 0, cin_b, top=to_top)
+                have_top = to_top
+                bn1_finalize(lt, Lmt, 0, 0, cin_b)
+                bn1_finalize(lm, Lmm, 1, 0, cin_b)
+                bn1_finalize(lb, Lmb, 2, 0, blk["layers"][lb]["Kp"])
+                bn1_direct(lt, Lmt, 0)
+                bn1_direct(lm, Lmm, 1)
+                bn1_direct(lb, Lmb, 2)
+                l -= 3
+            elif l >= 1:
                 la, lb = l, l - 1
                 cin_a, cin_b = blk["layers"][la]["Cin"], blk["layers"][lb]["Cin"]
                 Lma = conv2_backward(la, 0, narrow_lo=cin_b, top=have_top)
diff --git a/emlight_amd/_lib.py b/emlight_amd/_lib.py
--- a/emlight_amd/_lib.py
+++ b/emlight_amd/_lib.py
@@ -164,6 +164,10 @@
     "eml_dense_conv1x1_bwd_weight_f32": (_int, [_f32p, _int, ctypes.c_long, _int, _int, _int, _int, _int, _f32p,
                                                 _f32p, _f32p, _int, _f32p, _int, _f32p, _f32p, _f32p, _int, _f32p,
                                                 _f32p, _int, _f32p, _f32p, _int, _f32p, _int, _f32p, _f32p, _stream]),
+    "eml_dense_conv1x1_bwd_weight_n24_f32": (_int, [_f32p, _int, ctypes.c_long, _int, _int, _int, _int, _f32p, _f32p,
+                                                    _f32p, _int, _f32p, _int, _f32p, _f32p, _f32p, _f32p, _f32p, _int,
+                                                    _f32p, _f32p, _int, _f32p, _f32p, _int, _f32p, _f32p, _f32p,
+                                                    _stream]),
     "eml_dense_conv1x1_bwd_narrow_f32": (_int, [_f32p, _f32p, _int, _int, _f32p, _int, _f32p, _f32p, _f32p, _f32p,
                                                 ctypes.c_long, _f32p, _int, _f32p, _f32p, _int, _int, _stream]),
     "eml_dense_permute_w1_bwd_f32": (_int, [_f32p, _int, _int, _int, _int, _f32p, _stream]),
@@ -175,6 +179,8 @@
                                                     _stream]),
     "eml_dense_conv1x1_bwd_data_multi_top_f32": (_int, [ctypes.c_void_p] * 6 + [ctypes.c_long, _int, _f32p, _int, _int,
                                                         ctypes.c_void_p, _f32p, _stream]),
+    "eml_dense_conv1x1_bwd_data_masked_f32": (_int, [_int] + [ctypes.c_void_p] * 6 + [ctypes.c_long, _int, _int, _f32p,
+                                                     _int, _int, ctypes.c_void_p, _f32p, _stream]),
     "eml_dense_grad_materialize_f32": (_int, [_f32p, _int, _f32p, _int, _f32p, _f32p, _int, _int, ctypes.c_long,
                                               _stream]),
     "eml_dense_bn_bwd_stats_f32": (_int, [_f32p, _int, _f32p, _int, _f32p, _int, _int, _int, ctypes.c_long, _f32p,
diff --git a/emlight_amd/csrc/dense_bwd.hip b/emlight_amd/csrc/dense_bwd.hip
--- a/emlight_amd/csrc/dense_bwd.hip
+++ b/emlight_amd/csrc/dense_bwd.hip
@@ -1167,8 +1167,10 @@
   float* N12;
   double* partials;
   int Cin, k_lo, ldg;
+  const float* G2;
+  float* N12lo;
 };
-template <bool POOL, bool NARROW = false, int VEC = 2>
+template <bool POOL, bool NARROW = false, int VEC = 2, bool N24 = false>
 __global__ __launch_bounds__(256, (NARROW || VEC == 4) ? 2 : 1) void conv1x1_bwd_weight_kernel(
     const float* __restrict__ X, int ldx, int P, int Hin, int Win, int Kp, const float* __restrict__ scale1,
     const float* __restrict__ shift1, const float* __restrict__ DY, int ld_dy, const float* __restrict__ Zr,
@@ -1184,15 +1186,25 @@
   constexpr int GW = 16 * VEC;
   constexpr int MAXG = VEC == 2 ? 3 : 2;
   const int ngroups = (Kp + GW - 1) / GW;
-  float nsk[4] = {0.f, 0.f, 0.f, 0.f}, ntk[4] = {0.f, 0.f, 0.f, 0.f};
-  double ns1[4] = {0.0, 0.0, 0.0, 0.0};
+  static_assert(!N24 || (NARROW && VEC == 2 && !POOL), "the 24-channel narrow pass is an epilogue of the dense-layer form");
+  constexpr int NSET = N24 ? 2 : 1;
+  float nsk[NSET][4], ntk[NSET][4];
+  double ns1[NSET][4];
   const int kq = min(kk, 2);
-  if constexpr (NARROW) {
+  __shared__ float naff_l[N24 ? 48 : 1];
+  __shared__ double ns1_l[N24 ? 2 * 4 * 256 : 1];
+#pragma unroll
+  for (int s = 0; s < NSET; ++s)
 #pragma unroll
     for (int g = 0; g < 4; ++g) {
-      nsk[g] = kk < 3 ? scale1[na.k_lo + 4 * kq + g] : 0.f;
-      ntk[g] = kk < 3 ? shift1[na.k_lo + 4 * kq + g] : 0.f;
-    }
+      nsk[s][g] = (NARROW && !N24 && kk < 3) ? scale1[na.k_lo + 12 * s + 4 * kq + g] : 0.f;
+      ntk[s][g] = (NARROW && !N24 && kk < 3) ? shift1[na.k_lo + 12 * s + 4 * kq + g] : 0.f;
+      ns1[s][g] = 0.0;
+    }
+  if constexpr (N24) {
+    if (tid < 48) naff_l[tid] = tid < 24 ? scale1[na.k_lo + tid] : shift1[na.k_lo + tid - 24];
+#pragma unroll
+    for (int e = 0; e < 8; ++e) ns1_l[e * 256 + tid] = 0.0;
   }
 
   float sv[MAXG][VEC], tv[MAXG][VEC];
@@ -1212,7 +1224,7 @@
   }
   const int spix = tid >> 2, sq = tid & 3;
   __shared__ __attribute__((aligned(16))) float co_l[3 * 48];
-  __shared__ float wn_l[NARROW ? 12 * 64 : 1];
+  __shared__ float wn_l[NARROW ? NSET * 12 * 64 : 1];
   constexpr bool CO_LDS = NARROW || VEC == 4;
   float4 sa_r[CO_LDS ? 1 : 3], sb_r[CO_LDS ? 1 : 3], sc_r[CO_LDS ? 1 : 3];
   if constexpr (CO_LDS) {
@@ -1240,9 +1252,9 @@
     }
   }
   if constexpr (NARROW) {
-    for (int e = tid; e < 12 * 64; e += 256) {
-      const int st = e >> 6, l = e & 63, rr = l & 15, k4 = l >> 4;
-      wn_l[e] = rr < 12 ? na.W1[(size_t)(4 * st + k4) * na.Cin + na.k_lo + rr] : 0.f;
+    for (int e = tid; e < NSET * 12 * 64; e += 256) {
+      const int st = (e >> 6) % 12, l = e & 63, rr = l & 15, k4 = l >> 4, cs = 12 * (e / (12 * 64));
+      wn_l[e] = rr < 12 ? na.W1[(size_t)(4 * st + k4) * na.Cin + na.k_lo + cs + rr] : 0.f;
     }
   }
   __syncthreads();
@@ -1341,16 +1353,20 @@
     for (int chunk = blockIdx.x; chunk < nchunks; chunk += gridDim.x, ++it) {
       const float* dzb = dz_l[it & 1];
       stage_load(chunk + gridDim.x);
-      float2 nx[2], ng[2];
+      float2 nx[NSET][2], ng[NSET][2];
       const int pn = chunk * 64 + 16 * wave + r;
       if constexpr (NARROW) {
         const size_t pc = (size_t)min(pn, P - 1);
-        const float* xs = X + pc * ldx + na.k_lo + 4 * kq;
-        const float* gs = na.G + pc * na.ldg + (na.ldg == 12 ? 0 : na.k_lo) + 4 * kq;
-        nx[0] = *reinterpret_cast<const float2*>(xs);
-        nx[1] = *reinterpret_cast<const float2*>(xs + 2);
-        ng[0] = *reinterpret_cast<const float2*>(gs);
-        ng[1] = *reinterpret_cast<const float2*>(gs + 2);
+#pragma unroll
+        for (int s = 0; s < NSET; ++s) {
+          const int kb = na.k_lo + 12 * s;
+          const float* xs = X + pc * ldx + kb + 4 * kq;
+          const float* gs = (s == 1 ? na.G2 : na.G) + pc * na.ldg + (na.ldg == 12 ? 0 : kb) + 4 * kq;
+          nx[s][0] = *reinterpret_cast<const float2*>(xs);
+          nx[s][1] = *reinterpret_cast<const float2*>(xs + 2);
+          ng[s][0] = *reinterpret_cast<const float2*>(gs);
+          ng[s][1] = *reinterpret_cast<const float2*>(gs + 2);
+        }
       }
       if constexpr (NGW > 0) {
         float bzq[2][3];
@@ -1405,20 +1421,34 @@
         }
       }
       if constexpr (NARROW) {
-        asm volatile("" ::"v"(ng[0].x), "v"(ng[0].y), "v"(ng[1].x), "v"(ng[1].y), "v"(nx[0].x), "v"(nx[0].y), "v"(nx[1].x), "v"(nx[1].y));
-        f32x4 an = f32x4{0.f, 0.f, 0.f, 0.f};
-#pragma unroll
-        for (int st = 0; st < 12; ++st) an = mfma16(wn_l[st * 64 + lane], dzb[(16 * wave + r) * 48 + 4 * st + kk], an);
+#pragma unroll
+        for (int s = 0; s < NSET; ++s)
+          asm volatile("" ::"v"(ng[s][0].x), "v"(ng[s][0].y), "v"(ng[s][1].x), "v"(ng[s][1].y), "v"(nx[s][0].x), "v"(nx[s][0].y),
+                       "v"(nx[s][1].x), "v"(nx[s][1].y));
         const bool nv = pn < P && kk < 3;
-        const float xg[4] = {nx[0].x, nx[0].y, nx[1].x, nx[1].y}, gg[4] = {ng[0].x, ng[0].y, ng[1].x, ng[1].y};
-        float o4[4];
-#pragma unroll
-        for (int g = 0; g < 4; ++g) {
-          const float dam = (nv && fmaf(xg[g], nsk[g], ntk[g]) > 0.f) ? an[g] : 0.f;
-          o4[g] = fmaf(nsk[g], dam, gg[g]);
-          ns1[g] += (double)dam;
-        }
-        if (nv) *reinterpret_cast<float4*>(na.N12 + ((unsigned)pn * 12u + 4u * (unsigned)kk)) = make_float4(o4[0], o4[1], o4[2], o4[3]);
+#pragma unroll
+        for (int s = 0; s < NSET; ++s) {
+          f32x4 an = f32x4{0.f, 0.f, 0.f, 0.f};
+#pragma unroll
+          for (int st = 0; st < 12; ++st)
+            an = mfma16(wn_l[s * 12 * 64 + st * 64 + lane], dzb[(16 * wave + r) * 48 + 4 * st + kk], an);
+          const float xg[4] = {nx[s][0].x, nx[s][0].y, nx[s][1].x, nx[s][1].y};
+          const float gg[4] = {ng[s][0].x, ng[s][0].y, ng[s][1].x, ng[s][1].y};
+          float o4[4];
+#pragma unroll
+          for (int g = 0; g < 4; ++g) {
+            const float sk = N24 ? naff_l[12 * s + 4 * kq + g] : nsk[s][g];
+            const float tk = N24 ? naff_l[24 + 12 * s + 4 * kq + g] : ntk[s][g];
+            const float dam = (nv && fmaf(xg[g], sk, tk) > 0.f) ? an[g] : 0.f;
+            o4[g] = fmaf(sk, dam, gg[g]);
+            if constexpr (N24)
+              ns1_l[(s * 4 + g) * 256 + tid] += (double)dam;
+            else
+              ns1[s][g] += (double)dam;
+          }
+          float* out = (N24 && s == 0) ? na.N12lo : na.N12;
+          if (nv) *reinterpret_cast<float4*>(out + ((unsigned)pn * 12u + 4u * (unsigned)kk)) = make_float4(o4[0], o4[1], o4[2], o4[3]);
+        }
       }
       stage_write(dz_l[(it + 1) & 1]);
       eml::lds_barrier();
@@ -1447,17 +1477,26 @@
   }
   if constexpr (NARROW) {
     __syncthreads();
+    constexpr int NC = 12 * NSET;
     double* red = reinterpret_cast<double*>(&dz_l[0][0]);
-#pragma unroll
-    for (int g = 0; g < 4; ++g) {
-#pragma unroll
-      for (int o = 1; o < 16; o <<= 1) ns1[g] += shfl_xor_d(ns1[g], o);
-      if (r == 0 && kk < 3) red[wave * 12 + 4 * kk + g] = ns1[g];
-    }
+    if constexpr (N24) {
+#pragma unroll
+      for (int s = 0; s < NSET; ++s)
+#pragma unroll
+        for (int g = 0; g < 4; ++g) ns1[s][g] = ns1_l[(s * 4 + g) * 256 + tid];
+    }
+#pragma unroll
+    for (int s = 0; s < NSET; ++s)
+#pragma unroll
+      for (int g = 0; g < 4; ++g) {
+#pragma unroll
+        for (int o = 1; o < 16; o <<= 1) ns1[s][g] += shfl_xor_d(ns1[s][g], o);
+        if (r == 0 && kk < 3) red[wave * NC + 12 * s + 4 * kk + g] = ns1[s][g];
+      }
     __syncthreads();
-    if (tid < 12) {
+    if (tid < NC) {
       double* dst = na.partials + ((size_t)blockIdx.x * Kp + na.k_lo + tid) * 2;
-      dst[0] = (red[tid] + red[12 + tid]) + (red[24 + tid] + red[36 + tid]);
+      dst[0] = (red[tid] + red[NC + tid]) + (red[2 * NC + tid] + red[3 * NC + tid]);
       dst[1] = 0.0;
     }
   }
@@ -1896,7 +1935,7 @@
 
 template <int NL, int MT , bool RAW = false ,
           bool MASKED = false, bool TOP = false>
-__global__ __launch_bounds__(256, 2) void conv1x1_bwd_data_multi_kernel(BwdLayer L0, BwdLayer L1,
+__global__ __launch_bounds__(256, 2) void conv1x1_bwd_data_multi_kernel(BwdLayer L0, BwdLayer L1, BwdLayer L2,
                                                                         const float* __restrict__ X, int ldx,
                                                                         const float* __restrict__ mean,
                                                                         const float* __restrict__ istd, int P,
@@ -1904,13 +1943,15 @@
                                                                         int ldg, int KpMax,
                                                                         const unsigned long long* __restrict__ M0,
                                                                         const unsigned long long* __restrict__ M1,
+                                                                        const unsigned long long* __restrict__ M2,
                                                                         float* __restrict__ Top) {
   extern __shared__ __attribute__((aligned(16))) float smem[];
   double* sacc = reinterpret_cast<double*>(smem);
   float* vec_l = reinterpret_cast<float*>(sacc + (size_t)NL * 4 * KpMax * 2);
   const int tid = threadIdx.x, lane = tid & 63, wave = tid >> 6;
   const int r = lane & 15, kk = lane >> 4;
-  const BwdLayer Ls[2] = {L0, L1};
+  static_assert(NL >= 1 && NL <= 3, "1, 2 or 3 layers per pass");
+  const BwdLayer Ls[3] = {L0, L1, L2};
   for (int e = tid; e < NL * 4 * KpMax * 2; e += 256) sacc[e] = 0.0;
   for (int e = tid; e < KpMax; e += 256) {
     vec_l[e] = MASKED ? 0.f : mean[e];
@@ -1995,7 +2036,7 @@
         const int nnt = Ls[j].Kp >> 4;
         unsigned long long mk[MT][NCH][4];
         if constexpr (MASKED) {
-          const unsigned long long* __restrict__ Mj = j == 0 ? M0 : M1;
+          const unsigned long long* __restrict__ Mj = j == 0 ? M0 : j == 1 ? M1 : M2;
 #pragma unroll
           for (int m = 0; m < MT; ++m)
 #pragma unroll
@@ -2006,7 +2047,7 @@
               for (int g = 0; g < 4; ++g) mk[m][n][g] = Mj[wi + g];
             }
         }
-        const int cur = NL == 2 ? j : wsel;
+        const int cur = NL == 1 ? wsel : (j & 1);
         if (j + 1 < NL)
           load_w(j + 1, nt0, wq[cur ^ 1]);
         else
@@ -2086,6 +2127,12 @@
           }
         }
       }
+      if constexpr (NL == 3) {
+#pragma unroll
+        for (int jo = 0; jo < 3; ++jo)
+#pragma unroll
+          for (int n = 0; n < NCH; ++n) wq[0][jo][n] = wq[1][jo][n];
+      }
 #pragma unroll
       for (int n = 0; n < NCH; ++n) {
         const int nt = nt0 + n;
@@ -2093,8 +2140,9 @@
           const int k4 = 16 * nt + 4 * kk;
           const bool act = k4 + 3 >= k_lo && k4 < k_hi;
           if constexpr (TOP) {
-            const int t = k4 - (k_hi - 24);
-            float* cdst = Top + (t >= 12 ? (size_t)P * 12 + (t - 12) : (size_t)max(t, 0));
+            const int t = k4 - (k_hi - 12 * NL);
+            const int q = t >= 24 ? 2 : t >= 12 ? 1 : 0;
+            float* cdst = Top + (size_t)q * P * 12 + max(t - 12 * q, 0);
 #pragma unroll
             for (int m = 0; m < MT; ++m) {
               float* dst = t >= 0 ? cdst + prow[m] * 12 : Gd + prow[m] * ldg + k4;
@@ -2930,12 +2978,12 @@
   return eml::check_launch("eml_dense_bn_dgamma_direct_f32(reduce)");
 }
 
-extern "C" int eml_dense_conv1x1_bwd_weight_f32(const float* X, int ldx, long P, int Hin, int Win, int pool, int Kp,
-                                                int Cin, const float* scale1, const float* shift1, const float* DY,
-                                                int ld_dy, const float* Zr, int ld_z, const float* cA, const float* cB,
-                                                const float* cC, int Cout, float* partial, float* dW, int grid,
-                                                float* dz_out, const float* W1, int k_lo, const float* G, int ldg,
-                                                float* N12, double* partials_n, eml_stream_t stream) {
+namespace {
+int launch_bwd_weight(const float* X, int ldx, long P, int Hin, int Win, int pool, int Kp, int Cin, const float* scale1,
+                      const float* shift1, const float* DY, int ld_dy, const float* Zr, int ld_z, const float* cA,
+                      const float* cB, const float* cC, int Cout, float* partial, float* dW, int grid, float* dz_out,
+                      const float* W1, int k_lo, const float* G, int ldg, float* N12, double* partials_n, const float* G2,
+                      float* N12lo, eml_stream_t stream) {
   if (dz_out && (Cout != 48 || pool))
     return eml::fail(EML_EINVAL, "eml_dense_conv1x1_bwd_weight_f32: dz_out is for dense layers (Cout == 48, no pool)");
   if (N12 && (Cout != 48 || pool || !W1 || !G || !partials_n || k_lo < 0 || (k_lo & 1) || k_lo + 12 > Cin || (ldg & 1) ||
@@ -2951,11 +2999,11 @@
     int n_load = ((ld_dy < ld_z ? ld_dy : ld_z) - n0) & ~3;
     if (n_load > 48) n_load = 48;
     if (n_load < nv) return eml::fail(EML_EINVAL, "eml_dense_conv1x1_bwd_weight_f32: DY/Zr rows narrower than Cout");
-    const NarrowArgs na{W1, G, N12, partials_n, Cin, k_lo, ldg};
+    const NarrowArgs na{W1, G, N12, partials_n, Cin, k_lo, ldg, G2, N12lo};
     static const int vec_env = [] { const char* v = getenv("EML_W1_VEC"); return v ? atoi(v) : 0; }();
     const bool vec4 = !pool && (ldx & 3) == 0 && (reinterpret_cast<uintptr_t>(X) & 15) == 0 &&
                       vec_env == 4;
-    if (vec4 && N12 && vec_env == 4)
+    if (vec4 && N12 && !N12lo && vec_env == 4)
       hipLaunchKernelGGL((conv1x1_bwd_weight_kernel<false, true, 4>), dim3(grid), dim3(256), 0, (hipStream_t)stream, X, ldx,
                          (int)P, Hin, Win, Kp, scale1, shift1, DY + n0, ld_dy, Zr + n0, ld_z, cA + n0, cB + n0, cC + n0,
                          nv, n_load, partial, dz_out, na);
@@ -2967,6 +3015,10 @@
       hipLaunchKernelGGL((conv1x1_bwd_weight_kernel<true, false>), dim3(grid), dim3(256), 0, (hipStream_t)stream, X, ldx,
                          (int)P, Hin, Win, Kp, scale1, shift1, DY + n0, ld_dy, Zr + n0, ld_z, cA + n0, cB + n0, cC + n0,
                          nv, n_load, partial, nullptr, na);
+    else if (N12 && na.N12lo)
+      hipLaunchKernelGGL((conv1x1_bwd_weight_kernel<false, true, 2, true>), dim3(grid), dim3(256), 0, (hipStream_t)stream, X,
+                         ldx, (int)P, Hin, Win, Kp, scale1, shift1, DY + n0, ld_dy, Zr + n0, ld_z, cA + n0, cB + n0, cC + n0,
+                         nv, n_load, partial, dz_out, na);
     else if (N12)
       hipLaunchKernelGGL((conv1x1_bwd_weight_kernel<false, true>), dim3(grid), dim3(256), 0, (hipStream_t)stream, X, ldx,
                          (int)P, Hin, Win, Kp, scale1, shift1, DY + n0, ld_dy, Zr + n0, ld_z, cA + n0, cB + n0, cC + n0,
@@ -2983,6 +3035,31 @@
     if (rc) return rc;
   }
   return EML_OK;
+}
+}
+
+extern "C" int eml_dense_conv1x1_bwd_weight_f32(const float* X, int ldx, long P, int Hin, int Win, int pool, int Kp,
+                                                int Cin, const float* scale1, const float* shift1, const float* DY,
+                                                int ld_dy, const float* Zr, int ld_z, const float* cA, const float* cB,
+                                                const float* cC, int Cout, float* partial, float* dW, int grid,
+                                                float* dz_out, const float* W1, int k_lo, const float* G, int ldg,
+                                                float* N12, double* partials_n, eml_stream_t stream) {
+  return launch_bwd_weight(X, ldx, P, Hin, Win, pool, Kp, Cin, scale1, shift1, DY, ld_dy, Zr, ld_z, cA, cB, cC, Cout,
+                           partial, dW, grid, dz_out, W1, k_lo, G, ldg, N12, partials_n, nullptr, nullptr, stream);
+}
+
+extern "C" int eml_dense_conv1x1_bwd_weight_n24_f32(const float* X, int ldx, long P, int Hin, int Win, int Kp, int Cin,
+                                                    const float* scale1, const float* shift1, const float* DY, int ld_dy,
+                                                    const float* Zr, int ld_z, const float* cA, const float* cB,
+                                                    const float* cC, float* partial, float* dW, int grid, float* dz_out,
+                                                    const float* W1, int k_lo, const float* G_lo, const float* G_hi,
+                                                    int ldg, float* N12_lo, float* N12_hi, double* partials_n,
+                                                    eml_stream_t stream) {
+  if (!dz_out || !G_lo || !G_hi || !N12_lo || !N12_hi || k_lo + 24 > Cin || (ldg != 12 && k_lo + 24 > ldg))
+    return eml::fail(EML_EINVAL, "eml_dense_conv1x1_bwd_weight_n24_f32: needs dz_out, both G operands and outputs, and "
+                                 "k_lo + 24 <= Cin (k_lo=%d, Cin=%d)", k_lo, Cin);
+  return launch_bwd_weight(X, ldx, P, Hin, Win, 0, Kp, Cin, scale1, shift1, DY, ld_dy, Zr, ld_z, cA, cB, cC, 48, partial,
+                           dW, grid, dz_out, W1, k_lo, G_lo, ldg, N12_hi, partials_n, G_hi, N12_lo, stream);
 }
 
 extern "C" int eml_dense_permute_w1_bwd_f32(const float* W, int Cout, int Cin, int Kp, int Ko, float* Wd,
@@ -3054,10 +3131,12 @@
                           const float* X, int ldx, const float* mean, const float* istd, long P, int k_lo, int k_hi,
                           float* G, int ldg, int grid, const unsigned long long* const* relu_masks, float* top,
                           eml_stream_t stream) {
-  if (top && (n_layers != 2 || !relu_masks || Zr || k_lo != 0 || k_hi < 24 || (k_hi & 3) || P * 12 > 2147483647L))
-    return eml::fail(EML_EINVAL, "eml_dense_conv1x1_bwd_data_multi_top_f32: the compact top-24 output needs two layers, "
-                                 "relu_masks, materialised dz, k_lo == 0 and k_hi >= 24, a multiple of 4 (k_hi=%d)", k_hi);
-  if (n_layers < 1 || n_layers > 2 || !DZ || !Wd || !scale1 || !shift1 || !partials ||
+  if (top && (n_layers < 2 || n_layers > 3 || !relu_masks || Zr || k_lo != 0 || k_hi < 12 * n_layers || (k_hi & 3) ||
+              P * 12 * n_layers > 2147483647L))
+    return eml::fail(EML_EINVAL, "eml_dense_conv1x1_bwd_data_multi_top_f32: the compact top-12*n output needs two or three "
+                                 "layers, relu_masks, materialised dz, k_lo == 0 and k_hi >= 12*n, a multiple of 4 (k_hi=%d)",
+                     k_hi);
+  if (n_layers < 1 || n_layers > 3 || !DZ || !Wd || !scale1 || !shift1 || !partials ||
       !Kp || (!relu_masks && (!X || !mean || !istd)) || !G || P < 1 || grid < 1 || k_lo < 0 || k_hi <= k_lo ||
       (ldx & 3) || (ldg & 3))
     return eml::fail(EML_EINVAL, "eml_dense_conv1x1_bwd_data_multi_f32: bad arguments");
@@ -3066,10 +3145,10 @@
     return eml::fail(EML_EINVAL, "eml_dense_conv1x1_bwd_data_multi_f32: Zr given without cA/cB/cC");
   if (relu_masks && !raw)
     return eml::fail(EML_EINVAL, "eml_dense_conv1x1_bwd_data_multi_f32: relu_masks needs the materialised dz (Zr == NULL)");
-  BwdLayer L[2];
-  const unsigned long long* Mk[2] = {nullptr, nullptr};
+  BwdLayer L[3];
+  const unsigned long long* Mk[3] = {nullptr, nullptr, nullptr};
   int kmax = 0;
-  for (int j = 0; j < 2; ++j) {
+  for (int j = 0; j < 3; ++j) {
     const int s = j < n_layers ? j : 0;
     const unsigned long long* mk = relu_masks ? relu_masks[s] : nullptr;
     Mk[j] = mk;
@@ -3087,24 +3166,33 @@
   do {                                                                                                              \
     EML_ENSURE_LDS((&conv1x1_bwd_data_multi_kernel<NLV, MTV, RAWV, MSKV>), lds);                                 \
     hipLaunchKernelGGL((conv1x1_bwd_data_multi_kernel<NLV, MTV, RAWV, MSKV>), dim3(grid), dim3(256), lds,            \
-                       (hipStream_t)stream, L[0], L[1], X, ldx, mean, istd, (int)P, k_lo, k_hi, G, ldg, kmax,        \
-                       Mk[0], Mk[1], (float*)nullptr);                                                              \
+                       (hipStream_t)stream, L[0], L[1], L[2], X, ldx, mean, istd, (int)P, k_lo, k_hi, G, ldg, kmax,  \
+                       Mk[0], Mk[1], Mk[2], (float*)nullptr);                                                       \
+  } while (0)
+#define EML_LAUNCH_MULTI_TOP(NLV)                                                                                    \
+  do {                                                                                                              \
+    EML_ENSURE_LDS((&conv1x1_bwd_data_multi_kernel<NLV, 2, true, true, true>), lds);                                 \
+    hipLaunchKernelGGL((conv1x1_bwd_data_multi_kernel<NLV, 2, true, true, true>), dim3(grid), dim3(256), lds,        \
+                       (hipStream_t)stream, L[0], L[1], L[2], X, ldx, mean, istd, (int)P, k_lo, k_hi, G, ldg, kmax,  \
+                       Mk[0], Mk[1], Mk[2], top);                                                                   \
   } while (0)
   if (n_layers == 1) {
     if (relu_masks) EML_LAUNCH_MULTI(1, 4, true, true);
     else if (raw) EML_LAUNCH_MULTI(1, 4, true, false);
     else EML_LAUNCH_MULTI(1, 4, false, false);
+  } else if (n_layers == 3) {
+    if (!relu_masks) return eml::fail(EML_EINVAL, "eml_dense_conv1x1_bwd_data_masked_f32: three layers need relu_masks");
+    if (top) EML_LAUNCH_MULTI_TOP(3);
+    else EML_LAUNCH_MULTI(3, 2, true, true);
   } else if (top) {
-    EML_ENSURE_LDS((&conv1x1_bwd_data_multi_kernel<2, 2, true, true, true>), lds);
-    hipLaunchKernelGGL((conv1x1_bwd_data_multi_kernel<2, 2, true, true, true>), dim3(grid), dim3(256), lds,
-                       (hipStream_t)stream, L[0], L[1], X, ldx, mean, istd, (int)P, k_lo, k_hi, G, ldg, kmax, Mk[0], Mk[1],
-                       top);
+    EML_LAUNCH_MULTI_TOP(2);
   } else {
     if (relu_masks) EML_LAUNCH_MULTI(2, 2, true, true);
     else if (raw) EML_LAUNCH_MULTI(2, 2, true, false);
     else EML_LAUNCH_MULTI(2, 2, false, false);
   }
 #undef EML_LAUNCH_MULTI
+#undef EML_LAUNCH_MULTI_TOP
   return eml::check_launch("eml_dense_conv1x1_bwd_data_multi_f32");
 }
 }
@@ -3117,6 +3205,8 @@
                                                     const float* mean, const float* istd, long P, int k_lo, int k_hi,
                                                     float* G, int ldg, int grid,
                                                     const unsigned long long* const* relu_masks, eml_stream_t stream) {
+  if (n_layers < 1 || n_layers > 2)
+    return eml::fail(EML_EINVAL, "eml_dense_conv1x1_bwd_data_multi_f32: bad arguments (n_layers=%d)", n_layers);
   return launch_bwd_data_multi(n_layers, DZ, Zr, cA, cB, cC, Wd, scale1, shift1, partials, Kp, X, ldx, mean, istd, P, k_lo,
                                k_hi, G, ldg, grid, relu_masks, nullptr, stream);
 }
@@ -3130,6 +3220,18 @@
   if (!top) return eml::fail(EML_EINVAL, "eml_dense_conv1x1_bwd_data_multi_top_f32: top is NULL");
   return launch_bwd_data_multi(2, DZ, nullptr, nullptr, nullptr, nullptr, Wd, scale1, shift1, partials, Kp, nullptr, 0,
                                nullptr, nullptr, P, 0, k_hi, G, ldg, grid, relu_masks, top, stream);
+}
+
+extern "C" int eml_dense_conv1x1_bwd_data_masked_f32(int n_layers, const float* const* DZ, const float* const* Wd,
+                                                     const float* const* scale1, const float* const* shift1,
+                                                     double* const* partials, const int* Kp, long P, int k_lo, int k_hi,
+                                                     float* G, int ldg, int grid,
+                                                     const unsigned long long* const* relu_masks, float* top,
+                                                     eml_stream_t stream) {
+  if (!relu_masks || (top && n_layers < 2))
+    return eml::fail(EML_EINVAL, "eml_dense_conv1x1_bwd_data_masked_f32: needs relu_masks (and two or three layers for top)");
+  return launch_bwd_data_multi(n_layers, DZ, nullptr, nullptr, nullptr, nullptr, Wd, scale1, shift1, partials, Kp, nullptr, 0,
+                               nullptr, nullptr, P, k_lo, k_hi, G, ldg, grid, relu_masks, top, stream);
 }
 
 extern "C" int eml_dense_conv1x1_bwd_narrow_f32(const float* DZ, const float* W1, int Cin, int k_lo, const float* X,
diff --git a/include/emlight_hip.h b/include/emlight_hip.h
--- a/include/emlight_hip.h
+++ b/include/emlight_hip.h
@@ -181,6 +181,13 @@
                                      const float* W1, int k_lo, const float* G, int ldg, float* N12,
                                      double* partials_n, eml_stream_t stream);
 
+int eml_dense_conv1x1_bwd_weight_n24_f32(const float* X, int ldx, long P, int Hin, int Win, int Kp, int Cin,
+                                         const float* scale1, const float* shift1, const float* DY, int ld_dy,
+                                         const float* Zr, int ld_z, const float* cA, const float* cB,
+                                         const float* cC, float* partial, float* dW, int grid, float* dz_out,
+                                         const float* W1, int k_lo, const float* G_lo, const float* G_hi, int ldg,
+                                         float* N12_lo, float* N12_hi, double* partials_n, eml_stream_t stream);
+
 int eml_dense_permute_w1_bwd_f32(const float* W, int Cout, int Cin, int Kp, int Ko, float* Wd,
                                  eml_stream_t stream);
 
@@ -206,6 +213,12 @@
                                              double* const* partials, const int* Kp, long P, int k_hi, float* G,
                                              int ldg, int grid, const unsigned long long* const* relu_masks,
                                              float* top, eml_stream_t stream);
+
+int eml_dense_conv1x1_bwd_data_masked_f32(int n_layers, const float* const* DZ, const float* const* Wd,
+                                          const float* const* scale1, const float* const* shift1,
+                                          double* const* partials, const int* Kp, long P, int k_lo, int k_hi,
+                                          float* G, int ldg, int grid, const unsigned long long* const* relu_masks,
+                                          float* top, eml_stream_t stream);
 
 int eml_dense_conv1x1_bwd_narrow_f32(const float* DZ, const float* W1, int Cin, int k_lo, const float* X,
                                      int ldx, const float* scale1, const float* shift1,
```

Measured after the change: 567.4 images/s (median of 3 runs). No clear change (+0.0%).
